# cbiffle/rtiow-rust

Measured on AMD Instinct MI355X. Metric: Msamples/s (pixels*spp/s), book-1 random-spheres 1200x800, higher is better.
Workload: dtype f32

## Files before the change

include/rtiow_gpu_debug.h:

```cpp
#ifndef RTIOW_GPU_DEBUG_H
#define RTIOW_GPU_DEBUG_H
#include "rtiow_gpu.h"
#ifdef __cplusplus
extern "C" {
#endif

int rtg_debug_box_plan(rtg_builder* b, const rtg_id* world, size_t n, const uint32_t* words, size_t n_records,
                       uint8_t* mask_out, size_t capacity);

#ifdef __cplusplus
}
#endif
#endif
```

rtiow-rust_amd/capi.py:

```python
import ctypes as C
import math
import os
import time

import numpy as np

from . import noise

c_f32p = C.POINTER(C.c_float)
c_u32p = C.POINTER(C.c_uint32)
c_u8p = C.POINTER(C.c_uint8)

INVALID_ID = 0xFFFFFFFF
FLAG_COUNTERS = 1
FLAG_TRACE_KERNEL = 2
FLAG_PARTIAL = 4
FLAG_RESUME = 8
FLAG_SUM_SQUARES = 16
FLAG_SAMPLE_COUNTS = 32
FLAG_RETIRE = 64
RETIRE_MAX_RADIUS = 8
FLAG_DENOISE = 128
DENOISE_MAX_RADIUS = 8
DENOISE_MAX_PATCH = 3
# ... 202 lines not shown
    if be.prefix != "rtg_":
        raise ValueError("%s: %s (prefix %s) does not implement RTG_FLAG_%s" % (_FLAG_OF[part][0], be.path, be.prefix, _FLAG_OF[part][1]))


class Frame:

    def __init__(self, nx, ny, squares=False, counts=False, retire=False, denoise=None, features=None):
        lay = self.layout = FrameLayout(nx, ny, squares, counts, retire, _given(denoise), _given(features))
        self.nx, self.ny, self.squares = nx, ny, lay.squares
        self.buf = np.zeros(lay.words, dtype=np.float32)

        def plane(at, *shape):
            return None if at is None else self.buf[at:at + math.prod(shape)].reshape(shape)

        def block(cls, at):
            return None if at is None else cls.from_buffer(self.buf, at * 4)
        self.planes = plane(0, *((2, ny, nx, 3) if lay.squares else (ny, nx, 3)))
        self.counts = None if lay.counts is None else plane(lay.counts, ny, nx).view(np.uint32)
        self.denoised, self.albedo, self.normal = (plane(at, ny, nx, 3) for at in (lay.denoised, lay.albedo, lay.normal))
        self.depth = plane(lay.depth, ny, nx)
        self.retire, self.denoise, self.features = block(Retire, lay.retire), block(Denoise, lay.denoise), block(Features, lay.features)
        if self.denoise is not None:
            self.set_in(make_denoise(denoise))
        if self.features is not None:
            self.set_in(make_features(features))

    def flags(self):
        return {"squares": self.squares, "counts": self.counts is not None, "retire": self.retire is not None,
                "denoise": self.denoise is not None, "features": self.features is not None}

    def set_in(self, block):
        C.memmove(C.addressof(getattr(self, type(block).__name__.lower())), C.addressof(block), block.OUT_OFFSET)

    def copy_in(self, out=None, counts=None, retire=None):
        if out is not None:
            self.planes[...] = out
        if counts is not None:
            self.counts[...] = counts
        if retire is not None:
            C.memmove(C.addressof(self.retire), C.addressof(retire), C.sizeof(Retire))

    def copy_back(self, out=None, counts=None, retire=None):
        if out is not None:
            out[...] = self.planes
        if counts is not None:
            counts[...] = self.counts
        if retire is not None:
            C.memmove(C.addressof(retire), C.addressof(self.retire), C.sizeof(Retire))


class CountsFrame(Frame):

    def __init__(self, nx, ny, squares=False, retire=False):
        if retire and not squares:
            raise ValueError("a retire frame has two float planes: squares=True")
        super().__init__(nx, ny, squares, True, retire)


class DenoiseFrame(Frame):

    def __init__(self, nx, ny, counts=False, retire=False, denoise=None):
        super().__init__(nx, ny, True, counts, retire, denoise if _given(denoise) else True)


class FeaturesFrame(Frame):

    def __init__(self, nx, ny, squares=False, counts=False, retire=False, denoise=None, features=None):
        super().__init__(nx, ny, squares, counts, retire, denoise, features if _given(features) else True)


def features_frame(nx, ny, squares=False, counts=False, retire=False, denoise=None, features=None):
    return FeaturesFrame(nx, ny, squares, counts, retire, denoise, features)


def denoise_frame(nx, ny, counts=False, retire=False, denoise=None):
    return DenoiseFrame(nx, ny, counts, retire, denoise)


def counts_frame(nx, ny, squares=False, retire=False):
    return CountsFrame(nx, ny, squares, retire)


def _counts_call(out, counts, nx, ny, squares, retire=None):
    counts = np.asarray(counts)
    if counts.shape != (ny, nx):
        raise ValueError("counts= must have shape (ny, nx) = %s" % ((ny, nx),))
    if (out.dtype == np.float32 and out.flags.c_contiguous and counts.dtype == np.uint32 and counts.flags.c_contiguous
            and out.ctypes.data + out.nbytes == counts.ctypes.data
            and (retire is None or C.addressof(retire) == out.ctypes.data + retire_block_offset(nx, ny))):
        return out, None
    f = CountsFrame(nx, ny, squares, retire is not None)
    f.copy_in(out, counts, retire)
    return f.planes, f


def _host_frame(out, nx, ny, squares, kw):
    shape = (2, ny, nx, 3) if squares else (ny, nx, 3)
    if out is None:
        if _resumes(kw):
            raise ValueError("resume=True needs out= (the running sum to continue)")
        return np.zeros(shape, dtype=np.float32)
    if squares and not (isinstance(out, np.ndarray) and out.shape == shape and out.dtype == np.float32 and out.flags.c_contiguous):
        raise ValueError("squares=True needs out= a C-contiguous float32 array of shape %s" % (shape,))
    return out


def _render(supported, call, nx, ny, ns, seed, stats, out, counters, counts, retire, denoise, features, kw, exact, forward=False):
    kw = dict(kw)
    squares = kw.pop("squares", None)
    has_rt, has_dn, has_ft = _given(retire), _given(denoise), _given(features)
    in_place = isinstance(out, Frame)
    f = None
    plain = forward and not (in_place or isinstance(counts, np.ndarray) or isinstance(retire, Retire)
                             or isinstance(denoise, (dict, Denoise)) or isinstance(features, (dict, Features)))
    if plain:
        flags, parts = {"squares": squares, "counts": counts, "retire": retire, "denoise": denoise, "features": features}, ()
    else:
        if has_dn and not squares and (exact or not in_place):
            raise ValueError("denoise= needs squares=True (the filter reads both planes)")
        blocks = [make(x) for x, make in ((denoise, make_denoise), (features, make_features)) if _given(x) and x is not True]
        if in_place:
            f, name = out, type(out).__name__
            if (f.nx, f.ny) != (nx, ny):
                raise ValueError("out= is a %s of another size" % name)
            if isinstance(counts, np.ndarray) or (exact and (counts is not None or retire is not None)):
                raise ValueError("out= a %s brings its own counts / retire views" % name)
            if has_ft and f.features is None:
                raise ValueError("features=: out= must be a FeaturesFrame or an array")
            if (has_dn and f.denoise is None) or (has_rt and f.retire is None):
                raise ValueError("out= a %s has no such block" % name)
            if ((squares is not None or exact) and bool(squares) != f.squares) or (
                    exact and (has_dn != (f.denoise is not None) or has_ft != (f.features is not None))):
                raise ValueError("out= a %s: squares= / denoise= / features= must say what the frame holds" % name)
            if isinstance(retire, Retire):
                blocks.append(retire)
            flags = f.flags()
        else:
            if has_rt and not (isinstance(retire, Retire) and isinstance(counts, np.ndarray) and squares):
                raise ValueError("retire= needs a Retire, squares=True and counts= a uint32 array (the call writes it)")
            if counts is not None and np.asarray(counts).shape != (ny, nx):
                raise ValueError("counts= must have shape (ny, nx) = %s" % ((ny, nx),))
            if out is None and _resumes(kw):
                raise ValueError("resume=True needs out= (the running sum to continue)")
            flags = {"squares": bool(squares), "counts": counts is not None, "retire": has_rt, "denoise": has_dn, "features": has_ft}
        parts = [part for part, on in flags.items() if on]
    for part in parts:
        supported(part)
    if in_place:
        for block in blocks:
            f.set_in(block)
        ret, buf = f, f.buf
    elif (has_dn or has_ft) and not plain:
        f = (FeaturesFrame(nx, ny, squares, counts is not None, has_rt, denoise if has_dn else None, features) if has_ft else
             DenoiseFrame(nx, ny, counts is not None, has_rt, denoise))
        f.copy_in(None if out is None else _host_frame(out, nx, ny, squares, kw), counts, retire if has_rt else None)
        ret, buf = f, f.buf
    else:
        ret = out = buf = _host_frame(out, nx, ny, squares, kw)
        if counts is not None and not plain:
            buf, f = _counts_call(out, counts, nx, ny, squares, retire if has_rt else None)
    p = make_params(nx, ny, ns, seed=seed, flags=FLAG_COUNTERS if stats and counters else 0, **flags, **kw)
    st = call(p, buf)
    if f is not None and not in_place:
        f.copy_back(out, counts if has_rt else None, retire if has_rt else None)
    return (ret, st.as_dict()) if stats else ret


def _adaptive_host(cast, nx, ny, ns, step, target_se, min_samples, budget_s, out, seed, stats, radius, denoise, features, kw):
    if features is not None:
        f = FeaturesFrame(nx, ny, True, True, False, denoise) if out is None else out
        what = "features=: out= must be a FeaturesFrame(nx, ny, squares=True, counts=True, denoise=...)"
    elif denoise is not None:
        f = DenoiseFrame(nx, ny, True) if out is None else out
        what = "denoise=: out= must be a DenoiseFrame(nx, ny, counts=True)"
    else:
        f = CountsFrame(nx, ny, True) if out is None else out
        what = "out= must be a CountsFrame(nx, ny, squares=True)"
    on = {"denoise": True if denoise is not None else None, "features": True if features is not None else None}
    if not isinstance(f, Frame) or (f.nx, f.ny) != (nx, ny) or f.flags() != {
            "squares": True, "counts": True, "retire": False, "denoise": denoise is not None, "features": features is not None}:
        raise ValueError(what)
    for block in (features, denoise):
        if block is not None:
            f.set_in(block)
    more = () if features is None else (f,)
    f.counts[...] = ns
    active = np.ones((ny, nx), dtype=bool)
    t0 = time.perf_counter()
    done = 0
    while done < ns:
        end = min(ns, done + step)
        _, st = cast(end, seed=seed, out=f, sample_begin=done, resume=True, partial=True, squares=True, stats=True, counters=False,
                     **on, **kw)
        if features is not None:
            f.features.compute = 0
        if stats is not None:
            stats.append(st)
        done = end
        held = np.minimum(f.counts, done).astype(np.uint32)
        se = noise.standard_error_counts(f.planes[0], f.planes[1], held)
        if radius:
            retire = noise.retire(active, done, se, min_samples, target_se, radius=radius, present=f.counts > 0)
        else:
            retire = noise.retire(active, done, se, min_samples, target_se)
        f.counts[retire] = done
        active &= ~retire
        pv = CountsFrame(nx, ny)
        pv.copy_in(f.planes[0], held)
        cast(done, seed=seed, out=pv, sample_begin=done, resume=True, **kw)
        if denoise is not None:
            yield (held, pv.planes, se, f.denoised.copy()) + more
        else:
            yield (held, pv.planes, se) + more
        if not active.any():
            return
        if budget_s is not None and time.perf_counter() - t0 >= budget_s:
            return


ERR_INVALID, ERR_EMPTY_BVH, ERR_NAN, ERR_RANGE, ERR_UNSUPPORTED, ERR_DEVICE = -1, -2, -3, -4, -5, -6


class RtError(RuntimeError):
    def __init__(self, code, msg):
        super().__init__("rt error %d: %s" % (code, msg))
        self.code = code


def _f3(v):
    return (C.c_float * 3)(float(v[0]), float(v[1]), float(v[2]))


ABI_SYMBOLS = [
    "version", "last_error", "device_count", "builder_create", "builder_destroy",
    "texture_constant", "texture_checker", "texture_perlin", "builder_set_perlin_tables",
    "material_lambertian", "material_metal", "material_dielectric", "material_diffuse_light",
    "material_isotropic", "object_sphere", "object_rect", "object_flip_normals", "object_translate",
    "object_scale", "object_rotate_y", "object_and", "object_rect_prism", "object_linear_move",
    "object_constant_medium", "object_bvh", "object_bvh_sah", "camera_look", "scene_create", "scene_destroy",
    "scene_set_option", "scene_info", "par_cast", "par_cast_device", "par_cast_multi", "multi_reset", "debug_hit_top", "debug_samples", "debug_math", "debug_flatten", "debug_flatten_pool2", "tonemap", "tonemap_device",
]


class Backend:

    def __init__(self, path, prefix):
        if not os.path.exists(path):
            raise FileNotFoundError(
                "%s not found -- build it first (python -c 'import __graft_entry__ as g; g.build()')" % path)
        self.path = path
        self.prefix = prefix
        self.lib = C.CDLL(path)
        f = self._fn
        f("last_error", C.c_char_p, [])
        f("version", C.c_char_p, [])
        f("builder_create", C.c_int, [C.POINTER(C.c_void_p)])
        f("builder_destroy", None, [C.c_void_p])
        f("texture_constant", C.c_uint32, [C.c_void_p, c_f32p])
        f("texture_checker", C.c_uint32, [C.c_void_p, C.c_uint32, C.c_uint32])
        f("texture_perlin", C.c_uint32, [C.c_void_p, C.c_float])
        f("builder_set_perlin_tables", C.c_int, [C.c_void_p, c_f32p, c_u8p, c_u8p, c_u8p])
        f("material_lambertian", C.c_uint32, [C.c_void_p, C.c_uint32])
        f("material_metal", C.c_uint32, [C.c_void_p, c_f32p, C.c_float])
        f("material_dielectric", C.c_uint32, [C.c_void_p, C.c_float])
        f("material_diffuse_light", C.c_uint32, [C.c_void_p, C.c_uint32, C.c_float])
        f("material_isotropic", C.c_uint32, [C.c_void_p, C.c_uint32])
        f("object_sphere", C.c_uint32, [C.c_void_p, C.c_float, C.c_uint32])
        f("object_rect", C.c_uint32, [C.c_void_p, C.c_int] + [C.c_float] * 5 + [C.c_uint32])
        f("object_flip_normals", C.c_uint32, [C.c_void_p, C.c_uint32])
        f("object_translate", C.c_uint32, [C.c_void_p, c_f32p, C.c_uint32])
        f("object_scale", C.c_uint32, [C.c_void_p, c_f32p, C.c_uint32])
        f("object_rotate_y", C.c_uint32, [C.c_void_p, C.c_float, C.c_uint32])
        f("object_and", C.c_uint32, [C.c_void_p, C.c_uint32, C.c_uint32])
        f("object_rect_prism", C.c_uint32, [C.c_void_p, c_f32p, c_f32p, C.c_uint32])
        f("object_linear_move", C.c_uint32, [C.c_void_p, C.c_uint32, c_f32p])
        f("object_constant_medium", C.c_uint32, [C.c_void_p, C.c_uint32, C.c_float, C.c_uint32])
        f("object_bvh", C.c_uint32, [C.c_void_p, c_u32p, C.c_size_t, C.c_float, C.c_float])
        f("object_bvh_sah", C.c_uint32, [C.c_void_p, c_u32p, C.c_size_t, C.c_float, C.c_float])
        f("camera_look", C.c_int, [c_f32p, c_f32p, c_f32p] + [C.c_float] * 6 + [C.POINTER(Camera)])
        f("scene_create", C.c_int, [C.c_void_p, c_u32p, C.c_size_t, C.c_int, C.POINTER(C.c_void_p)])
        f("scene_destroy", None, [C.c_void_p])
        self._declare_render()
        f("debug_hit_top", C.c_int, [C.c_void_p, C.c_size_t, c_f32p, C.c_uint64, C.c_float, c_f32p, c_u32p])
        f("debug_samples", C.c_int, [C.c_void_p, C.POINTER(Camera), C.POINTER(Params), C.c_size_t,
                                     c_u32p, c_u32p, c_u32p, c_f32p, c_u32p])
        f("debug_math", C.c_int, [C.c_int, C.c_int, C.c_size_t, c_f32p, c_f32p, c_f32p])
        f("tonemap", C.c_int, [C.c_int, C.c_size_t, c_f32p, c_u8p])

    def _declare_render(self):
        f = self._fn
        f("device_count", C.c_int, [C.POINTER(C.c_int)])
        f("scene_set_option", C.c_int, [C.c_void_p, C.c_char_p, C.c_int])
        f("scene_info", C.c_int, [C.c_void_p, c_u32p, c_u32p, c_u32p, C.POINTER(C.c_uint64), c_u32p])
        f("par_cast", C.c_int, [C.c_void_p, C.POINTER(Camera), C.POINTER(Params), c_f32p, C.POINTER(Stats)])
        f("par_cast_device", C.c_int, [C.c_void_p, C.POINTER(Camera), C.POINTER(Params), C.c_void_p,
                                       C.c_void_p, C.POINTER(Stats)])
        f("par_cast_multi", C.c_int, [C.POINTER(C.c_void_p), C.c_int, C.POINTER(Camera), C.POINTER(Params), c_f32p,
                                      C.POINTER(Stats)])
        f("multi_reset", C.c_int, [C.c_char_p, C.POINTER(C.c_uint64)])
        f("debug_flatten", C.c_int, [C.c_void_p, c_u32p, C.c_size_t, c_u32p, c_u32p, c_u32p, C.c_size_t])
        f("debug_flatten_pool2", C.c_int, [C.c_void_p, c_u32p, C.c_size_t, c_u32p, c_u32p, c_u32p, C.c_size_t])
        f("tonemap_device", C.c_int, [C.c_int, C.c_size_t, C.c_void_p, C.c_void_p, C.c_void_p])
        f("debug_box_plan", C.c_int, [C.c_void_p, c_u32p, C.c_size_t, c_u32p, C.c_size_t, c_u8p, C.c_size_t])

    def _fn(self, name, restype, argtypes):
        try:
            fn = getattr(self.lib, self.prefix + name)
        except AttributeError:
            def fn(*_a, _n=self.prefix + name):
                raise RtError(ERR_INVALID, "%s: symbol %s is not exported by this build" % (self.path, _n))
            setattr(self, "_" + name, fn)
            return fn
        fn.restype = restype
        fn.argtypes = argtypes
        setattr(self, "_" + name, fn)
        return fn

    def last_error(self):
        return (self._last_error() or b"").decode()

    def check(self, code):
        if code != 0:
            raise RtError(code, self.last_error())

    def check_id(self, i):
        if i == INVALID_ID:
            raise RtError(-1, self.last_error())
        return i

    def builder(self):
        return Builder(self)

    def device_count(self):
        n = C.c_int(0)
        self.check(self._device_count(C.byref(n)))
        return n.value

    def camera_look(self, look_from, look_at, up, fov, aspect, aperture, focus_dist, exposure=(0.0, 1.0)):
        cam = Camera()
        self.check(self._camera_look(_f3(look_from), _f3(look_at), _f3(up), fov, aspect, aperture,
                                     focus_dist, exposure[0], exposure[1], C.byref(cam)))
        return cam

    def par_cast_multi(self, scenes, camera, nx, ny, ns, seed=0xDEADBEEF, stats=False, out=None, counters=None, **kw):
        kw = dict(kw)
        counts, retire, denoise, features = (kw.pop(k, None) for k in ("counts", "retire", "denoise", "features"))
        return _render(lambda part: _supported(self, part), lambda p, buf: self._par_cast_multi_call(scenes, camera, p, buf),
                       nx, ny, ns, seed, stats, out, True if counters is None else counters, counts, retire, denoise, features, kw,
                       exact=False, forward=True)

    def _par_cast_multi_call(self, scenes, camera, p, buf):
        st = Stats.new()
        arr = (C.c_void_p * len(scenes))(*[s.h for s in scenes])
        self.check(self._par_cast_multi(arr, len(scenes), C.byref(camera), C.byref(p), buf.ctypes.data_as(c_f32p), C.byref(st)))
        return st

    def adaptive_multi(self, scenes, camera, nx, ny, ns, step, target_se, min_samples=16, budget_s=None, out=None, seed=0xDEADBEEF,
                       stats=None, radius=0, denoise=None, features=None, **kw):
        if step < 1:
            raise ValueError("step must be >= 1")
        if not 0 <= radius <= RETIRE_MAX_RADIUS:
            raise ValueError("radius must be in 0 .. %d" % RETIRE_MAX_RADIUS)
        _supported(self, "squares")
        _supported(self, "counts")
        features = make_features(features) if _given(features) else None
        denoise = make_denoise(denoise) if _given(denoise) else None
        yield from _adaptive_host(lambda n, **k: self.par_cast_multi(scenes, camera, nx, ny, n, **k), nx, ny, ns, step,
                                  target_se, min_samples, budget_s, out, seed, stats, radius, denoise, features, kw)

    def multi_reset(self, rccl_library=None):
        n = C.c_uint64(0)
        self.check(self._multi_reset(rccl_library.encode() if rccl_library else None, C.byref(n)))
        return n.value

    def tonemap(self, img, device=0):
        x = np.ascontiguousarray(img, dtype=np.float32)
        out = np.empty(x.shape, dtype=np.uint8)
        self.check(self._tonemap(device, x.size, x.ctypes.data_as(c_f32p), out.ctypes.data_as(c_u8p)))
        return out

    def debug_math(self, op, x, y=None, device=0):
        x = np.ascontiguousarray(x, dtype=np.float32)
        out = np.empty_like(x)
        yp = None
        if y is not None:
            y = np.ascontiguousarray(y, dtype=np.float32)
            yp = y.ctypes.data_as(c_f32p)
        self.check(self._debug_math(device, op, x.size, x.ctypes.data_as(c_f32p), yp,
                                    out.ctypes.data_as(c_f32p)))
        return out


class Builder:

    def __init__(self, backend):
        self.be = backend
        h = C.c_void_p()
        backend.check(backend._builder_create(C.byref(h)))
        self.h = h
        self._scenes = []

    def close(self):
        if self.h:
            self.be._builder_destroy(self.h)
            self.h = None

    def __del__(self):
        try:
            self.close()
        except Exception:
            pass

    def constant(self, color):
        return self.be.check_id(self.be._texture_constant(self.h, _f3(color)))

    def checker(self, t0, t1):
        return self.be.check_id(self.be._texture_checker(self.h, t0, t1))

    def perlin(self, scale):
        return self.be.check_id(self.be._texture_perlin(self.h, scale))

    def set_perlin_tables(self, vecs, perm_x, perm_y, perm_z):
        vecs = np.ascontiguousarray(vecs, dtype=np.float32).reshape(768)
        px, py, pz = (np.ascontiguousarray(a, dtype=np.uint8) for a in (perm_x, perm_y, perm_z))
        self.be.check(self.be._builder_set_perlin_tables(
            self.h, vecs.ctypes.data_as(c_f32p), px.ctypes.data_as(c_u8p), py.ctypes.data_as(c_u8p),
            pz.ctypes.data_as(c_u8p)))

    def lambertian(self, albedo):
        return self.be.check_id(self.be._material_lambertian(self.h, albedo))

    def metal(self, albedo, fuzz):
        return self.be.check_id(self.be._material_metal(self.h, _f3(albedo), fuzz))

    def dielectric(self, ref_idx):
        return self.be.check_id(self.be._material_dielectric(self.h, ref_idx))

    def diffuse_light(self, emission, brightness):
        return self.be.check_id(self.be._material_diffuse_light(self.h, emission, brightness))

    def isotropic(self, albedo):
        return self.be.check_id(self.be._material_isotropic(self.h, albedo))

    def sphere(self, radius, material):
        return self.be.check_id(self.be._object_sphere(self.h, radius, material))

    def rect(self, orthogonal_to, range0, range1, k, material):
        return self.be.check_id(self.be._object_rect(self.h, orthogonal_to, range0[0], range0[1],
                                                     range1[0], range1[1], k, material))

    def flip_normals(self, obj):
        return self.be.check_id(self.be._object_flip_normals(self.h, obj))

    def translate(self, offset, obj):
        return self.be.check_id(self.be._object_translate(self.h, _f3(offset), obj))

    def scale(self, factor, obj):
        return self.be.check_id(self.be._object_scale(self.h, _f3(factor), obj))

    def rotate_y(self, degrees, obj):
        return self.be.check_id(self.be._object_rotate_y(self.h, degrees, obj))

    def and_(self, a, b):
        return self.be.check_id(self.be._object_and(self.h, a, b))

    def rect_prism(self, p0, p1, material):
        return self.be.check_id(self.be._object_rect_prism(self.h, _f3(p0), _f3(p1), material))

    def linear_move(self, obj, motion):
        return self.be.check_id(self.be._object_linear_move(self.h, obj, _f3(motion)))

    def constant_medium(self, boundary, density, material):
        return self.be.check_id(self.be._object_constant_medium(self.h, boundary, density, material))

    def bvh(self, objs, exposure=(0.0, 1.0)):
        arr = (C.c_uint32 * max(1, len(objs)))(*objs)
        return self.be.check_id(self.be._object_bvh(self.h, arr, len(objs), exposure[0], exposure[1]))

    def flatten(self, world):
        arr = (C.c_uint32 * max(1, len(world)))(*world)
        n, feat = C.c_uint32(), C.c_uint32()
        self.be.check(self.be._debug_flatten(self.h, arr, len(world), C.byref(n), C.byref(feat), None, 0))
        words = np.zeros((n.value, 8), dtype=np.uint32)
        self.be.check(self.be._debug_flatten(self.h, arr, len(world), C.byref(n), C.byref(feat),
                                             words.ctypes.data_as(c_u32p), n.value))
        return words, feat.value

    def flatten_pool2(self, world):
        arr = (C.c_uint32 * max(1, len(world)))(*world)
        n = C.c_uint32()
        table = np.zeros(24, dtype=np.uint32)
        self.be.check(self.be._debug_flatten_pool2(self.h, arr, len(world), C.byref(n), table.ctypes.data_as(c_u32p), None, 0))
        words = np.zeros((n.value, 8), dtype=np.uint32)
        self.be.check(self.be._debug_flatten_pool2(self.h, arr, len(world), C.byref(n), table.ctypes.data_as(c_u32p),
                                                   words.ctypes.data_as(c_u32p), n.value))
        items = [tuple(int(v) for v in table[4 * k:4 * k + 4]) for k in range(int(table[20]))]
        return words, items, int(table[21]), int(table[22])

    def box_plan(self, world=None, words=None):
        if words is not None:
            words = np.ascontiguousarray(words, dtype=np.uint32)
            mask = np.zeros(len(words), dtype=np.uint8)
            n = self.be._debug_box_plan(None, None, 0, words.ctypes.data_as(c_u32p), len(words), mask.ctypes.data_as(c_u8p), len(mask))
        else:
            arr = (C.c_uint32 * max(1, len(world)))(*world)
            n = self.be._debug_box_plan(self.h, arr, len(world), None, 0, None, 0)
            if n < 0:
                self.be.check(n)
            mask = np.zeros(n, dtype=np.uint8)
            n = self.be._debug_box_plan(self.h, arr, len(world), None, 0, mask.ctypes.data_as(c_u8p), len(mask))
        if n < 0:
            self.be.check(n)
        return mask

    def bvh_sah(self, objs, exposure=(0.0, 1.0)):
        arr = (C.c_uint32 * max(1, len(objs)))(*objs)
        return self.be.check_id(self.be._object_bvh_sah(self.h, arr, len(objs), exposure[0], exposure[1]))

    def scene(self, world, device=0):
        arr = (C.c_uint32 * max(1, len(world)))(*world)
        h = C.c_void_p()
        self.be.check(self.be._scene_create(self.h, arr, len(world), device, C.byref(h)))
        sc = self.be.scene_class(self.be, h, self)
        sc.apply_env_options()
        return sc


class Scene:
    def __init__(self, backend, handle, builder):
        self.be = backend
        self.h = handle
        self._builder = builder

    def close(self):
        if self.h:
            self.be._scene_destroy(self.h)
            self.h = None

    def __del__(self):
        try:
            self.close()
        except Exception:
            pass

    ENV_OPTIONS = ("kernel", "chunks", "lpt", "lpt_phase1", "lpt_deep", "lpt_shift", "ray_lds", "sync", "block", "wg_per_cu", "window",
                   "box_leave", "refill_min", "gather_min", "run_ahead", "run_ahead_min", "sphere_min", "verbose", "bvh4", "box_chains", "box_prune", "force_rccl", "multi_gather", "multi_planes", "scratch_mb", "frames_in_flight", "small_frames", "drain_share", "hoist", "deep_sized", "mat_lds", "pool2", "p2_refill", "p2_box_leave", "p2_park", "p2_sphere", "p2_prism", "p2_list", "p2_push")

    def set_option(self, name, value):
        self.be.check(self.be._scene_set_option(self.h, name.encode(), int(value)))

    def apply_env_options(self):
        if not hasattr(self.be, "_scene_set_option"):
            return
        for name in self.ENV_OPTIONS:
            v = os.environ.get("RTG_" + name.upper())
            if v is not None:
                self.set_option(name, int(v))

    def info(self):
        a, b, c, d, e = C.c_uint32(), C.c_uint32(), C.c_uint32(), C.c_uint64(), C.c_uint32()
        self.be.check(self.be._scene_info(self.h, C.byref(a), C.byref(b), C.byref(c), C.byref(d), C.byref(e)))
        return {"instructions": a.value, "materials": b.value, "textures": c.value, "hbm_bytes": d.value, "box_followers": e.value}

    def _par_cast_args(self, args, threads):
        return args

    def par_cast(self, camera, nx, ny, ns, seed=0xDEADBEEF, stats=False, out=None, threads=0, counts=None, counters=None,
                 retire=None, denoise=None, features=None, **kw):
        def call(p, buf):
            st = Stats.new()
            self.be.check(self.be._par_cast(*self._par_cast_args(
                [self.h, C.byref(camera), C.byref(p), buf.ctypes.data_as(c_f32p), C.byref(st)], threads)))
            return st
        return _render(lambda part: _supported(self.be, part), call, nx, ny, ns, seed, stats, out,
                       stats if counters is None else counters, counts, retire, denoise, features, kw, exact=True)

    def par_cast_device(self, camera, params, d_out_ptr, stream=None, want_stats=False, sample_begin=None, partial=None,
                        resume=None, squares=None, counts=None, retire=None, denoise=None, features=None):
        over = {"squares": squares, "counts": counts, "retire": retire, "denoise": denoise, "features": features}
        bits = {"squares": FLAG_SUM_SQUARES, "counts": FLAG_SAMPLE_COUNTS, "retire": FLAG_RETIRE, "denoise": FLAG_DENOISE,
                "features": FLAG_FEATURES}
        has = {part: bool(params.flags & bits[part] if on is None else on if isinstance(on, (bool, int)) else True)
               for part, on in over.items()}
        for part in ("features", "denoise", "squares", "counts", "retire"):
            if has[part] if part == "squares" else _given(over[part]):
                _supported(self.be, part)
        lay = FrameLayout(params.nx, params.ny, **has)
        blocks = [(over[part], 4 * at, n) for part, at, n in (("retire", lay.retire, C.sizeof(Retire)),
                                                             ("denoise", lay.denoise, Denoise.OUT_OFFSET),
                                                             ("features", lay.features, Features.OUT_OFFSET))
                  if isinstance(over[part], C.Structure)]
        for block, at, n in blocks:
            self._block_copy(d_out_ptr, block, stream, True, at, n)
        if _given(counts) and counts is not True:
            self._upload_counts(lay, counts, d_out_ptr, stream)
        if sample_begin is not None or partial is not None or resume is not None or any(on is not None for on in over.values()):
            q = Params()
            C.pointer(q)[0] = params
            if sample_begin is not None:
                q.sample_begin = sample_begin
            for on, bit in [(partial, FLAG_PARTIAL), (resume, FLAG_RESUME)] + [(on if on is None else has[part], bits[part])
                                                                             for part, on in over.items()]:
                if on is not None:
                    q.flags = (q.flags | bit) if on else (q.flags & ~bit)
            params = q
        st = Stats.new()
        self.be.check(self.be._par_cast_device(self.h, C.byref(camera), C.byref(params), d_out_ptr, stream,
                                               C.byref(st) if want_stats else None))
        for block, at, _ in blocks:
            self._block_copy(d_out_ptr, block, stream, False, at, C.sizeof(block))
        return st.as_dict() if want_stats else None

    def _block_copy(self, d_out_ptr, block, stream, to_device, offset, nbytes):
        hip, hs = _hip_runtime(), _stream(stream)
        dev, host = C.c_void_p(_device_ptr(d_out_ptr) + offset), C.c_void_p(C.addressof(block))
        what = "hipMemcpyAsync(%s block)" % type(block).__name__.lower()
        _hip_ok(hip.hipMemcpyAsync(*((dev, host, nbytes, 1) if to_device else (host, dev, nbytes, 2)), hs), what)
        _hip_ok(hip.hipStreamSynchronize(hs), what)

    def _upload_counts(self, lay, counts, d_out_ptr, stream):
        hip, hs = _hip_runtime(), _stream(stream)
        dst = C.c_void_p(_device_ptr(d_out_ptr) + 4 * lay.counts)
        if hasattr(counts, "data_ptr") and getattr(counts, "is_cuda", False):
            if tuple(counts.shape) != (lay.ny, lay.nx) or counts.element_size() != 4 or not counts.is_contiguous():
                raise ValueError("counts= must be a contiguous 4-byte [ny, nx] tensor")
            _hip_ok(hip.hipMemcpyAsync(dst, C.c_void_p(counts.data_ptr()), 4 * lay.n, 3, hs), "hipMemcpyAsync(count plane)")
        else:
            host = np.ascontiguousarray(counts, dtype=np.uint32)
            if host.shape != (lay.ny, lay.nx):
                raise ValueError("counts= must have shape (ny, nx) = %s" % ((lay.ny, lay.nx),))
            _hip_ok(hip.hipMemcpyAsync(dst, C.c_void_p(host.ctypes.data), 4 * lay.n, 1, hs), "hipMemcpyAsync(count plane)")
            _hip_ok(hip.hipStreamSynchronize(hs), "hipMemcpyAsync(count plane)")

    def _loop_block(self, part, given, make):
        if not _given(given):
            return None
        _supported(self.be, part)
        return make(given)

    def adaptive(self, camera, nx, ny, ns, step, target_se, min_samples=16, budget_s=None, out=None, seed=0xDEADBEEF,
                 stats=None, radius=0, preview=None, stream=None, denoise=None, denoised=None, features=None, **kw):
        if step < 1:
            raise ValueError("step must be >= 1")
        _supported(self.be, "squares")
        _supported(self.be, "counts")
        if not 0 <= radius <= RETIRE_MAX_RADIUS:
            raise ValueError("radius must be in 0 .. %d" % RETIRE_MAX_RADIUS)
        features, denoise = self._loop_block("features", features, make_features), self._loop_block("denoise", denoise, make_denoise)
        if out is not None and not isinstance(out, Frame):
            _supported(self.be, "retire")
            if preview is None:
                raise ValueError("a device frame needs a device preview buffer (preview=)")
            if denoise is not None and denoised is None:
                raise ValueError("denoise= on a device frame needs a device buffer for the filtered frame (denoised=)")
            yield from self._adaptive_device(camera, nx, ny, ns, step, target_se, min_samples, budget_s, out, seed, stats,
                                             radius, preview, stream, kw, denoise, denoised, features)
            return
        yield from _adaptive_host(lambda n, **k: self.par_cast(camera, nx, ny, n, **k), nx, ny, ns, step, target_se,
                                  min_samples, budget_s, out, seed, stats, radius, denoise, features, kw)

    def _adaptive_device(self, camera, nx, ny, ns, step, target_se, min_samples, budget_s, out, seed, stats, radius, preview,
                         stream, kw, denoise=None, denoised=None, features=None):
        hip, hs, ok = _hip_runtime(), _stream(stream), _hip_ok
        d_out, d_pv = _device_ptr(out), _device_ptr(preview)
        lay = FrameLayout(nx, ny, True, True, True, denoise is not None, features is not None)
        plane, counts_at = lay.n, d_out + 4 * lay.counts
        ok(hip.hipMemsetD32Async(C.c_void_p(counts_at), ns - (1 << 32) if ns >= 1 << 31 else ns, plane, hs), "hipMemsetD32Async(counts)")
        block = Retire(target_se=float(target_se), min_samples=int(min_samples), radius=int(radius))
        self._block_copy(d_out, block, stream, True, 4 * lay.retire, C.sizeof(Retire))
        if denoise is not None:
            self._block_copy(d_out, denoise, stream, True, 4 * lay.denoise, Denoise.OUT_OFFSET)
        more = ()
        if features is not None:
            self._block_copy(d_out, features, stream, True, 4 * lay.features, Features.OUT_OFFSET)
            more = (4 * lay.features,)
        t0 = time.perf_counter()
        done = 0
        while done < ns:
            end = min(ns, done + step)
            st = self.par_cast_device(camera, make_params(nx, ny, end, seed=seed, sample_begin=done, resume=True, partial=True,
                                                          squares=True, counts=True, retire=True, denoise=denoise is not None,
                                                          features=features is not None, **kw), d_out, hs,
                                      want_stats=stats is not None)
            if features is not None and features.compute:
                features.compute = 0
                self._block_copy(d_out, features, stream, True, 4 * lay.features, Features.OUT_OFFSET)
            if denoise is not None:
                ok(hip.hipMemcpyAsync(C.c_void_p(_device_ptr(denoised)), C.c_void_p(d_out + 4 * lay.denoised), plane * 3 * 4, 3, hs),
                   "hipMemcpyAsync(denoised)")
            if stats is not None:
                stats.append(st)
            done = end
            ok(hip.hipMemcpyAsync(C.c_void_p(d_pv), C.c_void_p(d_out), plane * 3 * 4, 3, hs), "hipMemcpyAsync(preview)")
            ok(hip.hipMemcpyAsync(C.c_void_p(d_pv + plane * 3 * 4), C.c_void_p(counts_at), plane * 4, 3, hs), "hipMemcpyAsync(preview counts)")
            self.par_cast_device(camera, make_params(nx, ny, done, seed=seed, sample_begin=done, resume=True, counts=True, **kw),
                                 d_pv, hs)
            self._block_copy(d_out, block, stream, False, 4 * lay.retire, C.sizeof(Retire))
            info = block.as_dict()
            if denoise is not None:
                yield (done, preview, info, denoised) + more
            else:
                yield (done, preview, info) + more
            if info["active"] == 0:
                return
            if budget_s is not None and time.perf_counter() - t0 >= budget_s:
                return

    def progressive(self, camera, nx, ny, ns, step, seed=0xDEADBEEF, budget_s=None, out=None, preview=None, stream=None,
                    squares=False, target_rmse=None, denoise=None, denoised=None, features=None, **kw):
        if step < 1:
            raise ValueError("step must be >= 1")
        features = self._loop_block("features", features, make_features)
        squares = bool(squares) or target_rmse is not None or _given(denoise)
        if squares:
            _supported(self.be, "squares")
        denoise = self._loop_block("denoise", denoise, make_denoise)
        if out is not None and not isinstance(out, np.ndarray):
            if target_rmse is not None:
                raise ValueError("target_rmse needs host frames: there is no device-side error reduction")
            if preview is None:
                raise ValueError("a device running sum needs a device preview buffer (preview=)")
            if denoise is not None and denoised is None:
                raise ValueError("denoise= on a device frame needs a device buffer for the filtered frame (denoised=)")
            yield from self._progressive_device(camera, nx, ny, ns, step, seed, budget_s, out, preview, stream, squares, kw,
                                                denoise, denoised, features)
            return
        shape = (2, ny, nx, 3) if squares else (ny, nx, 3)
        acc = np.zeros(shape, dtype=np.float32) if out is None else out
        frame = None
        if features is not None:
            frame = FeaturesFrame(nx, ny, squares, denoise=denoise, features=features)
        elif denoise is not None:
            frame = DenoiseFrame(nx, ny, denoise=denoise)
        if frame is not None:
            frame.copy_in(acc)
        on = {"denoise": True if denoise is not None else None, "features": True if features is not None else None}
        more = () if features is None else (frame,)
        sums = acc[0] if squares else acc
        t0 = time.perf_counter()
        done = 0
        while done < ns:
            end = min(ns, done + step)
            self.par_cast(camera, nx, ny, end, seed=seed, out=acc if frame is None else frame, sample_begin=done, resume=True, partial=True,
                          squares=squares, **on, **kw)
            if frame is not None:
                frame.copy_back(acc)
            if features is not None:
                frame.features.compute = 0
            done = end
            pv = sums.copy()
            self.par_cast(camera, nx, ny, done, seed=seed, out=pv, sample_begin=done, resume=True, **kw)
            if squares:
                se = noise.standard_error(acc[0], acc[1], done)
                if denoise is not None:
                    yield (done, pv, se, frame.denoised.copy()) + more
                else:
                    yield (done, pv, se) + more
                if target_rmse is not None and float(np.sqrt(np.mean(se * se))) <= target_rmse:
                    return
            else:
                yield (done, pv) + more
            if budget_s is not None and time.perf_counter() - t0 >= budget_s:
                return

    def _progressive_device(self, camera, nx, ny, ns, step, seed, budget_s, acc, preview, stream, squares, kw, denoise=None,
                            denoised=None, features=None):
        hip, hs = _hip_runtime(), _stream(stream)
        d_acc, d_preview = C.c_void_p(_device_ptr(acc)), C.c_void_p(_device_ptr(preview))
        lay = FrameLayout(nx, ny, squares, False, False, denoise is not None, features is not None)
        if denoise is not None:
            self._block_copy(acc, denoise, stream, True, 4 * lay.denoise, Denoise.OUT_OFFSET)
        more = ()
        if features is not None:
            self._block_copy(acc, features, stream, True, 4 * lay.features, Features.OUT_OFFSET)
            more = (4 * lay.features,)
        t0 = time.perf_counter()
        done = 0
        while done < ns:
            end = min(ns, done + step)
            self.par_cast_device(camera, make_params(nx, ny, end, seed=seed, sample_begin=done, resume=True, partial=True,
                                                     squares=squares, denoise=denoise is not None, features=features is not None,
                                                     **kw), d_acc, hs)
            if features is not None and features.compute:
                features.compute = 0
                self._block_copy(acc, features, stream, True, 4 * lay.features, Features.OUT_OFFSET)
            done = end
            if denoise is not None:
                _hip_ok(hip.hipMemcpyAsync(C.c_void_p(_device_ptr(denoised)), C.c_void_p(d_acc.value + 4 * lay.denoised), lay.n * 3 * 4, 3, hs),
                        "hipMemcpyAsync(denoised)")
            _hip_ok(hip.hipMemcpyAsync(d_preview, d_acc, lay.n * 3 * 4, 3, hs), "hipMemcpyAsync(preview)")
            self.par_cast_device(camera, make_params(nx, ny, done, seed=seed, sample_begin=done, resume=True, **kw), d_preview, hs)
            if denoise is not None:
                yield (done, preview, acc, denoised) + more
            else:
                yield ((done, preview, acc) if squares else (done, preview)) + more
            if budget_s is not None:
                _hip_ok(hip.hipStreamSynchronize(hs), "hipStreamSynchronize")
                if time.perf_counter() - t0 >= budget_s:
                    return

    def debug_hit_top(self, rays, seed=1, t_near=0.001):
        rays = np.ascontiguousarray(rays, dtype=np.float32).reshape(-1, 7)
        n = rays.shape[0]
        out = np.zeros((n, 8), dtype=np.float32)
        mat = np.zeros(n, dtype=np.uint32)
        self.be.check(self.be._debug_hit_top(self.h, n, rays.ctypes.data_as(c_f32p), seed, t_near,
                                             out.ctypes.data_as(c_f32p), mat.ctypes.data_as(c_u32p)))
        return out, mat

    def debug_samples(self, camera, nx, ny, ns, xs, ys, samples, seed=0xDEADBEEF, trace_kernel=False, **kw):
        p = make_params(nx, ny, ns, seed=seed, flags=FLAG_TRACE_KERNEL if trace_kernel else 0, **kw)
        xs, ys, samples = (np.ascontiguousarray(a, dtype=np.uint32) for a in (xs, ys, samples))
        n = xs.size
        rgb = np.zeros((n, 3), dtype=np.float32)
        info = np.zeros((n, 4), dtype=np.uint32)
        self.be.check(self.be._debug_samples(self.h, C.byref(camera), C.byref(p), n,
                                             xs.ctypes.data_as(c_u32p), ys.ctypes.data_as(c_u32p),
                                             samples.ctypes.data_as(c_u32p), rgb.ctypes.data_as(c_f32p),
                                             info.ctypes.data_as(c_u32p)))
        return rgb, info


Backend.scene_class = Scene
```

rtiow-rust_amd/csrc/rt_box_plan.h:

```cpp
#pragma once
#include <cmath>
#include <cstddef>
#include <cstdint>
#include <cstring>
#include <vector>

#include "flat_scene.h"

namespace rtg {

constexpr uint8_t BOX_KEPT = 0, BOX_FOLLOWER = 1, BOX_PRUNED = 2;
#ifndef RT_BOX_PLAN_PROBES
#define RT_BOX_PLAN_PROBES 256
#endif
#ifndef RT_BOX_PLAN_FULL
#define RT_BOX_PLAN_FULL 0
#endif
constexpr uint32_t BOX_PLAN_PROBES = RT_BOX_PLAN_PROBES;
constexpr bool BOX_PLAN_FULL = RT_BOX_PLAN_FULL != 0;

struct BoxPlan {
  uint32_t n_pruned = 0;
  uint32_t n_sure = 0;
  uint32_t n_rays = 0;
};

namespace box_plan_detail {
inline float as_f(uint32_t u) {
  float f;
  std::memcpy(&f, &u, 4);
  return f;
}
inline bool aabb_hit(const uint32_t* lo, const uint32_t* hi, const float* o, const float* inv, float t_near, float best) {
  const float mn[3] = {as_f(lo[0]), as_f(lo[2]), as_f(hi[0])}, mx[3] = {as_f(lo[1]), as_f(lo[3]), as_f(hi[1])};
  float t0[3], t1[3];
  for (int a = 0; a < 3; a++) {
    const float u = (mn[a] - o[a]) * inv[a], v = (mx[a] - o[a]) * inv[a];
    t0[a] = inv[a] < 0.f ? v : u, t1[a] = inv[a] < 0.f ? u : v;
  }
  const float start = fmaxf(t_near, fmaxf(fmaxf(t0[0], t0[1]), t0[2]));
  const float end = fminf(best, fminf(fminf(t1[0], t1[1]), t1[2]));
  return end > start;
}
inline bool sphere_hit(const uint32_t* lo, uint32_t flags, const float* o, const float* d, float dd, float t_near, float best, float* t_out) {
  float p[3] = {o[0], o[1], o[2]};
  if (flags & F_TRANSLATE)
    for (int a = 0; a < 3; a++) p[a] = o[a] - as_f(lo[a]);
  const float r = as_f(lo[3]);
  const float b = p[0] * d[0] + p[1] * d[1] + p[2] * d[2];
  const float c = p[0] * p[0] + p[1] * p[1] + p[2] * p[2] - r * r;
  const float disc = b * b - dd * c;
  if (disc > 0.f) {
    const float sq = sqrtf(disc);
    float t = (-b - sq) / dd;
    if (t < best && t >= t_near) return *t_out = t, true;
    t = (-b + sq) / dd;
    if (t < best && t >= t_near) return *t_out = t, true;
  }
  return false;
}
struct Rng {
  uint64_t s;
  uint64_t next() {
    uint64_t z = (s += 0x9e3779b97f4a7c15ull);
    z = (z ^ (z >> 30)) * 0xbf58476d1ce4e5b9ull;
    z = (z ^ (z >> 27)) * 0x94d049bb133111ebull;
    return z ^ (z >> 31);
  }
  float unit() { return (float)(next() >> 40) * (1.f / 16777216.f); }
  void in_unit_sphere(float* v) {
    do {
      for (int a = 0; a < 3; a++) v[a] = 2.f * unit() - 1.f;
    } while (v[0] * v[0] + v[1] * v[1] + v[2] * v[2] >= 1.f);
  }
};
}

inline BoxPlan box_plan(const uint32_t (*lo)[4], const uint32_t (*hi)[4], size_t n, const uint8_t* follower, uint8_t* mask,
                        uint8_t* sure = nullptr, uint32_t n_probes = BOX_PLAN_PROBES) {
  using namespace box_plan_detail;
  BoxPlan out;
  for (size_t j = 0; j < n; j++) {
    mask[j] = follower && follower[j] ? BOX_FOLLOWER : BOX_KEPT;
    if (sure) sure[j] = 0;
  }
  auto op = [&](size_t j) { return hi[j][3] & 0xffu; };
  auto skip = [&](size_t j) { return (size_t)hi[j][2]; };
  if (n < 4 || n > 0x7fffffffu) return out;
  std::vector<int32_t> parent(n, -1);
  std::vector<uint32_t> depth(n, 0);
  {
    std::vector<uint32_t> open;
    for (size_t j = 0; j < n; j++) {
      while (!open.empty() && skip(open.back()) <= j) open.pop_back();
      if (!open.empty()) parent[j] = (int32_t)open.back(), depth[j] = (uint32_t)open.size();
      if (op(j) != OP_BOX) continue;
      if (skip(j) <= j || skip(j) >= n || (!open.empty() && skip(j) > skip(open.back()))) return out;
      open.push_back((uint32_t)j);
    }
  }
  auto leaf_box = [&](size_t j) { return op(j) == OP_BOX && j + 2 < n && op(j + 1) == OP_SPHERE && skip(j) == j + 2; };
  auto finite6 = [&](size_t j) {
    return std::isfinite(as_f(lo[j][0])) && std::isfinite(as_f(lo[j][1])) && std::isfinite(as_f(lo[j][2])) &&
           std::isfinite(as_f(lo[j][3])) && std::isfinite(as_f(hi[j][0])) && std::isfinite(as_f(hi[j][1]));
  };
  auto contains = [&](size_t j, size_t c) {
    return as_f(lo[j][0]) <= as_f(lo[c][0]) && as_f(lo[j][1]) >= as_f(lo[c][1]) && as_f(lo[j][2]) <= as_f(lo[c][2]) &&
           as_f(lo[j][3]) >= as_f(lo[c][3]) && as_f(hi[j][0]) <= as_f(hi[c][0]) && as_f(hi[j][1]) >= as_f(hi[c][1]);
  };
  std::vector<uint8_t> prunable(n, 0);
  uint32_t n_prunable = 0;
  for (size_t j = n; j-- > 0;) {
    if (op(j) != OP_BOX || j + 1 >= n || op(j + 1) != OP_BOX) continue;
    const size_t L = j + 1, R = skip(L);
    if (!(L < R && R < skip(j)) || op(R) != OP_BOX || skip(R) != skip(j)) continue;
    if (!finite6(j) || !finite6(L) || !finite6(R) || !contains(j, L) || !contains(j, R)) continue;
    if (!(leaf_box(L) || prunable[L]) || !(leaf_box(R) || prunable[R])) continue;
    prunable[j] = 1, n_prunable++;
  }
  if (!n_prunable) return out;
  std::vector<uint8_t> choosable(prunable);
  for (size_t j = 0; j + 1 < n; j++) {
    if (!prunable[j] || !follower) continue;
    size_t k = j + 1;
    while (k + 1 < n && follower[k] && !leaf_box(k)) k++;
    if (follower[k] && leaf_box(k)) choosable[j] = 0;
  }

  std::vector<uint64_t> n_pass(n, 0);
  std::vector<uint32_t> spheres, starts;
  for (size_t j = 0; j < n; j++)
    if (op(j) == OP_SPHERE) spheres.push_back((uint32_t)j);
  auto centre = [&](uint32_t j, float* c) {
    for (int a = 0; a < 3; a++) c[a] = (hi[j][3] & F_TRANSLATE) ? as_f(lo[j][a]) : 0.f;
  };
  float cmin[3] = {INFINITY, INFINITY, INFINITY}, cmax[3] = {-INFINITY, -INFINITY, -INFINITY};
  for (uint32_t j : spheres) {
    float c[3];
    centre(j, c);
    for (int a = 0; a < 3; a++) cmin[a] = fminf(cmin[a], c[a]), cmax[a] = fmaxf(cmax[a], c[a]);
  }
  std::vector<uint8_t> enclosing(n, 0);
  for (uint32_t j : spheres) {
    float cj[3];
    centre(j, cj);
    const float r = as_f(lo[j][3]);
    float far2 = 0.f;
    for (int a = 0; a < 3; a++) {
      const float d = fmaxf(cmax[a] - cj[a], cj[a] - cmin[a]);
      far2 += d * d;
    }
    const bool all = spheres.size() > 1 && far2 < r * r;
    enclosing[j] = all;
    if (!all && std::isfinite(r) && std::isfinite(cj[0]) && std::isfinite(cj[1]) && std::isfinite(cj[2])) starts.push_back(j);
  }
  uint64_t n_rays = 0;
  if (!starts.empty()) {
    Rng rng{0x626f78706c616e31ull ^ (uint64_t)n};
    const float t_near = 0.001f;
    while (n_rays < n_probes) {
      const uint32_t s0 = starts[rng.next() % starts.size()];
      float c[3], nrm[3], o[3], d[3], v[3];
      centre(s0, c);
      do rng.in_unit_sphere(nrm);
      while (nrm[0] * nrm[0] + nrm[1] * nrm[1] + nrm[2] * nrm[2] < 1e-4f);
      const float len = sqrtf(nrm[0] * nrm[0] + nrm[1] * nrm[1] + nrm[2] * nrm[2]), r0 = as_f(lo[s0][3]);
      for (int a = 0; a < 3; a++) nrm[a] /= len, o[a] = c[a] + r0 * nrm[a];
      const uint32_t bounces = 1u + (uint32_t)(rng.next() % 3u);
      for (uint32_t k = 0; k <= bounces && n_rays < n_probes; k++) {
        rng.in_unit_sphere(v);
        for (int a = 0; a < 3; a++) d[a] = nrm[a] + v[a];
        const float inv[3] = {1.f / d[0], 1.f / d[1], 1.f / d[2]};
        const float dd = d[0] * d[0] + d[1] * d[1] + d[2] * d[2];
        float best = 3.402823466e+38f;
        int64_t best_pc = -1;
        n_rays++;
        for (size_t pc = 0; pc < n;) {
          const uint32_t o_ = op(pc);
          if (o_ == OP_BOX) {
            if (aabb_hit(lo[pc], hi[pc], o, inv, t_near, best)) n_pass[pc]++, pc++;
            else pc = skip(pc);
          } else if (o_ == OP_SPHERE) {
            float t;
            if (sphere_hit(lo[pc], hi[pc][3], o, d, dd, t_near, best, &t)) best = t, best_pc = (int64_t)pc;
            pc++;
          } else break;
        }
        if (best_pc < 0 || enclosing[best_pc]) break;
        centre((uint32_t)best_pc, c);
        const float r = as_f(lo[best_pc][3]);
        for (int a = 0; a < 3; a++) o[a] = o[a] + best * d[a], nrm[a] = (o[a] - c[a]) / r;
        if (!(std::isfinite(nrm[0]) && std::isfinite(nrm[1]) && std::isfinite(nrm[2]))) break;
      }
    }
  }
  out.n_rays = (uint32_t)n_rays;

  uint64_t states = 0;
  for (size_t j = 0; BOX_PLAN_FULL && j < n; j++)
    if (op(j) == OP_BOX) states += depth[j] + 2u;
  const bool dp = BOX_PLAN_FULL && states <= (1ull << 26);
  std::vector<uint32_t> kidx(n, 0);
  std::vector<uint8_t> pruned(n, 0);
  if (dp) {
    std::vector<std::vector<uint64_t>> acc(n);
    std::vector<std::vector<uint8_t>> choice(n);
    std::vector<uint64_t> path_pass;
    for (size_t j = n; j-- > 0;) {
      if (op(j) != OP_BOX) continue;
      const uint32_t dj = depth[j];
      if (acc[j].empty()) acc[j].assign(dj + 2u, 0);
      path_pass.assign(dj + 1u, n_rays);
      for (int32_t a = parent[j], k = (int32_t)dj; a >= 0; a = parent[a], k--) path_pass[k] = n_pass[a];
      std::vector<uint64_t> f(dj + 1u);
      choice[j].assign(dj + 1u, 0);
      for (uint32_t k = 0; k <= dj; k++) {
        const uint64_t own = follower && follower[j] ? 0u : path_pass[k];
        const uint64_t keep = own + acc[j][dj + 1u], leave = acc[j][k];
        if (choosable[j] && leave <= keep) f[k] = leave, choice[j][k] = 1;
        else f[k] = keep;
      }
      std::vector<uint64_t>().swap(acc[j]);
      if (parent[j] >= 0) {
        std::vector<uint64_t>& up = acc[parent[j]];
        if (up.empty()) up.assign(dj + 1u, 0);
        for (uint32_t k = 0; k <= dj; k++) up[k] += f[k];
      }
    }
    for (size_t j = 0; j < n; j++) {
      if (op(j) != OP_BOX) continue;
      const int32_t p = parent[j];
      kidx[j] = p < 0 ? 0u : (pruned[p] ? kidx[p] : depth[j]);
      pruned[j] = choice[j][kidx[j]];
    }
  } else {
    for (size_t j = 0; j < n; j++) pruned[j] = choosable[j] && n_rays && n_pass[j] == n_rays;
  }
  for (size_t j = 0; j < n; j++) {
    if (!pruned[j] || mask[j] == BOX_FOLLOWER) continue;
    mask[j] = BOX_PRUNED, out.n_pruned++;
    if (n_pass[j] == n_rays) {
      out.n_sure++;
      if (sure) sure[j] = 1;
    }
  }
  return out;
}

}
```

rtiow-rust_amd/csrc/rtg_api.hip:

```cpp
#include <hip/hip_runtime.h>

#include <dlfcn.h>
#include <rccl/rccl.h>

#include <chrono>
#include <cmath>
#include <cstdio>
#include <cstdlib>
#include <cstring>
#include <map>
#include <mutex>
#include <functional>
#include <string>
#include <tuple>
#include <vector>

#include "../../include/rtiow_gpu.h"
#include "../../include/rtiow_gpu_debug.h"
#include "rt_pool.h"
#include "rt_box_plan.h"
#include "rt_retire.h"
#include "rt_denoise.h"
#include "rt_features.h"
#include "rt_multi_planes.h"
#include "rt_pool_full.h"
#include "rt_sync_full.h"
#include "rt_pool2.h"
#include "rt_trace.h"
#include "scene_builder.h"

using namespace rtg;

#include "rtg_kernels.inc"

namespace {
thread_local std::string g_err;

int fail(int code, const std::string& msg) {
  g_err = msg;
  return code;
}
int hip_fail(hipError_t e, const char* what) {
  return fail(RTG_ERR_DEVICE, std::string(what) + ": " + hipGetErrorString(e));
}
#define HIP_TRY(expr)                                   \
  do {                                                  \
    hipError_t e_ = (expr);                             \
    if (e_ != hipSuccess) return hip_fail(e_, #expr);   \
  } while (0)
}

struct rtg_builder {
  SceneBuilder sb;
};

constexpr int RTG_MAX_FRAMES = 4;
enum class KernelKind { baseline, lean_pool, full_pool, lock_step, pool2 };
struct LaunchCtx {
  unsigned long long* d_counters = nullptr;
  hipEvent_t ev0 = nullptr, ev1 = nullptr, done = nullptr;
  bool busy = false;
  float* d_stack = nullptr;
  size_t stack_bytes = 0;
  uint32_t* d_slots = nullptr;
  size_t slots_bytes = 0;
  float* d_scratch = nullptr;
  size_t scratch_bytes = 0;
  LaunchConsts* d_consts = nullptr;
  uint32_t* d_lpt = nullptr;
  size_t lpt_bytes = 0;
  LptQueue lpt_desc{};
  KernelKind last_kernel = KernelKind::baseline;
  uint32_t last_pix_work = 0;
  uint32_t* d_list = nullptr;
  size_t list_bytes = 0;
  uint32_t* d_compact = nullptr;
  size_t compact_bytes = 0;
  unsigned long long counts_samples = 0;
  void* d_retire = nullptr;
  size_t retire_bytes = 0;
  const char* refusal = nullptr;
  void* d_denoise = nullptr;
  size_t denoise_bytes = 0;
  rtg_denoise denoise_in{};
  uint32_t* d_features = nullptr;
  size_t features_bytes = 0;
  rtg_features features_in{};
};

struct rtg_scene {
  int device = 0;
  DevScene dev{};
  uint32_t features = 0;
  uint32_t n_prog = 0, n_mat = 0, n_tex = 0;
  uint64_t bytes = 0;
  void* buffers[15] = {};
  const uint32_t* d_parent = nullptr;
  hipStream_t own_stream = nullptr;
  int num_cus = 0;
  float* d_frame = nullptr;
  size_t frame_bytes = 0;
  int force_chunks = 0;
  uint64_t scratch_limit = 0;
  bool whole_scratch = false;
  int verbose = 0;
  int window = -1;
  int ray_lds = 1;
  int force_rccl = 0;
  int multi_gather = 0;
  float* d_pack = nullptr;
  size_t pack_bytes = 0;
  float* d_recv = nullptr;
  size_t recv_bytes = 0;
  int multi_planes = 0;
  hipEvent_t post0 = nullptr, post1 = nullptr;
  hipEvent_t pack0 = nullptr, pack1 = nullptr, unpack0 = nullptr;
  int bvh4 = 0;
  uint32_t wide_bytes = 0;
  int box_chains = 1;
  uint32_t n_followers = 0;
  const uint32_t* d_chain_off = nullptr;
  uint32_t chain_bytes = 0;
  int box_prune = 1;
  uint32_t n_pruned = 0;
  float plan_ms = 0.f;
  const uint32_t* d_prune_off[2] = {nullptr, nullptr};
  uint32_t prune_bytes[2] = {0, 0};
  std::vector<uint32_t> plan_ops;
  std::vector<uint8_t> plan_mask;
  int sync_full = -1;
  uint32_t n_box = 0;
  int lpt = 2;
  int lpt_deep = 4;
  int lpt_shift = 0;
  int lpt_phase1 = 0;
  int kernel_version = 3;
  PoolTuning pool_tune{40, 16, 24, 16, 16, 40};
  PoolTuning full_tune{20, 24, 32, 16, 24, 40};
  PoolTuning sync_tune{20, 16, 32, 16, 16, 40};
  int wg_per_cu = 0;
  int full_threads = 0;
  int pool_threads = 0;
  int mat_lds = 1;
  int deep_sized = 1;
  int hoist = 1;
  uint32_t seg_first = 0, seg_end = 0;
  int drain_share = 1;
  int pool2 = 1;
  uint32_t n_prog2 = 0, n_box2 = 0;
  DevScene dev2{};
  const P2Table* d_p2 = nullptr;
  Pool2Tuning pool2_tune{24, 48, 40, 4, 8, 24, 2};
  int guide_lds = 0;
  int small_frames = 1;
  LaunchCtx ctx[RTG_MAX_FRAMES];
  int n_ctx = 1, next_ctx = 0;
  LaunchCtx* cx = &ctx[0];
};

static void ctx_free_buffers(LaunchCtx* c) {
  if (c->busy) (void)hipEventSynchronize(c->done);
  c->busy = false;
  if (c->d_scratch) (void)hipFree(c->d_scratch);
  if (c->d_slots) (void)hipFree(c->d_slots);
  if (c->d_stack) (void)hipFree(c->d_stack);
  if (c->d_lpt) (void)hipFree(c->d_lpt);
  if (c->d_list) (void)hipFree(c->d_list);
  if (c->d_compact) (void)hipFree(c->d_compact);
  if (c->d_retire) (void)hipFree(c->d_retire);
  if (c->d_denoise) (void)hipFree(c->d_denoise);
  if (c->d_features) (void)hipFree(c->d_features);
  c->d_scratch = nullptr, c->scratch_bytes = 0, c->d_slots = nullptr, c->slots_bytes = 0;
  c->d_stack = nullptr, c->stack_bytes = 0, c->d_lpt = nullptr, c->lpt_bytes = 0;
  c->d_list = nullptr, c->list_bytes = 0, c->d_compact = nullptr, c->compact_bytes = 0;
  c->d_retire = nullptr, c->retire_bytes = 0;
  c->d_denoise = nullptr, c->denoise_bytes = 0;
  c->d_features = nullptr, c->features_bytes = 0;
}

static int ctx_acquire(rtg_scene* s) {
  LaunchCtx* c = &s->ctx[s->next_ctx];
  s->next_ctx = (s->next_ctx + 1) % s->n_ctx;
  if (!c->d_counters) {
    if (hipMalloc((void**)&c->d_counters, 64 * sizeof(unsigned long long)) != hipSuccess || hipMemset(c->d_counters, 0, 64 * sizeof(unsigned long long)) != hipSuccess ||
        hipMalloc((void**)&c->d_consts, sizeof(LaunchConsts) + sizeof(ListConsts)) != hipSuccess || hipEventCreate(&c->ev0) != hipSuccess ||
        hipEventCreate(&c->ev1) != hipSuccess || hipEventCreateWithFlags(&c->done, hipEventDisableTiming) != hipSuccess)
      return fail(RTG_ERR_DEVICE, "scene: launch-context allocation failed");
  }
  if (c->busy) {
    hipError_t e = hipEventSynchronize(c->done);
    c->busy = false;
    if (e != hipSuccess) return hip_fail(e, "hipEventSynchronize(previous frame of this launch context)");
  }
  s->cx = c;
  return RTG_OK;
}
static int ctx_release(rtg_scene* s, hipStream_t stream) {
  hipError_t e = hipEventRecord(s->cx->done, stream);
  if (e != hipSuccess) return hip_fail(e, "hipEventRecord(done)");
  s->cx->busy = true;
  return RTG_OK;
}

struct SampleSlice {
  uint32_t begin = 0;
  bool divide = true;
  bool squares = false;
  bool counts = false;
  uint32_t list_work = 0;
  ListConsts list{};
  bool retire = false;
  bool denoise = false;
  bool features = false;
  bool features_done = false;
  bool sliced() const { return begin != 0u || !divide; }
};
static SampleSlice slice_of(const rtg_params* p) {
  SampleSlice sl;
  if (p->flags & RTG_FLAG_RESUME) sl.begin = p->sample_begin;
  if (p->flags & RTG_FLAG_PARTIAL) sl.divide = false;
  if (p->flags & RTG_FLAG_SUM_SQUARES) sl.squares = true;
  if (p->flags & RTG_FLAG_SAMPLE_COUNTS) sl.counts = true;
  if (p->flags & RTG_FLAG_RETIRE) sl.retire = true;
  if (p->flags & RTG_FLAG_DENOISE) sl.denoise = true;
  if (p->flags & RTG_FLAG_FEATURES) sl.features = true;
  return sl;
}

static const char* retire_refusal(const rtg_retire& r, uint32_t nranks) {
  if (r.radius > RTG_RETIRE_MAX_RADIUS) return "RTG_FLAG_RETIRE: radius > RTG_RETIRE_MAX_RADIUS";
  if (!(r.target_se >= 0.0)) return "RTG_FLAG_RETIRE: target_se is NaN or negative";
  if (r.radius > 0u && nranks > 1u) return "RTG_FLAG_RETIRE: radius > 0 needs nranks = 1 (the neighbours live on other ranks)";
  return nullptr;
}

static const char* denoise_refusal(const rtg_denoise& r, uint32_t nranks) {
  if (r.radius > RTG_DENOISE_MAX_RADIUS) return "RTG_FLAG_DENOISE: radius > RTG_DENOISE_MAX_RADIUS";
  if (r.patch > RTG_DENOISE_MAX_PATCH) return "RTG_FLAG_DENOISE: patch > RTG_DENOISE_MAX_PATCH";
  if (!(r.k > 0.f) || !std::isfinite(r.k)) return "RTG_FLAG_DENOISE: k is NaN, infinite or <= 0";
  if (r.reserved_in != 0u) return "RTG_FLAG_DENOISE: reserved_in != 0";
  if (nranks > 1u) return "RTG_FLAG_DENOISE needs nranks = 1 (the neighbours live on other ranks)";
  return nullptr;
}

static const char* features_refusal(const rtg_features& r, bool denoise) {
  if (r.grid == 0u || r.grid > RTG_FEATURES_MAX_GRID) return "RTG_FLAG_FEATURES: grid is 0 or > RTG_FEATURES_MAX_GRID";
  if (r.compute > 1u) return "RTG_FLAG_FEATURES: compute > 1";
  if (r.reserved_in != 0u) return "RTG_FLAG_FEATURES: reserved_in != 0";
  for (float sg : {r.sigma_normal, r.sigma_albedo, r.sigma_depth})
    if (denoise && (!(sg > 0.f) || !std::isfinite(sg))) return "RTG_FLAG_FEATURES with RTG_FLAG_DENOISE: a sigma is NaN, infinite or <= 0";
  return nullptr;
}

#include "rtg_launch.inc"

template <typename T>
struct DevBuf {
  T* p = nullptr;
  ~DevBuf() {
    if (p) (void)hipFree(p);
  }
  hipError_t alloc(size_t n) { return hipMalloc((void**)&p, (n ? n : 1) * sizeof(T)); }
};

extern "C" {

const char* rtg_version(void) { return "rtiow-rust_amd 0.2 (gfx950 HIP; flat-program ray-pool kernels; flat-program encoding 3: OP_SEG = 9, OP_SAVE / OP_MERGE / OP_EXT = 10 / 11 / 12, OP_LIST = 13, MEDIUM lo.y = 1 / density)"; }
const char* rtg_last_error(void) { return g_err.c_str(); }

int rtg_device_count(int* n) {
  if (!n) return fail(RTG_ERR_INVALID, "null argument");
  int c = 0;
  hipError_t e = hipGetDeviceCount(&c);
  if (e != hipSuccess) {
    *n = 0;
    return hip_fail(e, "hipGetDeviceCount");
  }
  *n = c;
  return RTG_OK;
}

int rtg_builder_create(rtg_builder** out) {
  if (!out) return fail(RTG_ERR_INVALID, "null argument");
  *out = new rtg_builder();
  return RTG_OK;
}
void rtg_builder_destroy(rtg_builder* b) { delete b; }

static rtg_id bad(const char* msg) {
  fail(RTG_ERR_INVALID, msg);
  return RTG_INVALID_ID;
}

rtg_id rtg_texture_constant(rtg_builder* b, const float rgb[3]) {
  if (!b || !rgb) return bad("null argument");
  HostTexture t;
  t.kind = TEX_CONSTANT;
  t.rgb[0] = rgb[0], t.rgb[1] = rgb[1], t.rgb[2] = rgb[2];
  b->sb.textures.push_back(t);
  return (rtg_id)b->sb.textures.size() - 1;
}
rtg_id rtg_texture_checker(rtg_builder* b, rtg_id t0, rtg_id t1) {
  if (!b) return bad("null argument");
  if (t0 >= b->sb.textures.size() || t1 >= b->sb.textures.size()) return bad("checker: bad texture handle");
  HostTexture t;
  t.kind = TEX_CHECKER;
  t.t0 = t0, t.t1 = t1;
  b->sb.textures.push_back(t);
  return (rtg_id)b->sb.textures.size() - 1;
}
rtg_id rtg_texture_perlin(rtg_builder* b, float scale) {
  if (!b) return bad("null argument");
  if (!b->sb.has_perlin) return bad("perlin: call rtg_builder_set_perlin_tables first");
  HostTexture t;
  t.kind = TEX_PERLIN;
  t.scale = scale;
  b->sb.textures.push_back(t);
  return (rtg_id)b->sb.textures.size() - 1;
}
int rtg_builder_set_perlin_tables(rtg_builder* b, const float vecs[768], const uint8_t px[256],
                                  const uint8_t py[256], const uint8_t pz[256]) {
  if (!b || !vecs || !px || !py || !pz) return fail(RTG_ERR_INVALID, "null argument");
  for (int i = 0; i < 256; i++) {
    b->sb.perlin_vecs[4 * i] = vecs[3 * i], b->sb.perlin_vecs[4 * i + 1] = vecs[3 * i + 1];
    b->sb.perlin_vecs[4 * i + 2] = vecs[3 * i + 2], b->sb.perlin_vecs[4 * i + 3] = 0.f;
    b->sb.perlin_perm[i] = px[i], b->sb.perlin_perm[256 + i] = py[i], b->sb.perlin_perm[512 + i] = pz[i];
  }
  b->sb.has_perlin = true;
  return RTG_OK;
}

static rtg_id push_material(rtg_builder* b, uint32_t kind, rtg_id tex, const float* albedo, float param) {
  if (!b) return bad("null argument");
  HostMaterial m;
  m.kind = kind;
  if (tex != RTG_INVALID_ID) {
    if (tex >= b->sb.textures.size()) return bad("material: bad texture handle");
    m.tex = tex;
  }
  if (albedo) m.albedo[0] = albedo[0], m.albedo[1] = albedo[1], m.albedo[2] = albedo[2];
  m.param = param;
  b->sb.materials.push_back(m);
  return (rtg_id)b->sb.materials.size() - 1;
}
rtg_id rtg_material_lambertian(rtg_builder* b, rtg_id albedo) {
  if (albedo == RTG_INVALID_ID) return bad("material: bad texture handle");
  return push_material(b, MAT_LAMBERTIAN, albedo, nullptr, 0.f);
}
rtg_id rtg_material_metal(rtg_builder* b, const float albedo[3], float fuzz) {
  if (!albedo) return bad("null argument");
  return push_material(b, MAT_METAL, RTG_INVALID_ID, albedo, fuzz);
}
rtg_id rtg_material_dielectric(rtg_builder* b, float ref_idx) {
  return push_material(b, MAT_DIELECTRIC, RTG_INVALID_ID, nullptr, ref_idx);
}
rtg_id rtg_material_diffuse_light(rtg_builder* b, rtg_id emission, float brightness) {
  if (emission == RTG_INVALID_ID) return bad("material: bad texture handle");
  return push_material(b, MAT_DIFFUSE_LIGHT, emission, nullptr, brightness);
}
rtg_id rtg_material_isotropic(rtg_builder* b, rtg_id albedo) {
  if (albedo == RTG_INVALID_ID) return bad("material: bad texture handle");
  return push_material(b, MAT_ISOTROPIC, albedo, nullptr, 0.f);
}

static rtg_id push_object(rtg_builder* b, const HostObject& o) {
  if (!b) return bad("null argument");
  try {
    return b->sb.add_object(o);
  } catch (const BuildError& e) {
    fail(e.code, e.msg);
    return RTG_INVALID_ID;
  }
}
rtg_id rtg_object_sphere(rtg_builder* b, float radius, rtg_id material) {
  HostObject o;
  o.kind = HostObject::SPHERE;
  o.f[0] = radius;
  o.mat = material;
  return push_object(b, o);
}
rtg_id rtg_object_rect(rtg_builder* b, int axis, float r0s, float r0e, float r1s, float r1e, float k, rtg_id material) {
  HostObject o;
  o.kind = HostObject::RECT;
  o.axis = axis;
  o.f[0] = k, o.f[1] = r0s, o.f[2] = r0e, o.f[3] = r1s, o.f[4] = r1e;
  o.mat = material;
  return push_object(b, o);
}
static rtg_id wrapper(rtg_builder* b, HostObject::Kind kind, const float* v, rtg_id child) {
  HostObject o;
  o.kind = kind;
  if (v) o.f[0] = v[0], o.f[1] = v[1], o.f[2] = v[2];
  o.a = child;
  return push_object(b, o);
}
rtg_id rtg_object_flip_normals(rtg_builder* b, rtg_id object) { return wrapper(b, HostObject::FLIP, nullptr, object); }
rtg_id rtg_object_translate(rtg_builder* b, const float offset[3], rtg_id object) {
  if (!offset) return bad("null argument");
  return wrapper(b, HostObject::TRANSLATE, offset, object);
}
rtg_id rtg_object_scale(rtg_builder* b, const float factor[3], rtg_id object) {
  if (!factor) return bad("null argument");
  return wrapper(b, HostObject::SCALE, factor, object);
}
rtg_id rtg_object_rotate_y(rtg_builder* b, float degrees, rtg_id object) {
  float radians = degrees * 3.14159265358979323846f / 180.f;
  float sc[3] = {sinf(radians), cosf(radians), 0.f};
  return wrapper(b, HostObject::ROTATE_Y, sc, object);
}
rtg_id rtg_object_and(rtg_builder* b, rtg_id o0, rtg_id o1) {
  HostObject o;
  o.kind = HostObject::AND;
  o.a = o0, o.b = o1;
  return push_object(b, o);
}
rtg_id rtg_object_rect_prism(rtg_builder* b, const float p0[3], const float p1[3], rtg_id m) {
  if (!b || !p0 || !p1) return bad("null argument");
  rtg_id zp = rtg_object_rect(b, 2, p0[0], p1[0], p0[1], p1[1], p1[2], m);
  rtg_id yp = rtg_object_rect(b, 1, p0[0], p1[0], p0[2], p1[2], p1[1], m);
  rtg_id xp = rtg_object_rect(b, 0, p0[1], p1[1], p0[2], p1[2], p1[0], m);
  if (zp == RTG_INVALID_ID || yp == RTG_INVALID_ID || xp == RTG_INVALID_ID) return RTG_INVALID_ID;
  rtg_id zn = rtg_object_flip_normals(b, rtg_object_rect(b, 2, p0[0], p1[0], p0[1], p1[1], p0[2], m));
  rtg_id yn = rtg_object_flip_normals(b, rtg_object_rect(b, 1, p0[0], p1[0], p0[2], p1[2], p0[1], m));
  rtg_id xn = rtg_object_flip_normals(b, rtg_object_rect(b, 0, p0[1], p1[1], p0[2], p1[2], p0[0], m));
  return rtg_object_and(b, rtg_object_and(b, zp, rtg_object_and(b, yp, xp)),
                        rtg_object_and(b, zn, rtg_object_and(b, yn, xn)));
}
rtg_id rtg_object_linear_move(rtg_builder* b, rtg_id object, const float motion[3]) {
  if (!motion) return bad("null argument");
  return wrapper(b, HostObject::MOVE, motion, object);
}
rtg_id rtg_object_constant_medium(rtg_builder* b, rtg_id boundary, float density, rtg_id material) {
  HostObject o;
  o.kind = HostObject::MEDIUM;
  o.f[0] = density;
  o.a = boundary;
  o.mat = material;
  return push_object(b, o);
}
rtg_id rtg_object_bvh(rtg_builder* b, const rtg_id* objects, size_t n, float e0, float e1) {
  if (!b || (!objects && n)) return bad("null argument");
  try {
    return b->sb.add_bvh(objects, n, e0, e1);
  } catch (const BuildError& e) {
    fail(e.code, e.msg);
    return RTG_INVALID_ID;
  }
}

rtg_id rtg_object_bvh_sah(rtg_builder* b, const rtg_id* objects, size_t n, float e0, float e1) {
  if (!b || (!objects && n)) return bad("null argument");
  try {
    return b->sb.add_bvh(objects, n, e0, e1, true);
  } catch (const BuildError& e) {
    fail(e.code, e.msg);
    return RTG_INVALID_ID;
  }
}

int rtg_camera_look(const float from[3], const float at[3], const float up[3], float fov, float aspect,
                    float aperture, float focus_dist, float e0, float e1, rtg_camera* out) {
  if (!from || !at || !up || !out) return fail(RTG_ERR_INVALID, "null argument");
  auto dot3 = [](const float* a, const float* b) { return (a[0] * b[0] + a[1] * b[1]) + a[2] * b[2]; };
  auto unit = [&](float* v) {
    float len = sqrtf(dot3(v, v));
    v[0] = v[0] / len, v[1] = v[1] / len, v[2] = v[2] / len;
  };
  auto cross3 = [](const float* a, const float* b, float* r) {
    r[0] = a[1] * b[2] - a[2] * b[1];
    r[1] = -(a[0] * b[2] - a[2] * b[0]);
    r[2] = a[0] * b[1] - a[1] * b[0];
  };
  float lens_radius = aperture / 2.f;
  float theta = fov * 3.14159265358979323846f / 180.f;
  float half_height = tanf(theta / 2.f);
  float half_width = aspect * half_height;
  float w[3] = {from[0] - at[0], from[1] - at[1], from[2] - at[2]};
  unit(w);
  float u[3], v[3];
  cross3(up, w, u);
  unit(u);
  cross3(w, u, v);
  float hw_fd = half_width * focus_dist, hh_fd = half_height * focus_dist;
  float h2 = (2.f * half_width) * focus_dist, v2 = (2.f * half_height) * focus_dist;
  for (int i = 0; i < 3; i++) {
    out->origin[i] = from[i];
    out->lower_left_corner[i] = ((from[i] - hw_fd * u[i]) - hh_fd * v[i]) - focus_dist * w[i];
    out->horizontal[i] = h2 * u[i];
    out->vertical[i] = v2 * v[i];
    out->u[i] = u[i];
    out->v[i] = v[i];
  }
  out->lens_radius = lens_radius;
  out->exposure_start = e0;
  out->exposure_end = e1;
  return RTG_OK;
}

static int upload(void** dst, const void* src, size_t bytes, uint64_t* total) {
  size_t alloc = bytes ? bytes : 16;
  HIP_TRY(hipMalloc(dst, alloc));
  if (bytes) HIP_TRY(hipMemcpy(*dst, src, bytes, hipMemcpyHostToDevice));
  *total += alloc;
  return RTG_OK;
}

static int prune_table(rtg_scene* s, int chains) {
  if (s->d_prune_off[chains] || !s->n_pruned) return RTG_OK;
  const size_t n = s->plan_mask.size();
  std::vector<uint8_t> drop(n);
  std::vector<uint32_t> off(n);
  for (size_t i = 0; i < n; i++) drop[i] = s->plan_mask[i] == BOX_PRUNED || (chains && s->plan_mask[i] == BOX_FOLLOWER);
  s->prune_bytes[chains] = lds_image_offsets(s->plan_ops.data(), n, off.data(), drop.data());
  int rc = upload(&s->buffers[13 + chains], off.data(), n * sizeof(uint32_t), &s->bytes);
  if (rc) return rc;
  s->d_prune_off[chains] = (const uint32_t*)s->buffers[13 + chains];
  return RTG_OK;
}

void rtg_scene_destroy(rtg_scene* s) {
  if (!s) return;
  (void)hipSetDevice(s->device);
  for (void* p : s->buffers)
    if (p) (void)hipFree(p);
  for (LaunchCtx& c : s->ctx) {
    ctx_free_buffers(&c);
    if (c.d_counters) (void)hipFree(c.d_counters);
    if (c.d_consts) (void)hipFree(c.d_consts);
    if (c.ev0) (void)hipEventDestroy(c.ev0);
    if (c.ev1) (void)hipEventDestroy(c.ev1);
    if (c.done) (void)hipEventDestroy(c.done);
  }
  if (s->d_frame) (void)hipFree(s->d_frame);
  if (s->d_pack) (void)hipFree(s->d_pack);
  if (s->d_recv) (void)hipFree(s->d_recv);
  if (s->post0) (void)hipEventDestroy(s->post0);
  if (s->post1) (void)hipEventDestroy(s->post1);
  for (hipEvent_t ev : {s->pack0, s->pack1, s->unpack0})
    if (ev) (void)hipEventDestroy(ev);
  if (s->own_stream) (void)hipStreamDestroy(s->own_stream);
  delete s;
}

int rtg_scene_create(rtg_builder* b, const rtg_id* world, size_t n, int device, rtg_scene** out) {
  if (!b || !out || (!world && n)) return fail(RTG_ERR_INVALID, "null argument");
  FlatScene fs;
  try {
    b->sb.flatten(world, n, &fs);
  } catch (const BuildError& e) {
    return fail(e.code, e.msg);
  }
  int ndev = 0;
  if (hipGetDeviceCount(&ndev) != hipSuccess || ndev == 0)
    return fail(RTG_ERR_DEVICE, "no HIP device: the rtiow hot path has no CPU fallback");
  if (device < 0 || device >= ndev) return fail(RTG_ERR_INVALID, "bad device index");
  HIP_TRY(hipSetDevice(device));
  rtg_scene* s = new rtg_scene();
  s->device = device;
  s->features = fs.features;
  s->n_prog = (uint32_t)fs.lo.size();
  s->n_mat = (uint32_t)fs.mat.size() / 2;
  s->n_tex = (uint32_t)fs.tex.size() / 2;
  int rc;
  if ((rc = upload(&s->buffers[0], fs.lo.data(), fs.lo.size() * 16, &s->bytes)) ||
      (rc = upload(&s->buffers[1], fs.hi.data(), fs.hi.size() * 16, &s->bytes)) ||
      (rc = upload(&s->buffers[2], fs.mat.data(), fs.mat.size() * 16, &s->bytes)) ||
      (rc = upload(&s->buffers[3], fs.tex.data(), fs.tex.size() * 16, &s->bytes)) ||
      (rc = upload(&s->buffers[4], fs.perlin_vecs.data(), sizeof(float) * 1024, &s->bytes)) ||
      (rc = upload(&s->buffers[5], fs.perlin_perm.data(), 768, &s->bytes))) {
    rtg_scene_destroy(s);
    return rc;
  }
  s->dev.lo = (const uint4*)s->buffers[0];
  s->dev.hi = (const uint4*)s->buffers[1];
  s->dev.mat = (const uint4*)s->buffers[2];
  s->dev.tex = (const uint4*)s->buffers[3];
  s->dev.perlin_vecs = (const float4*)s->buffers[4];
  s->dev.perlin_perm = (const uint8_t*)s->buffers[5];
  s->dev.n_prog = s->n_prog;
  s->dev.n_mat = s->n_mat;
  for (const Packet& h : fs.hi) s->n_box += (h.w[3] & 0xffu) == OP_BOX ? 1u : 0u;
  {
    std::vector<uint32_t> parent(fs.hi.size(), 0xffffffffu), open;
    for (size_t i = 0; i < fs.hi.size(); i++) {
      const uint32_t op = fs.hi[i].w[3] & 0xffu;
      if (op == OP_POP && !open.empty()) open.pop_back();
      parent[i] = open.empty() ? 0xffffffffu : open.back();
      if (op == OP_PUSH) open.push_back((uint32_t)i);
    }
    if ((rc = upload(&s->buffers[8], parent.data(), parent.size() * sizeof(uint32_t), &s->bytes))) {
      rtg_scene_destroy(s);
      return rc;
    }
    s->d_parent = (const uint32_t*)s->buffers[8];
  }
  for (size_t i = 0; i < fs.hi.size(); i++)
    if ((fs.hi[i].w[3] & 0xffu) == OP_SEG) s->seg_first = (uint32_t)i + 1u, s->seg_end = fs.hi[i].w[2];
  if (!fs.hi2.empty()) {
    if ((rc = upload(&s->buffers[9], fs.lo2.data(), fs.lo2.size() * 16, &s->bytes)) ||
        (rc = upload(&s->buffers[10], fs.hi2.data(), fs.hi2.size() * 16, &s->bytes)) ||
        (rc = upload(&s->buffers[11], &fs.p2, sizeof(P2Table), &s->bytes))) {
      rtg_scene_destroy(s);
      return rc;
    }
    s->dev2 = s->dev;
    s->dev2.lo = (const uint4*)s->buffers[9], s->dev2.hi = (const uint4*)s->buffers[10];
    s->dev2.n_prog = s->n_prog2 = (uint32_t)fs.hi2.size();
    s->dev2.lds_off = nullptr, s->dev2.lds_image_bytes = 0;
    s->d_p2 = (const P2Table*)s->buffers[11];
    for (const Packet& h : fs.hi2) s->n_box2 += (h.w[3] & 0xffu) == OP_BOX ? 1u : 0u;
  }
  if ((fs.features & (FEAT_ALL | FEAT_BOUNDARY)) == 0) {
    std::vector<uint32_t> ops(fs.hi.size()), off(fs.hi.size());
    for (size_t i = 0; i < fs.hi.size(); i++) ops[i] = fs.hi[i].w[3];
    s->dev.lds_image_bytes = lds_image_offsets(ops.data(), ops.size(), off.data());
    if ((rc = upload(&s->buffers[6], off.data(), off.size() * sizeof(uint32_t), &s->bytes))) {
      rtg_scene_destroy(s);
      return rc;
    }
    s->dev.lds_off = (const uint32_t*)s->buffers[6];
    std::vector<uint8_t> follower(fs.hi.size());
    s->n_followers = box_chain_followers(reinterpret_cast<const uint32_t (*)[4]>(fs.lo.data()), reinterpret_cast<const uint32_t (*)[4]>(fs.hi.data()), fs.hi.size(), follower.data());
    if (s->n_followers) {
      s->chain_bytes = lds_image_offsets(ops.data(), ops.size(), off.data(), follower.data());
      if ((rc = upload(&s->buffers[12], off.data(), off.size() * sizeof(uint32_t), &s->bytes))) {
        rtg_scene_destroy(s);
        return rc;
      }
      s->d_chain_off = (const uint32_t*)s->buffers[12];
    }
    if (s->dev.lds_image_bytes - LDS_BOX_BYTES * (s->n_box / 2u) <= 160u * 1024u) {
      s->plan_mask.resize(fs.hi.size());
      const auto t0 = std::chrono::steady_clock::now();
      s->n_pruned = box_plan(reinterpret_cast<const uint32_t (*)[4]>(fs.lo.data()), reinterpret_cast<const uint32_t (*)[4]>(fs.hi.data()), fs.hi.size(), follower.data(), s->plan_mask.data()).n_pruned;
      s->plan_ms = std::chrono::duration<float, std::milli>(std::chrono::steady_clock::now() - t0).count();
      if (s->n_pruned) {
        s->plan_ops = ops;
        if ((rc = prune_table(s, 1))) {
          rtg_scene_destroy(s);
          return rc;
        }
      }
    }
    std::vector<uint32_t> wide;
    if (build_wide_image(fs.lo.data(), fs.hi.data(), fs.hi.size(), wide)) {
      if ((rc = upload(&s->buffers[7], wide.data(), wide.size() * sizeof(uint32_t), &s->bytes))) {
        rtg_scene_destroy(s);
        return rc;
      }
      s->wide_bytes = (uint32_t)(wide.size() * sizeof(uint32_t));
    }
  }
  hipDeviceProp_t prop;
  if (hipGetDeviceProperties(&prop, device) == hipSuccess) s->num_cus = prop.multiProcessorCount;
  if (s->num_cus <= 0) s->num_cus = 256;
  if ((rc = ctx_acquire(s))) {
    rtg_scene_destroy(s);
    return rc;
  }
  s->next_ctx = 0;
  *out = s;
  return RTG_OK;
}


int rtg_scene_set_option(rtg_scene* s, const char* name, int value) {
  if (!s || !name) return fail(RTG_ERR_INVALID, "null argument");
  const std::string k(name);
  const uint32_t u = (uint32_t)value;
  if (k == "kernel") s->kernel_version = value;
  else if (k == "chunks") s->force_chunks = value;
  else if (k == "scratch_mb") s->scratch_limit = value > 0 ? (uint64_t)value << 20 : 0;
  else if (k == "lpt") s->lpt = value;
  else if (k == "lpt_phase1") s->lpt_phase1 = value;
  else if (k == "lpt_deep") s->lpt_deep = value;
  else if (k == "lpt_shift") s->lpt_shift = std::min(6, std::max(0, value));
  else if (k == "ray_lds") s->ray_lds = value;
  else if (k == "box_chains") {
    if (!value) {
      HIP_TRY(hipSetDevice(s->device));
      int rc = prune_table(s, 0);
      if (rc) return rc;
    }
    s->box_chains = value;
  }
  else if (k == "box_prune") {
    if (value < 0 || value > 2) return fail(RTG_ERR_INVALID, "box_prune: 0 .. 2");
    s->box_prune = value;
  }
  else if (k == "bvh4") {
    if (value && !s->wide_bytes) return fail(RTG_ERR_INVALID, "bvh4: the scene is not one Bvh of spheres (no 4-wide image)");
    if (value && pool_lds_bytes(s->wide_bytes, s->n_mat, (uint32_t)(s->pool_threads > 0 ? s->pool_threads : RT_POOL_MAX_THREADS) / 64u, true, false) > 160 * 1024)
      return fail(RTG_ERR_INVALID, "bvh4: the 4-wide image does not fit a CU's 160 KB of LDS (the 4-wide walk only exists LDS-staged)");
    s->bvh4 = value;
  }
  else if (k == "frames_in_flight") {
    if (value < 1 || value > RTG_MAX_FRAMES) return fail(RTG_ERR_INVALID, "frames_in_flight: 1 .. 4");
    HIP_TRY(hipSetDevice(s->device));
    for (int i = value; i < RTG_MAX_FRAMES; i++) ctx_free_buffers(&s->ctx[i]);
    s->n_ctx = value, s->next_ctx = 0;
  }
  else if (k == "force_rccl") s->force_rccl = value;
  else if (k == "multi_gather") s->multi_gather = value;
  else if (k == "multi_planes") s->multi_planes = value;
  else if (k == "sync") s->sync_full = value;
  else if (k == "block") {
    if (value < 64 || value > 1024 || value % 64) return fail(RTG_ERR_INVALID, "block: a multiple of 64 in [64, 1024]");
    s->pool_threads = s->full_threads = value;
  }
  else if (k == "wg_per_cu") s->wg_per_cu = value;
  else if (k == "drain_share") s->drain_share = value;
  else if (k == "hoist") s->hoist = value;
  else if (k == "pool2") s->pool2 = value;
  else if (k == "deep_sized") s->deep_sized = value;
  else if (k == "mat_lds") s->mat_lds = value;
  else if (k == "guide_lds") s->guide_lds = value;
  else if (k == "small_frames") s->small_frames = value;
  else if (k == "verbose") s->verbose = value;
  else if (k == "window") s->window = value;
  else if (k == "box_leave") s->pool_tune.box_leave = s->full_tune.box_leave = s->sync_tune.box_leave = u;
  else if (k == "refill_min") s->pool_tune.refill_min = s->full_tune.refill_min = s->sync_tune.refill_min = u;
  else if (k == "gather_min") s->pool_tune.gather_min = s->full_tune.gather_min = s->sync_tune.gather_min = u;
  else if (k == "run_ahead") s->pool_tune.run_ahead = s->full_tune.run_ahead = s->sync_tune.run_ahead = u;
  else if (k == "run_ahead_min") s->pool_tune.run_ahead_min = s->full_tune.run_ahead_min = s->sync_tune.run_ahead_min = u;
  else if (k == "sphere_min") s->pool_tune.sphere_min = s->full_tune.sphere_min = s->sync_tune.sphere_min = std::max(1u, u);
  else if (k == "p2_refill") s->pool2_tune.refill_min = u;
  else if (k == "p2_box_leave") s->pool2_tune.box_leave = u;
  else if (k == "p2_park") s->pool2_tune.park_max = u;
  else if (k == "p2_sphere") s->pool2_tune.t_sphere = std::max(1u, u);
  else if (k == "p2_prism") s->pool2_tune.t_prism = std::max(1u, u);
  else if (k == "p2_list") s->pool2_tune.t_list = std::max(1u, u);
  else if (k == "p2_push") s->pool2_tune.t_push = std::max(1u, u);
  else return fail(RTG_ERR_INVALID, "rtg_scene_set_option: unknown option '" + k + "'");
  return RTG_OK;
}

int rtg_scene_info(const rtg_scene* s, uint32_t* n_instructions, uint32_t* n_materials, uint32_t* n_textures,
                   uint64_t* hbm_bytes, uint32_t* n_box_followers) {
  if (!s) return fail(RTG_ERR_INVALID, "null argument");
  if (n_instructions) *n_instructions = s->n_prog;
  if (n_materials) *n_materials = s->n_mat;
  if (n_textures) *n_textures = s->n_tex;
  if (hbm_bytes) *hbm_bytes = s->bytes;
  if (n_box_followers) *n_box_followers = s->n_followers;
  return RTG_OK;
}

static DevCamera to_dev(const rtg_camera* c) {
  DevCamera d;
  auto v = [](const float* p) { return V3{p[0], p[1], p[2]}; };
  d.origin = v(c->origin), d.llc = v(c->lower_left_corner), d.horizontal = v(c->horizontal);
  d.vertical = v(c->vertical), d.u = v(c->u), d.v = v(c->v);
  d.lens_radius = c->lens_radius, d.e0 = c->exposure_start, d.e1 = c->exposure_end;
  return d;
}

static int check_params(const rtg_scene* s, const rtg_camera* camera, const rtg_params* p, DevParams* out) {
  if (!s || !camera || !p) return fail(RTG_ERR_INVALID, "null argument");
  if (p->struct_size != sizeof(rtg_params)) return fail(RTG_ERR_INVALID, "rtg_params.struct_size mismatch");
  if (p->nx == 0 || p->ny == 0 || p->ns == 0) return fail(RTG_ERR_INVALID, "nx, ny, ns must be > 0");
  if ((uint64_t)p->nx * p->ny > 0xffffffffull) return fail(RTG_ERR_INVALID, "image too large for 32-bit pixel index");
  if (!(camera->exposure_start < camera->exposure_end))
    return fail(RTG_ERR_RANGE, "Uniform::sample_single called with low >= high");
  if (!std::isfinite(camera->exposure_start) || !std::isfinite(camera->exposure_end))
    return fail(RTG_ERR_RANGE, "Uniform::sample_single called with non-finite boundaries");
  if (!std::isfinite(camera->exposure_end - camera->exposure_start))
    return fail(RTG_ERR_RANGE, "exposure range wider than f32::MAX is not supported");
  DevParams d;
  d.nx = p->nx, d.ny = p->ny, d.ns = p->ns, d.max_bounces = p->max_bounces;
  d.t_near = p->t_near;
  d.seed_lo = (uint32_t)p->seed, d.seed_hi = (uint32_t)(p->seed >> 32);
  d.tile_w = p->tile_w ? p->tile_w : 16u;
  d.tile_h = p->tile_h ? p->tile_h : 16u;
  if (d.tile_w % 8u || d.tile_h % 8u) return fail(RTG_ERR_INVALID, "tile_w / tile_h must be multiples of 8");
  d.nranks = p->nranks ? p->nranks : 1u;
  d.rank = p->rank;
  if (d.rank >= d.nranks) return fail(RTG_ERR_INVALID, "rank >= nranks");
  if ((p->flags & RTG_FLAG_RESUME) && p->sample_begin > p->ns) return fail(RTG_ERR_INVALID, "RTG_FLAG_RESUME: sample_begin > ns");
  if ((p->flags & RTG_FLAG_RETIRE) && (~p->flags & (RTG_FLAG_SAMPLE_COUNTS | RTG_FLAG_SUM_SQUARES)))
    return fail(RTG_ERR_INVALID, "RTG_FLAG_RETIRE needs RTG_FLAG_SAMPLE_COUNTS | RTG_FLAG_SUM_SQUARES");
  if ((p->flags & RTG_FLAG_DENOISE) && !(p->flags & RTG_FLAG_SUM_SQUARES)) return fail(RTG_ERR_INVALID, "RTG_FLAG_DENOISE needs RTG_FLAG_SUM_SQUARES");
  if ((p->flags & RTG_FLAG_DENOISE) && d.nranks > 1u) return fail(RTG_ERR_INVALID, "RTG_FLAG_DENOISE needs nranks = 1 (the neighbours live on other ranks)");
  *out = d;
  return RTG_OK;
}

static int print_schedule_stats(rtg_scene* s, float ms) {
  if (s->cx->lpt_desc.n_blocks && s->cx->d_lpt) {
    std::vector<uint32_t> ctl(LPT_CTL);
    HIP_TRY(hipMemcpy(ctl.data(), s->cx->lpt_desc.ctl, LPT_CTL * sizeof(uint32_t), hipMemcpyDeviceToHost));
    std::string line;
    for (uint32_t c = 0; c < LPT_CLASSES; c++)
      if (ctl[c]) line += " " + std::to_string(c) + ":" + std::to_string(ctl[c]);
    fprintf(stderr, "[rtg] cost-ordered queue: %u of %u blocks filed, class:blocks%s\n", ctl[LPT_CLASSES], s->cx->lpt_desc.n_blocks, line.c_str());
  }
  unsigned long long q[24];
  HIP_TRY(hipMemcpy(q, s->cx->d_counters + 8, sizeof(q), hipMemcpyDeviceToHost));
  if (q[18]) {
    const double us = (double)ms * 1000. / (double)q[16], n = (double)q[18];
    fprintf(stderr, "[rtg] wave timeline (us from its start): sees the work queue empty at min %.0f / mean %.0f / max %.0f; done at mean %.0f / max %.0f\n",
            (double)((1ull << 62) - q[19]) * us, (double)q[20] / n * us, (double)q[21] * us, (double)q[17] / n * us, (double)q[16] * us);
  }
  double tt = (double)(q[8] + q[9] + q[10] + q[11]);
  fprintf(stderr, "[rtg] wave-time shares (s_memtime, instrumented variant): shade %.1f%% gen+pull|service %.1f%% box %.1f%% sphere %.1f%%; "
          "per pass: shade %.0f, gen|service %.0f, box %.0f, sphere %.0f ticks\n", 100 * q[8] / tt, 100 * q[9] / tt, 100 * q[10] / tt,
          100 * q[11] / tt, q[4] ? (double)q[8] / q[4] : 0., q[4] ? (double)q[9] / q[4] : 0., q[0] ? (double)q[10] / q[0] : 0.,
          q[2] ? (double)q[11] / q[2] : 0.);
  if (q[15]) {
    unsigned long long f[2];
    HIP_TRY(hipMemcpy(f, s->cx->d_counters + 5, sizeof(f), hipMemcpyDeviceToHost));
    fprintf(stderr, "[rtg] services %llu: finish step %.1f%% of wave time (%.0f ticks each), refill step %.1f%% (%.0f ticks per refill)\n", f[0],
            100 * f[1] / tt, f[0] ? (double)f[1] / f[0] : 0., 100 * q[15] / tt, q[6] ? (double)q[15] / q[6] : 0.);
  }
#ifdef RT_CENSUS
  {
    unsigned long long c[32];
    HIP_TRY(hipMemcpy(c, s->cx->d_counters + 32, sizeof(c), hipMemcpyDeviceToHost));
    static const char* nm[13] = {"BOX", "END", "no-ray", "held", "?", "?", "SPHERE", "RECT", "PUSH", "POP", "MEDIUM", "PRISM", "BEND"};
    for (int k = 0; k < 2; k++) {
      std::string line;
      char buf[64];
      for (int j = 0; j < 13; j++)
        if (c[16 * k + j]) snprintf(buf, sizeof buf, " %s %.1f", nm[j], (double)c[16 * k + j] / (double)c[16 * k + 15]), line += buf;
      fprintf(stderr, "[rtg] lane census at %s (%llu):%s\n", k ? "slow-pass iterations" : "box steps", c[16 * k + 15], line.c_str());
    }
  }
#endif
  fprintf(stderr, "[rtg] pool schedule: box steps %llu (avg %.1f lanes), sphere passes %llu (avg %.1f lanes), shade passes %llu "
            "(avg %.1f lanes), end / camera-ray passes %llu (avg %.1f lanes), refills %llu (avg %.1f lanes)\n", q[0], q[0] ? (double)q[1] / q[0] : 0.0, q[2],
            q[2] ? (double)q[3] / q[2] : 0.0, q[4], q[4] ? (double)q[5] / q[4] : 0.0, q[12], q[12] ? (double)q[13] / q[12] : 0.0, q[6],
            q[6] && q[7] ? (double)q[7] / q[6] : 0.0);
  return RTG_OK;
}

int rtg_par_cast_device(rtg_scene* s, const rtg_camera* camera, const rtg_params* params, float* d_out,
                        void* hip_stream, rtg_stats* stats) {
  DevParams d;
  int rc = check_params(s, camera, params, &d);
  if (rc) return rc;
  if (!d_out) return fail(RTG_ERR_INVALID, "null output");
  if (stats && stats->struct_size != sizeof(rtg_stats)) return fail(RTG_ERR_INVALID, "rtg_stats.struct_size mismatch");
  HIP_TRY(hipSetDevice(s->device));
  hipStream_t stream = (hipStream_t)hip_stream;
  if ((rc = ctx_acquire(s))) return rc;
  DevCamera cam = to_dev(camera);
  bool count = stats && (params->flags & RTG_FLAG_COUNTERS);
  const SampleSlice sl = slice_of(params);
#define HIP_TRY_CTX(expr)                               \
  do {                                                  \
    hipError_t e_ = (expr);                             \
    if (e_ != hipSuccess) {                             \
      (void)hipStreamSynchronize(stream);               \
      return hip_fail(e_, #expr);                       \
    }                                                   \
  } while (0)
  if ((sl.denoise || sl.features) && !sl.counts) {
    if (sl.denoise) {
      const void* d_block = reinterpret_cast<const uint32_t*>(d_out) + denoise_block_word(d.nx, d.ny, false, false);
      HIP_TRY(hipMemcpyAsync(&s->cx->denoise_in, d_block, offsetof(rtg_denoise, filtered), hipMemcpyDeviceToHost, stream));
    }
    if (sl.features) HIP_TRY(read_features_block(d, d_out, stream, sl, &s->cx->features_in));
    HIP_TRY(hipStreamSynchronize(stream));
    if (sl.denoise)
      if (const char* why = denoise_refusal(s->cx->denoise_in, d.nranks)) return fail(RTG_ERR_INVALID, why);
    if (sl.features)
      if (const char* why = features_refusal(s->cx->features_in, sl.denoise)) return fail(RTG_ERR_INVALID, why);
  }
  if (count) {
    HIP_TRY_CTX(hipMemsetAsync(s->cx->d_counters, 0, 7 * sizeof(unsigned long long), stream));
    HIP_TRY_CTX(hipMemsetAsync(s->cx->d_counters + 8, 0, 24 * sizeof(unsigned long long), stream));
    HIP_TRY_CTX(hipMemsetAsync(s->cx->d_counters + 32, 0, 32 * sizeof(unsigned long long), stream));
  }
#ifdef RT_TIMELINE
  static uint32_t* d_tl = nullptr;
  const size_t tl_bytes = (size_t)1024 * 16 * 16 * sizeof(uint32_t);
  if (!count) {
    if (!d_tl) HIP_TRY_CTX(hipMalloc((void**)&d_tl, tl_bytes));
    HIP_TRY_CTX(hipMemsetAsync(d_tl, 0, tl_bytes, stream));
    static unsigned long long tl_ptr;
    tl_ptr = (unsigned long long)(uintptr_t)d_tl;
    HIP_TRY_CTX(hipMemcpyAsync(s->cx->d_counters + 31, &tl_ptr, sizeof(tl_ptr), hipMemcpyHostToDevice, stream));
  }
#endif
  if (stats) HIP_TRY_CTX(hipEventRecord(s->cx->ev0, stream));
  s->cx->refusal = nullptr;
  HIP_TRY_CTX(count ? launch_render<true>(s, cam, d, d_out, stream, sl) : launch_render<false>(s, cam, d, d_out, stream, sl));
  if ((rc = ctx_release(s, stream))) {
    (void)hipStreamSynchronize(stream);
    return rc;
  }
#undef HIP_TRY_CTX
  if (s->cx->refusal) return fail(RTG_ERR_INVALID, s->cx->refusal);
  if (stats) {
    HIP_TRY(hipEventRecord(s->cx->ev1, stream));
    HIP_TRY(hipEventSynchronize(s->cx->ev1));
    float ms = 0.f;
    HIP_TRY(hipEventElapsedTime(&ms, s->cx->ev0, s->cx->ev1));
#ifdef RT_TIMELINE
    if (!count && getenv("RTG_TIMELINE_OUT")) {
      std::vector<uint32_t> h_tl(tl_bytes / sizeof(uint32_t));
      HIP_TRY(hipMemcpy(h_tl.data(), d_tl, tl_bytes, hipMemcpyDeviceToHost));
      if (FILE* f = fopen(getenv("RTG_TIMELINE_OUT"), "wb")) {
        fwrite(&ms, sizeof(ms), 1, f);
        fwrite(h_tl.data(), 1, tl_bytes, f);
        fclose(f);
      }
    }
#endif
    stats->kernel_ms = ms;
    stats->samples = sl.counts ? s->cx->counts_samples : owned_pixels(d) * (d.ns - sl.begin);
    unsigned long long h[8] = {0, 0, 0, 0, 0, 0, 0, 0};
    if (count) HIP_TRY(hipMemcpy(h, s->cx->d_counters, sizeof(h), hipMemcpyDeviceToHost));
    stats->aabb_tests = h[0], stats->prim_tests = h[1], stats->shaded_hits = h[2], stats->rays = h[3], stats->draws = h[4];
    if (count && s->verbose && (rc = print_schedule_stats(s, ms))) return rc;
  }
  return RTG_OK;
}

struct FrameBlocks {
  rtg_retire retire{};
  rtg_denoise denoise{};
  rtg_features features{};
};
struct FrameLayout {
  size_t bytes = 0;
  size_t count_bytes = 0;
  size_t block_bytes = 0, dblock_bytes = 0, fblock_bytes = 0;
  size_t plane_bytes = 0, fplanes_bytes = 0;
  size_t in_bytes = 0;
  size_t frame_bytes = 0;
};
static FrameLayout frame_layout(uint32_t nx, uint32_t ny, const SampleSlice& sl) {
  FrameLayout L;
  const size_t n = (size_t)nx * ny;
  L.bytes = n * 3 * sizeof(float) * (sl.squares ? 2 : 1);
  L.count_bytes = sl.counts ? n * sizeof(uint32_t) : 0;
  L.block_bytes = sl.retire ? retire_block_word(nx, ny) * sizeof(float) : 0;
  L.dblock_bytes = sl.denoise ? denoise_block_word(nx, ny, sl.counts, sl.retire) * sizeof(float) : 0;
  L.fblock_bytes = sl.features ? features_block_word(nx, ny, sl) * sizeof(float) : 0;
  L.plane_bytes = n * 3 * sizeof(float), L.fplanes_bytes = n * 7 * sizeof(float);
  L.in_bytes = sl.denoise ? L.dblock_bytes + sizeof(rtg_denoise) + L.plane_bytes : sl.retire ? L.block_bytes + sizeof(rtg_retire) : L.bytes + L.count_bytes;
  L.frame_bytes = sl.features ? L.fblock_bytes + sizeof(rtg_features) + L.fplanes_bytes : L.in_bytes;
  return L;
}
static int check_blocks(const FrameLayout& L, const SampleSlice& sl, const float* out_rgb, uint32_t nranks, FrameBlocks* fb) {
  const char* base = reinterpret_cast<const char*>(out_rgb);
  if (sl.retire) {
    memcpy(&fb->retire, base + L.block_bytes, sizeof(rtg_retire));
    if (const char* why = retire_refusal(fb->retire, nranks)) return fail(RTG_ERR_INVALID, why);
  }
  if (sl.denoise) {
    memcpy(&fb->denoise, base + L.dblock_bytes, sizeof(rtg_denoise));
    if (const char* why = denoise_refusal(fb->denoise, nranks)) return fail(RTG_ERR_INVALID, why);
  }
  if (sl.features) {
    memcpy(&fb->features, base + L.fblock_bytes, sizeof(rtg_features));
    if (const char* why = features_refusal(fb->features, sl.denoise)) return fail(RTG_ERR_INVALID, why);
  }
  return RTG_OK;
}
struct Extents {
  struct { size_t lo, hi; } e[4];
  int n = 0;
  void add(size_t lo, size_t hi) {
    if (hi > lo) e[n].lo = lo, e[n].hi = hi, n++;
  }
};
static Extents upload_extents(const FrameLayout& L, const SampleSlice& sl, bool other_ranks, uint32_t features_compute) {
  Extents x;
  if (other_ranks || sl.begin != 0u || sl.counts) x.add(0, L.in_bytes);
  else if (sl.denoise) x.add(L.dblock_bytes, L.dblock_bytes + sizeof(rtg_denoise));
  if (sl.features) x.add(L.fblock_bytes, L.fblock_bytes + sizeof(rtg_features) + (other_ranks || (features_compute == 0u && sl.denoise) ? L.fplanes_bytes : 0));
  return x;
}
static Extents copy_back_extents(const FrameLayout& L, const SampleSlice& sl, uint32_t features_compute) {
  Extents x;
  x.add(0, sl.retire ? L.bytes + L.count_bytes : L.bytes);
  if (sl.retire) x.add(L.block_bytes + offsetof(rtg_retire, active), L.block_bytes + offsetof(rtg_retire, reserved2));
  if (sl.denoise) x.add(L.dblock_bytes + offsetof(rtg_denoise, filtered), L.in_bytes);
  if (sl.features) x.add(L.fblock_bytes + offsetof(rtg_features, traced), L.fblock_bytes + sizeof(rtg_features) + (features_compute ? L.fplanes_bytes : 0));
  return x;
}

int rtg_par_cast(rtg_scene* s, const rtg_camera* camera, const rtg_params* params, float* out_rgb, rtg_stats* stats) {
  if (!s || !params || !out_rgb) return fail(RTG_ERR_INVALID, "null argument");
  {
    DevParams d;
    const int rc0 = check_params(s, camera, params, &d);
    if (rc0) return rc0;
  }
  const SampleSlice sl = slice_of(params);
  const FrameLayout L = frame_layout(params->nx, params->ny, sl);
  FrameBlocks fb;
  if (int rc0 = check_blocks(L, sl, out_rgb, params->nranks ? params->nranks : 1u, &fb)) return rc0;
  HIP_TRY(hipSetDevice(s->device));
  hipError_t e = grow((void**)&s->d_frame, &s->frame_bytes, L.frame_bytes ? L.frame_bytes : 16);
  if (e != hipSuccess) return hip_fail(e, "hipMalloc(framebuffer)");
  float* d_out = s->d_frame;
  char* dev = reinterpret_cast<char*>(d_out);
  char* host = reinterpret_cast<char*>(out_rgb);
  const Extents up = upload_extents(L, sl, params->nranks > 1, fb.features.compute);
  for (int i = 0; i < up.n && e == hipSuccess; i++) e = hipMemcpy(dev + up.e[i].lo, host + up.e[i].lo, up.e[i].hi - up.e[i].lo, hipMemcpyHostToDevice);
  int rc = (e == hipSuccess) ? rtg_par_cast_device(s, camera, params, d_out, nullptr, stats) : hip_fail(e, "hipMemcpy");
  if (rc == RTG_OK) {
    e = hipDeviceSynchronize();
    const Extents back = copy_back_extents(L, sl, fb.features.compute);
    for (int i = 0; i < back.n && e == hipSuccess; i++) e = hipMemcpy(host + back.e[i].lo, dev + back.e[i].lo, back.e[i].hi - back.e[i].lo, hipMemcpyDeviceToHost);
    if (e != hipSuccess) rc = hip_fail(e, "render / copy back");
  }
  return rc;
}

#include "rtg_multi.inc"

#include "rtg_probes.inc"

}
```

rtiow-rust_amd/csrc/rtg_launch.inc:

```
static uint64_t scratch_cap(int n_ctx) {
  size_t free_b = 0, total_b = 0;
  if (hipMemGetInfo(&free_b, &total_b) != hipSuccess) return (16ull << 30) / (uint64_t)std::max(1, n_ctx);
  return (uint64_t)free_b / 2 / (uint64_t)std::max(1, n_ctx);
}

static uint32_t samples_per_pass(const rtg_scene* s, uint64_t pix_work, uint32_t ns) {
  const uint64_t per_sample = pix_work * 3 * sizeof(float);
  uint64_t budget = s->scratch_limit ? s->scratch_limit : std::max<uint64_t>(scratch_cap(s->n_ctx), s->cx->scratch_bytes);
  if (s->whole_scratch) budget = ~0ull;
  uint64_t k = std::max<uint64_t>(1, budget / std::max<uint64_t>(per_sample, 1));
  k = std::min<uint64_t>(k, 0xfffffffeull / std::max<uint64_t>(pix_work, 1));
  k = std::max<uint64_t>(1, std::min<uint64_t>(k, ns));
  const uint64_t n_pass = (ns + k - 1) / k;
  return (uint32_t)((ns + n_pass - 1) / n_pass);
}

static uint64_t rank_pix_work(const DevParams& d) {
  const uint32_t tiles_x = (d.nx + d.tile_w - 1) / d.tile_w, tiles_y = (d.ny + d.tile_h - 1) / d.tile_h, tiles = tiles_x * tiles_y;
  const uint32_t owned = tiles > d.rank ? (tiles - d.rank + d.nranks - 1) / d.nranks : 0;
  return ((uint64_t)owned * d.tile_w * d.tile_h + 255u) & ~255ull;
}
static uint64_t owned_pixels(const DevParams& d) {
  uint64_t px = 0;
  uint32_t tiles_x = (d.nx + d.tile_w - 1) / d.tile_w, tiles_y = (d.ny + d.tile_h - 1) / d.tile_h;
  for (uint32_t ty = 0; ty < tiles_y; ty++)
    for (uint32_t tx = 0; tx < tiles_x; tx++) {
      if ((ty * tiles_x + tx) % d.nranks != d.rank) continue;
      uint32_t w = std::min(d.tile_w, d.nx - tx * d.tile_w), h = std::min(d.tile_h, d.ny - ty * d.tile_h);
      px += (uint64_t)w * h;
    }
  return px;
}

static hipError_t grow(void** buf, size_t* have, size_t need) {
  if (need <= *have) return hipSuccess;
  if (*buf) (void)hipFree(*buf);
  *buf = nullptr, *have = 0;
  hipError_t e = hipMalloc(buf, need);
  if (e == hipSuccess) *have = need;
  return e;
}

static hipError_t setup_lpt(rtg_scene* s, ChunkMode& cm, uint64_t capacity);
static void launch_pass_setup(rtg_scene* s, const LaunchConsts& c, uint32_t* queue, hipStream_t stream);

static hipError_t kernel_setup(rtg_scene* s, const void* kernel, int bt, size_t lds, int* per_cu) {
  static std::mutex mu;
  static std::map<std::pair<int, const void*>, size_t> raised;
  static std::map<std::tuple<int, const void*, int, size_t>, int> occupancy;
  std::lock_guard<std::mutex> lock(mu);
  size_t& have = raised[std::make_pair(s->device, kernel)];
  if (have < lds) {
    static std::map<int, int> device_cap;
    int& cap = device_cap[s->device];
    if (cap == 0 && (hipDeviceGetAttribute(&cap, hipDeviceAttributeMaxSharedMemoryPerBlock, s->device) != hipSuccess || cap <= 0)) cap = 64 * 1024;
    const int want = std::min(160 * 1024, std::max(cap, (int)std::min<size_t>(lds, 160 * 1024)));
    hipError_t e = hipFuncSetAttribute(kernel, hipFuncAttributeMaxDynamicSharedMemorySize, want);
    if (e == hipSuccess) {
      have = (size_t)want;
    } else {
      (void)hipGetLastError();
      e = hipFuncSetAttribute(kernel, hipFuncAttributeMaxDynamicSharedMemorySize, (int)lds);
      if (e != hipSuccess) return e;
      have = lds;
    }
  }
  const auto key = std::make_tuple(s->device, kernel, bt, lds);
  auto it = occupancy.find(key);
  if (it == occupancy.end()) {
    int n = 0;
    hipError_t e = hipOccupancyMaxActiveBlocksPerMultiprocessor(&n, kernel, bt, lds);
    if (e != hipSuccess) return e;
    it = occupancy.emplace(key, n).first;
  }
  *per_cu = s->wg_per_cu > 0 ? s->wg_per_cu : std::max(1, it->second);
  return hipSuccess;
}

struct PoolGeometry { int bt; uint32_t grid, work_block; };
static PoolGeometry pool_geometry(const rtg_scene* s, uint64_t total_work, int bt_max, int forced_bt, uint32_t pool, bool shrink_mid) {
  PoolGeometry g;
  g.bt = forced_bt > 0 && forced_bt <= bt_max ? forced_bt : bt_max;
  g.work_block = WORK_BLOCK;
  const uint64_t lanes_worth = (total_work + 63) / 64;
  const uint64_t cus = (uint64_t)std::max(1, s->num_cus);
  if (s->small_frames && lanes_worth < cus * (uint64_t)(bt_max / 64)) {
    if (forced_bt <= 0) g.bt = 64 * (int)std::min<uint64_t>((uint64_t)(bt_max / 64), (lanes_worth + cus - 1) / cus);
    g.work_block = 64;
    g.grid = (uint32_t)std::max<uint64_t>(1, (lanes_worth + (uint64_t)(g.bt / 64) - 1) / (uint64_t)(g.bt / 64));
    return g;
  }
  const uint64_t waves = (uint64_t)(g.bt / 64);
  uint64_t want = (total_work + waves * pool - 1) / (waves * pool);
  g.grid = (uint32_t)std::min<uint64_t>(want ? want : 1, 0xffffffffull);
  if (s->small_frames && shrink_mid && total_work < std::min<uint64_t>(g.grid, cus) * waves * WORK_BLOCK * 4) g.work_block = 64;
  return g;
}

struct PoolLaunch {
  KernelKind kind;
  int bt, per_cu;
  size_t lds;
  PoolGeometry geo;
  uint32_t pool;
};

template <typename Chunks, typename Issue>
static hipError_t sample_passes(rtg_scene* s, const DevParams& d, float* d_out, hipStream_t stream, const SampleSlice& sl,
                                const PoolLaunch& L, uint32_t per_pass, Chunks chunks, Issue issue) {
  for (uint32_t s0 = sl.begin; s0 < d.ns; s0 += per_pass) {
    DevParams dp = d;
    dp.ns = std::min(d.ns, s0 + per_pass);
    ChunkMode cm = chunks(s0, dp.ns);
    cm.work_block = L.geo.work_block;
    const uint64_t total_work = (uint64_t)cm.pix_work * cm.n_chunks;
    if (total_work > 0xfffffffeull) return hipErrorInvalidValue;
    const uint32_t grid = (uint32_t)std::min<uint64_t>(L.geo.grid, (uint64_t)s->num_cus * L.per_cu);
    hipError_t e = setup_lpt(s, cm, (uint64_t)grid * (uint32_t)(L.bt / 64) * L.pool);
    if (e != hipSuccess) return e;
    if (cm.lpt) cm.work_block = WORK_BLOCK;
    e = issue(s0, dp, cm, grid, (uint32_t)total_work);
    if (e == hipSuccess) e = hipGetLastError();
    if (e != hipSuccess) return e;
    if (cm.scratch && sl.counts) {
      void (*fold)(DevParams, ChunkMode, PixMap, float*, ListConsts) = sl.squares ? fold_samples_list_kernel<true> : fold_samples_list_kernel<false>;
      hipLaunchKernelGGL(fold, dim3((uint32_t)(((uint64_t)cm.pix_work + 255) / 256)), dim3(256), 0, stream, dp, cm, make_pixmap(dp), d_out, sl.list);
      e = hipGetLastError();
      if (e != hipSuccess) return e;
    } else if (cm.scratch) {
      void (*fold)(DevParams, ChunkMode, PixMap, float*, uint32_t) = sl.squares ? fold_samples_sq_kernel : fold_samples_kernel;
      hipLaunchKernelGGL(fold, dim3((uint32_t)(((uint64_t)cm.pix_work + 255) / 256)), dim3(256), 0, stream, dp, cm, make_pixmap(dp), d_out,
                         sl.divide ? d.ns : 0u);
      e = hipGetLastError();
      if (e != hipSuccess) return e;
    }
  }
  return hipSuccess;
}

template <bool COUNT>
static hipError_t launch_pool(rtg_scene* s, const DevCamera& cam, const DevParams& d, float* d_out,
                              hipStream_t stream, const SampleSlice& sl) {
  const uint64_t pix_work = sl.counts ? sl.list_work : rank_pix_work(d);
  if (pix_work == 0) return hipSuccess;
  if (pix_work > 0xfffffffeull) return hipErrorInvalidValue;
  const uint32_t ns_call = d.ns - sl.begin;
  uint64_t n_chunks = ns_call;
  if (s->force_chunks > 0) n_chunks = (uint64_t)s->force_chunks;
  if (n_chunks > ns_call) n_chunks = ns_call;
  const bool use_scratch = n_chunks > 1 || sl.sliced() || sl.squares || sl.counts;
  uint32_t per_pass = d.ns, chunk = d.ns;
  if (use_scratch) {
    per_pass = samples_per_pass(s, pix_work, ns_call);
    chunk = (uint32_t)((ns_call + n_chunks - 1) / n_chunks);
    if (per_pass < ns_call || sl.begin % chunk != 0u || sl.squares || sl.counts) chunk = 1u;
    hipError_t ea = grow((void**)&s->cx->d_scratch, &s->cx->scratch_bytes, pix_work * per_pass * 3 * sizeof(float));
    if (ea != hipSuccess) return ea;
  }
  s->cx->last_pix_work = use_scratch && per_pass == d.ns ? (uint32_t)pix_work : 0u;
  uint32_t* queue = (uint32_t*)(s->cx->d_counters + 7);
  const uint64_t work0 = pix_work * (use_scratch ? (std::min(ns_call, per_pass) + chunk - 1) / chunk : 1u);
  const PoolGeometry geo = pool_geometry(s, work0, RT_POOL_MAX_THREADS, s->pool_threads, POOL, true);
  const int bt = geo.bt;
  const uint32_t waves = (uint32_t)bt / 64;
  const size_t lds_limit = 160 * 1024;
  const bool wide = s->bvh4 && s->wide_bytes != 0 && !sl.counts;
  const bool chains = !COUNT && !wide && s->box_chains && s->d_chain_off != nullptr;
  const bool prune = !wide && s->box_prune && (!COUNT || s->box_prune == 2) && s->d_prune_off[s->box_chains ? 1 : 0] != nullptr;
  DevScene dev = s->dev;
  if (wide) dev.lds_off = (const uint32_t*)s->buffers[7], dev.lds_image_bytes = s->wide_bytes;
  if (chains) dev.lds_off = s->d_chain_off, dev.lds_image_bytes = s->chain_bytes;
  if (prune) dev.lds_off = s->d_prune_off[s->box_chains ? 1 : 0], dev.lds_image_bytes = s->prune_bytes[s->box_chains ? 1 : 0];
  const uint32_t image = dev.lds_image_bytes;
  bool use_lds = image != 0 && pool_lds_bytes(image, s->n_mat, waves, true, false) <= lds_limit;
  if (wide && !use_lds) return hipErrorNotSupported;
  bool ray_lds = s->ray_lds && pool_lds_bytes(image, s->n_mat, waves, use_lds, true) <= lds_limit && (!use_lds || image < (1u << 17));
  size_t lds = pool_lds_bytes(image, s->n_mat, waves, use_lds, ray_lds);
  if (s->verbose && s->ray_lds && !ray_lds && use_lds && image >= (1u << 17) && pool_lds_bytes(image, s->n_mat, waves, use_lds, true) <= lds_limit)
    fprintf(stderr, "[rtg] pool: the LDS image is %u B (>= 128 KB): the slots' hot fields stay in global memory although they would fit LDS (their 16-bit best_pc holds image offsets / 8 < 2^14)\n", image);
  void (*kernel)(DevScene, const LaunchConsts*, float*, uint32_t, uint32_t*, unsigned long long*, PoolTuning, uint32_t*);
  if (sl.counts) {
    if (ray_lds) kernel = use_lds ? render_lean_pool<true, COUNT, true, false, true> : render_lean_pool<false, COUNT, true, false, true>;
    else kernel = use_lds ? render_lean_pool<true, COUNT, false, false, true> : render_lean_pool<false, COUNT, false, false, true>;
  } else if (wide) kernel = ray_lds ? render_lean_pool<true, COUNT, true, true> : render_lean_pool<true, COUNT, false, true>;
  else if (ray_lds) kernel = use_lds ? render_lean_pool<true, COUNT, true> : render_lean_pool<false, COUNT, true>;
  else kernel = use_lds ? render_lean_pool<true, COUNT, false> : render_lean_pool<false, COUNT, false>;
  if (s->verbose && (chains || prune) && use_lds)
    fprintf(stderr, "[rtg] pool: box chains: %u follower record(s)%s, box pruning: %u interior record(s)%s (plan %.2f ms): LDS image %u B, %u records of %u; without followers %u B, full image %u B\n",
            s->n_followers, s->box_chains ? " dropped" : " kept", s->n_pruned, prune ? " dropped" : " kept", s->plan_ms, image,
            s->n_prog - (s->box_chains ? s->n_followers : 0u) - (prune ? s->n_pruned : 0u), s->n_prog, s->chain_bytes ? s->chain_bytes : s->dev.lds_image_bytes, s->dev.lds_image_bytes);
  PoolLaunch L{KernelKind::lean_pool, bt, 0, lds, geo, POOL};
  hipError_t e = kernel_setup(s, (const void*)kernel, bt, lds, &L.per_cu);
  if (e != hipSuccess) return e;
  auto chunks = [&](uint32_t s0, uint32_t end) {
    ChunkMode cm{};
    cm.scratch = nullptr, cm.chunk = d.ns, cm.n_chunks = 1, cm.pix_work = (uint32_t)pix_work, cm.s_begin = s0;
    if (use_scratch) {
      cm.chunk = chunk;
      cm.n_chunks = (end - s0 + chunk - 1) / chunk;
      cm.scratch = s->cx->d_scratch - 3ull * s0 * pix_work;
    }
    return cm;
  };
  auto issue = [&](uint32_t s0, const DevParams& dp, const ChunkMode& cm, uint32_t grid, uint32_t total_work) {
    if (s->verbose)
      fprintf(stderr, "[rtg] pool: samples [%u, %u) of %u: grid %u x %d threads, %d WG/CU, lds %zu B (program staged: %d, hot slot fields in LDS: %d), %u chunk(s) of %u samples, cost-ordered queue after %u chunk(s)\n",
              s0, dp.ns, d.ns, grid, bt, L.per_cu, lds, (int)use_lds, (int)ray_lds, cm.n_chunks, cm.chunk, (cm.lpt_samples - (cm.lpt_samples ? s0 : 0u)) / (cm.chunk ? cm.chunk : 1u));
    hipError_t eg = grow((void**)&s->cx->d_slots, &s->cx->slots_bytes, (size_t)grid * waves * POOL * POOL_FIELDS * sizeof(uint32_t));
    if (eg != hipSuccess) return eg;
    launch_pass_setup(s, LaunchConsts{cam, dp, cm, make_pixmap(dp)}, queue, stream);
    hipLaunchKernelGGL(kernel, dim3(grid), dim3(bt), lds, stream, dev, (const LaunchConsts*)s->cx->d_consts, d_out, total_work, queue,
                       s->cx->d_counters, s->pool_tune, s->cx->d_slots);
    return hipSuccess;
  };
  return sample_passes(s, d, d_out, stream, sl, L, per_pass, chunks, issue);
}

static bool build_wide_image(const Packet* lo, const Packet* hi, size_t n, std::vector<uint32_t>& out) {
  struct T { uint32_t box; int left, right; uint32_t sphere; };
  std::vector<T> nodes;
  auto op_of = [&](size_t i) { return hi[i].w[3] & 0xffu; };
  if (n < 4 || op_of(n - 1) != OP_END || op_of(0) != OP_BOX || hi[0].w[2] != n - 1) return false;
  bool ok = true;
  std::function<int(size_t, size_t&)> parse = [&](size_t i, size_t& end) -> int {
    if (i >= n || op_of(i) != OP_BOX) { ok = false; end = i + 1; return -1; }
    end = hi[i].w[2];
    const int id = (int)nodes.size();
    nodes.push_back(T{(uint32_t)i, -1, -1, 0});
    if (op_of(i + 1) == OP_SPHERE) {
      if (end != i + 2) ok = false;
      nodes[id].sphere = (uint32_t)(i + 1);
      return id;
    }
    size_t e1 = 0, e2 = 0;
    const int l = parse(i + 1, e1);
    if (!ok || e1 >= end) { ok = false; return id; }
    const int r = parse(e1, e2);
    if (e2 != end) ok = false;
    nodes[id].left = l, nodes[id].right = r;
    return id;
  };
  size_t end0 = 0;
  const int root = parse(0, end0);
  if (!ok || root < 0 || nodes[root].left < 0) return false;
  out.clear();
  auto alloc = [&](uint32_t bytes) { const uint32_t at = (uint32_t)out.size() * 4u; out.resize(out.size() + bytes / 4u, 0u); return at; };
  std::function<uint32_t(int, uint32_t, uint32_t)> emit = [&](int t, uint32_t parent, uint32_t level) -> uint32_t {
    if (level > 7u) { ok = false; return 0; }
    const uint32_t at = alloc(WIDE_NODE_BYTES);
    int entry[4];
    uint32_t n_ch = 0;
    for (int x : {nodes[t].left, nodes[t].right}) {
      if (nodes[x].left < 0) entry[n_ch++] = x;
      else entry[n_ch++] = nodes[x].left, entry[n_ch++] = nodes[x].right;
    }
    uint32_t child[4] = {0, 0, 0, 0}, leafmask = 0;
    for (uint32_t k = 0; k < n_ch; k++) {
      const T e = nodes[entry[k]];
      const Packet bl = lo[e.box], bh = hi[e.box];
      uint32_t* b = out.data() + at / 4u + 4u + 12u * k;
      b[0] = bl.w[0], b[1] = bl.w[1], b[2] = bl.w[2], b[3] = bl.w[3], b[4] = bh.w[0], b[5] = bh.w[1];
      b[6] = bl.w[1], b[7] = bl.w[0], b[8] = bl.w[3], b[9] = bl.w[2], b[10] = bh.w[1], b[11] = bh.w[0];
      if (e.left < 0) {
        const uint32_t sp = alloc(WIDE_SPHERE_BYTES);
        uint32_t* r = out.data() + sp / 4u;
        r[0] = hi[e.sphere].w[2], r[1] = hi[e.sphere].w[3];
        r[2] = lo[e.sphere].w[0], r[3] = lo[e.sphere].w[1], r[4] = lo[e.sphere].w[2], r[5] = lo[e.sphere].w[3];
        r[6] = at, r[7] = 0u;
        child[k] = sp, leafmask |= 1u << k;
      } else {
        child[k] = emit(entry[k], at, level + 1u);
      }
    }
    uint32_t* h = out.data() + at / 4u;
    h[0] = parent, h[1] = LDS_BOX_BIT | OP_BOX | (level << 8) | (n_ch << 12) | (leafmask << 16);
    h[2] = (child[0] >> 3) | ((child[1] >> 3) << 16), h[3] = (child[2] >> 3) | ((child[3] >> 3) << 16);
    return at;
  };
  emit(root, WIDE_NO_PARENT, 0u);
  return ok && out.size() * 4u < 512u * 1024u;
}

static hipError_t setup_lpt(rtg_scene* s, ChunkMode& cm, uint64_t capacity) {
  cm.lpt = nullptr, cm.lpt_samples = 0, cm.lpt_deep = 0;
  const uint32_t n_blocks = cm.pix_work / LPT_BLOCK;
  if (!s->lpt || !cm.scratch || cm.n_chunks < 6 || n_blocks < 64 || n_blocks > 65536 || cm.pix_work % LPT_BLOCK) return hipSuccess;
  uint32_t phase1 = std::max<uint32_t>(std::min(8u, std::max(2u, cm.n_chunks / 8u)), (uint32_t)((2 * capacity + cm.pix_work - 1) / cm.pix_work));
  if (s->lpt_phase1 > 0) phase1 = (uint32_t)s->lpt_phase1;
  if (phase1 < 1 || phase1 > cm.n_chunks / 3) return hipSuccess;
  const size_t words = 16 + (size_t)n_blocks * (1 + LPT_CLASSES) + LPT_CTL;
  hipError_t e = grow((void**)&s->cx->d_lpt, &s->cx->lpt_bytes, words * sizeof(uint32_t));
  if (e != hipSuccess) return e;
  LptQueue q;
  memset(&q, 0, sizeof(q));
  static_assert(sizeof(LptQueue) <= 64, "descriptor slot");
  q.cost = s->cx->d_lpt + 16, q.ctl = q.cost + n_blocks, q.list = q.ctl + LPT_CTL;
  q.n_blocks = n_blocks, q.phase1 = phase1;
  q.phase2_base = phase1 * cm.pix_work;
  q.span = LPT_BLOCK * (cm.n_chunks - phase1);
  q.mode = (uint32_t)s->lpt, q.shift = (uint32_t)s->lpt_shift;
  s->cx->lpt_desc = q;
  cm.lpt = reinterpret_cast<const LptQueue*>(s->cx->d_lpt);
  cm.lpt_samples = cm.s_begin + phase1 * cm.chunk;
  cm.lpt_deep = (uint32_t)s->lpt_deep;
  return hipSuccess;
}

static void launch_pass_setup(rtg_scene* s, const LaunchConsts& c, uint32_t* queue, hipStream_t stream) {
  const bool lpt = c.cm.lpt != nullptr;
  const LptQueue q = lpt ? s->cx->lpt_desc : LptQueue{};
  hipLaunchKernelGGL(write_pass_setup, dim3(1), dim3(256), 0, stream, s->cx->d_consts, c, (unsigned long long*)queue,
                     lpt ? reinterpret_cast<LptQueue*>(s->cx->d_lpt) : (LptQueue*)nullptr, q, lpt ? q.n_blocks + LPT_CTL : 0u);
}

template <bool COUNT>
static hipError_t launch_full_pool(rtg_scene* s, const DevCamera& cam, const DevParams& d, float* d_out,
                                   hipStream_t stream, const SampleSlice& sl) {
  const uint64_t pix_work = sl.counts ? sl.list_work : rank_pix_work(d);
  if (pix_work == 0) return hipSuccess;
  if (pix_work > 0xfffffffeull) return hipErrorInvalidValue;
  const uint32_t ns_call = d.ns - sl.begin;
  const uint32_t per_pass = samples_per_pass(s, pix_work, ns_call);
  const bool tex = (s->features & FEAT_TEXTURE) != 0;
  const int bt_max = tex ? RT_FULL_TEX_THREADS : 1024;
  const PoolGeometry geo = pool_geometry(s, pix_work * std::min(ns_call, per_pass), bt_max, s->full_threads, FPOOL, false);
  const int bt = geo.bt;
  const uint32_t waves = (uint32_t)bt / 64;
  hipError_t e = grow((void**)&s->cx->d_scratch, &s->cx->scratch_bytes, pix_work * per_pass * 3 * sizeof(float));
  if (e != hipSuccess) return e;
  s->cx->last_pix_work = per_pass == d.ns ? (uint32_t)pix_work : 0u;
  uint32_t* queue = (uint32_t*)(s->cx->d_counters + 7);
  const size_t list_bytes = full_pool_lds_bytes(0, waves);
  const size_t budget = 160 * 1024;
  uint32_t window = s->n_prog;
  int prog = 1;
  if ((size_t)window * 32 + list_bytes > budget) window = (uint32_t)((budget - list_bytes) / 32), prog = 2;
  if (s->window >= 0) {
    window = std::min<uint32_t>(s->n_prog, (uint32_t)s->window);
    prog = window == 0 ? 0 : (window == s->n_prog ? 1 : 2);
  }
  const size_t mat_bytes = (size_t)s->n_mat * 32;
  const bool mats_in_lds = s->mat_lds > 0 && prog == 1 && full_pool_lds_bytes(window, waves) + mat_bytes <= budget;
  const size_t lds = full_pool_lds_bytes(window, waves) + (mats_in_lds ? mat_bytes : 0);
  void (*kernel)(DevScene, const LaunchConsts*, float*, uint32_t, uint32_t*, unsigned long long*, PoolTuning, uint32_t*, float*,
                 uint32_t);
  const bool genb = (s->features & FEAT_BOUNDARY) != 0;
  if (sl.counts && genb) {
    if (prog == 0) kernel = tex ? render_full_pool<0, true, COUNT, true, true> : render_full_pool<0, false, COUNT, true, true>;
    else if (prog == 1) kernel = tex ? render_full_pool<1, true, COUNT, true, true> : render_full_pool<1, false, COUNT, true, true>;
    else kernel = tex ? render_full_pool<2, true, COUNT, true, true> : render_full_pool<2, false, COUNT, true, true>;
  } else if (sl.counts) {
    if (prog == 0) kernel = tex ? render_full_pool<0, true, COUNT, false, true> : render_full_pool<0, false, COUNT, false, true>;
    else if (prog == 1) kernel = tex ? render_full_pool<1, true, COUNT, false, true> : render_full_pool<1, false, COUNT, false, true>;
    else kernel = tex ? render_full_pool<2, true, COUNT, false, true> : render_full_pool<2, false, COUNT, false, true>;
  } else if (genb) {
    if (prog == 0) kernel = tex ? render_full_pool<0, true, COUNT, true> : render_full_pool<0, false, COUNT, true>;
    else if (prog == 1) kernel = tex ? render_full_pool<1, true, COUNT, true> : render_full_pool<1, false, COUNT, true>;
    else kernel = tex ? render_full_pool<2, true, COUNT, true> : render_full_pool<2, false, COUNT, true>;
  } else if (prog == 0) kernel = tex ? render_full_pool<0, true, COUNT> : render_full_pool<0, false, COUNT>;
  else if (prog == 1) kernel = tex ? render_full_pool<1, true, COUNT> : render_full_pool<1, false, COUNT>;
  else kernel = tex ? render_full_pool<2, true, COUNT> : render_full_pool<2, false, COUNT>;
  const bool tiny_bvh = s->n_box <= 32u;
  const bool tiny_frame = pix_work * std::min(ns_call, per_pass) <= (uint64_t)std::max(1, s->num_cus) * 64u;
  const bool lock_step = (s->sync_full > 0 || (s->sync_full < 0 && (s->n_box == 0 || tiny_bvh || tiny_frame))) && prog == 1;
  const bool p2_size_ok = s->pool2 > 1 || pix_work * (uint64_t)ns_call >= (32ull << 20);
  const bool mats3 = s->mat_lds > 0 && pool2_lds_bytes(s->n_prog2, s->n_mat, waves) <= budget;
  const size_t lds3 = pool2_lds_bytes(s->n_prog2, mats3 ? s->n_mat : 0u, waves);
  const bool pool2 = s->pool2 > 0 && p2_size_ok && s->n_prog2 != 0 && !lock_step && !genb && lds3 <= budget;
  PoolLaunch L{KernelKind::full_pool, bt, 0, lds, geo, FPOOL};
  LaunchConsts consts{};
  consts.parent = s->d_parent;
  e = kernel_setup(s, (const void*)kernel, bt, lds, &L.per_cu);
  if (e != hipSuccess) return e;
  void (*sync_kernel)(DevScene, const LaunchConsts*, float*, uint32_t, uint32_t*, unsigned long long*, PoolTuning, float*, uint32_t) = nullptr;
  void (*pool2_kernel)(DevScene, const LaunchConsts*, float*, uint32_t, uint32_t*, unsigned long long*, Pool2Tuning, uint32_t*, const P2Table*) = nullptr;
  if (lock_step) {
    L.kind = KernelKind::lock_step;
    if (sl.counts && genb) sync_kernel = tex ? render_full_sync<1, true, COUNT, true, true> : render_full_sync<1, false, COUNT, true, true>;
    else if (sl.counts) sync_kernel = tex ? render_full_sync<1, true, COUNT, false, true> : render_full_sync<1, false, COUNT, false, true>;
    else if (genb) sync_kernel = tex ? render_full_sync<1, true, COUNT, true> : render_full_sync<1, false, COUNT, true>;
    else sync_kernel = tex ? render_full_sync<1, true, COUNT, false> : render_full_sync<1, false, COUNT, false>;
    L.lds = (size_t)window * 32;
    L.geo = pool_geometry(s, pix_work * std::min(ns_call, per_pass), bt_max, s->full_threads, 64u, false);
    if (L.geo.bt != bt) L.geo = geo;
    e = kernel_setup(s, (const void*)sync_kernel, bt, L.lds, &L.per_cu);
  } else if (pool2) {
    L.kind = KernelKind::pool2;
    if (sl.counts) pool2_kernel = tex ? render_full_pool2<true, COUNT, true> : render_full_pool2<false, COUNT, true>;
    else pool2_kernel = tex ? render_full_pool2<true, COUNT> : render_full_pool2<false, COUNT>;
    L.lds = lds3;
    const uint32_t tab = s->n_prog2 * 32u + DC_WORDS * 4u;
    consts.mat_lds = mats3 ? tab + P2_TABLE_BYTES : 0u;
    consts.p2_lists = tab + P2_TABLE_BYTES + (mats3 ? s->n_mat * 32u : 0u);
    e = kernel_setup(s, (const void*)pool2_kernel, bt, L.lds, &L.per_cu);
  } else {
    if (mats_in_lds) consts.mat_lds = (uint32_t)full_pool_lds_bytes(window, waves);
    if (s->hoist > 0 && s->seg_end > s->seg_first) consts.seg_first = s->seg_first * RSZ, consts.seg_end = s->seg_end * RSZ;
  }
  if (e != hipSuccess) return e;
  s->cx->last_kernel = L.kind;
  auto chunks = [&](uint32_t s0, uint32_t end) {
    ChunkMode cm{};
    cm.scratch = s->cx->d_scratch - 3ull * s0 * pix_work, cm.chunk = 1u, cm.n_chunks = end - s0, cm.pix_work = (uint32_t)pix_work, cm.s_begin = s0;
    cm.drain_share = (uint32_t)std::max(0, s->drain_share);
    return cm;
  };
  auto issue = [&](uint32_t s0, const DevParams& dp, const ChunkMode& cm, uint32_t grid, uint32_t total_work) {
    hipError_t eg = grow((void**)&s->cx->d_slots, &s->cx->slots_bytes, (size_t)grid * std::max(full_pool_wg_words(waves), pool2_slot_words(waves)) * sizeof(uint32_t));
    if (eg != hipSuccess) return eg;
    eg = grow((void**)&s->cx->d_stack, &s->cx->stack_bytes, (size_t)grid * waves * (genb ? 2 : 1) * MAX_XFORM_DEPTH * 6 * 64 * sizeof(float));
    if (eg != hipSuccess) return eg;
    const bool p2 = L.kind == KernelKind::pool2;
    if (s->verbose)
      fprintf(stderr, "[rtg] full pool%s: samples [%u, %u) of %u: grid %u x %d threads, %d WG/CU, lds %zu B (program window: %u of %u records), cost-ordered queue after %u chunk(s)\n",
              p2 ? " 2 (second program)" : "", s0, dp.ns, d.ns, grid, bt, L.per_cu, p2 ? lds3 : lds, p2 ? s->n_prog2 : window, p2 ? s->n_prog2 : s->n_prog,
              cm.lpt_samples - (cm.lpt_samples ? s0 : 0u));
    LaunchConsts c = consts;
    c.cam = cam, c.P = dp, c.cm = cm, c.pm = make_pixmap(dp);
    launch_pass_setup(s, c, queue, stream);
    if (L.kind == KernelKind::lock_step)
      hipLaunchKernelGGL(sync_kernel, dim3(grid), dim3(bt), L.lds, stream, s->dev, (const LaunchConsts*)s->cx->d_consts, d_out, total_work, queue,
                         s->cx->d_counters, s->sync_tune, s->cx->d_stack, window);
    else if (p2)
      hipLaunchKernelGGL(pool2_kernel, dim3(grid), dim3(bt), L.lds, stream, s->dev2, (const LaunchConsts*)s->cx->d_consts, d_out, total_work, queue,
                         s->cx->d_counters, s->pool2_tune, s->cx->d_slots, s->d_p2);
    else
      hipLaunchKernelGGL(kernel, dim3(grid), dim3(bt), L.lds, stream, s->dev, (const LaunchConsts*)s->cx->d_consts, d_out, total_work, queue,
                         s->cx->d_counters, s->full_tune, s->cx->d_slots, s->cx->d_stack, window);
    return hipSuccess;
  };
  return sample_passes(s, d, d_out, stream, sl, L, per_pass, chunks, issue);
}

static hipError_t launch_resolve(const DevParams& d, float* d_out, hipStream_t stream) {
  const uint64_t pix_work = rank_pix_work(d);
  if (pix_work == 0) return hipSuccess;
  if (pix_work > 0xfffffffeull) return hipErrorInvalidValue;
  hipLaunchKernelGGL(resolve_sum_kernel, dim3((uint32_t)((pix_work + 255) / 256)), dim3(256), 0, stream, d, make_pixmap(d), (uint32_t)pix_work, d_out);
  return hipGetLastError();
}

static hipError_t launch_resolve_counts(const DevParams& d, float* d_out, hipStream_t stream, const uint32_t* counts) {
  const uint64_t pix_work = rank_pix_work(d);
  if (pix_work == 0) return hipSuccess;
  if (pix_work > 0xfffffffeull) return hipErrorInvalidValue;
  hipLaunchKernelGGL(resolve_counts_kernel, dim3((uint32_t)(pix_work / 256u)), dim3(256), 0, stream, d, make_pixmap(d), (uint32_t)pix_work, d_out, counts);
  return hipGetLastError();
}

static hipError_t launch_retire(rtg_scene* s, const DevParams& d, float* d_out, hipStream_t stream, uint64_t pix_work, const rtg_retire& r) {
  const uint32_t n_blk = (uint32_t)(pix_work / 256u);
  const uint64_t plane = (uint64_t)d.nx * d.ny;
  RetireBufs b;
  b.pitch = (d.nx + 31u) / 32u + 1u;
  hipError_t e = grow(&s->cx->d_retire, &s->cx->retire_bytes, (size_t)n_blk * 28u + (size_t)d.ny * b.pitch * 4u);
  if (e != hipSuccess) return e;
  b.blk_se2 = reinterpret_cast<double*>(s->cx->d_retire);
  b.blk_held = reinterpret_cast<unsigned long long*>(b.blk_se2 + n_blk);
  b.blk_u32 = reinterpret_cast<uint32_t*>(b.blk_held + n_blk);
  b.okbits = b.blk_u32 + 3ull * n_blk;
  b.planes = d_out;
  b.counts = reinterpret_cast<uint32_t*>(d_out + 6ull * plane);
  b.block = reinterpret_cast<uint32_t*>(d_out) + retire_block_word(d.nx, d.ny);
  const RetireArgs a{r.target_se, d.ns, r.min_samples, r.radius};
  if (n_blk != 0u) {
    const PixMap pm = make_pixmap(d);
    hipLaunchKernelGGL(retire_mark_kernel, dim3(n_blk), dim3(256), 0, stream, d, pm, a, b);
    hipLaunchKernelGGL(retire_apply_kernel, dim3(n_blk), dim3(256), 0, stream, d, pm, a, b);
  }
  hipLaunchKernelGGL(retire_finish_kernel, dim3(1), dim3(256), 0, stream, n_blk, b);
  return hipGetLastError();
}

static hipError_t launch_denoise(rtg_scene* s, const DevParams& d, float* d_out, hipStream_t stream, const SampleSlice& sl, const rtg_denoise& in,
                                 const rtg_features* guide = nullptr) {
  const uint64_t n_pix = (uint64_t)d.nx * d.ny;
  const uint32_t n_blk = (uint32_t)((n_pix + 255u) / 256u);
  const size_t frec_at = (size_t)n_pix * 32u + (((size_t)n_blk * 8u + 15u) & ~(size_t)15u);
  hipError_t e = grow(&s->cx->d_denoise, &s->cx->denoise_bytes, frec_at + (guide ? (size_t)n_pix * 32u : 0u));
  if (e != hipSuccess) return e;
  uint32_t* words = reinterpret_cast<uint32_t*>(d_out);
  DenoiseBufs b;
  b.planes = d_out;
  b.counts = sl.counts ? words + 6ull * n_pix : nullptr;
  b.rec = reinterpret_cast<float4*>(s->cx->d_denoise);
  b.blk_u32 = reinterpret_cast<uint32_t*>(b.rec + 2ull * n_pix);
  b.block = words + denoise_block_word(d.nx, d.ny, sl.counts, sl.retire);
  b.outp = reinterpret_cast<float*>(b.block + 16);
  const DenoiseArgs a{in.k, in.radius, in.patch, d.ns};
  const int guided = !guide ? 0 : (s->guide_lds > 0 ? 2 : 1);
  void (*filter)(uint32_t, uint32_t, DenoiseArgs, DenoiseBufs, DenoiseGuide) =
      guided == 0 ? denoise_filter_kernel<0> : (guided == 1 ? denoise_filter_kernel<1> : denoise_filter_kernel<2>);
  const size_t lds = denoise_lds_bytes(in.radius, in.patch, guided == 2);
// ... 220 lines not shown
```

rtiow-rust_amd/csrc/rtg_probes.inc:

```
int rtg_debug_hit_top(rtg_scene* s, size_t n, const float* rays, uint64_t seed, float t_near, float* out,
                      uint32_t* out_material) {
  if (!s || !rays || !out || !out_material) return fail(RTG_ERR_INVALID, "null argument");
  HIP_TRY(hipSetDevice(s->device));
  DevBuf<float> d_rays, d_out;
  DevBuf<uint32_t> d_mat;
  HIP_TRY(d_rays.alloc(7 * n));
  HIP_TRY(d_out.alloc(8 * n));
  HIP_TRY(d_mat.alloc(n));
  HIP_TRY(hipMemcpy(d_rays.p, rays, 7 * n * sizeof(float), hipMemcpyHostToDevice));
  dim3 grid((uint32_t)((n + 63) / 64)), block(64);
  if (n) {
    if (s->features & FEAT_DEEP)
      hipLaunchKernelGGL((debug_hit_top_kernel<FEAT_ALL | FEAT_DEEP>), grid, block, 0, 0, s->dev, (uint32_t)n, d_rays.p, (uint32_t)seed,
                         (uint32_t)(seed >> 32), t_near, d_out.p, d_mat.p);
    else if (s->features == 0)
      hipLaunchKernelGGL((debug_hit_top_kernel<0u>), grid, block, 0, 0, s->dev, (uint32_t)n, d_rays.p, (uint32_t)seed,
                         (uint32_t)(seed >> 32), t_near, d_out.p, d_mat.p);
    else
      hipLaunchKernelGGL((debug_hit_top_kernel<FEAT_ALL>), grid, block, 0, 0, s->dev, (uint32_t)n, d_rays.p,
                         (uint32_t)seed, (uint32_t)(seed >> 32), t_near, d_out.p, d_mat.p);
  }
  HIP_TRY(hipGetLastError());
  HIP_TRY(hipDeviceSynchronize());
  HIP_TRY(hipMemcpy(out, d_out.p, 8 * n * sizeof(float), hipMemcpyDeviceToHost));
  HIP_TRY(hipMemcpy(out_material, d_mat.p, n * sizeof(uint32_t), hipMemcpyDeviceToHost));
  return RTG_OK;
}

int rtg_debug_samples(rtg_scene* s, const rtg_camera* camera, const rtg_params* params, size_t n, const uint32_t* xs,
                      const uint32_t* ys, const uint32_t* samples, float* out_rgb, uint32_t* out_info) {
  DevParams d;
  int rc = check_params(s, camera, params, &d);
  if (rc) return rc;
  if (!xs || !ys || !samples || !out_rgb || !out_info) return fail(RTG_ERR_INVALID, "null argument");
  if (params->flags & (RTG_FLAG_PARTIAL | RTG_FLAG_RESUME)) return fail(RTG_ERR_INVALID, "rtg_debug_samples renders whole frames: RTG_FLAG_PARTIAL / RTG_FLAG_RESUME are not accepted");
  if (params->flags & RTG_FLAG_SUM_SQUARES) return fail(RTG_ERR_INVALID, "rtg_debug_samples: RTG_FLAG_SUM_SQUARES is not accepted");
  if (params->flags & RTG_FLAG_SAMPLE_COUNTS) return fail(RTG_ERR_INVALID, "rtg_debug_samples: RTG_FLAG_SAMPLE_COUNTS is not accepted");
  if (params->flags & RTG_FLAG_RETIRE) return fail(RTG_ERR_INVALID, "rtg_debug_samples: RTG_FLAG_RETIRE is not accepted");
  if (params->flags & RTG_FLAG_DENOISE) return fail(RTG_ERR_INVALID, "rtg_debug_samples: RTG_FLAG_DENOISE is not accepted");
  if (params->flags & RTG_FLAG_FEATURES) return fail(RTG_ERR_INVALID, "rtg_debug_samples: RTG_FLAG_FEATURES is not accepted");
  HIP_TRY(hipSetDevice(s->device));
  if (params->flags & RTG_FLAG_TRACE_KERNEL) {
    const uint32_t tiles_x = (d.nx + d.tile_w - 1) / d.tile_w;
    const uint64_t pix_work = rank_pix_work(d);
    const size_t trace_waves = (size_t)s->num_cus * std::max(32, s->wg_per_cu > 0 ? s->wg_per_cu * 16 : 0);
    const size_t table = (size_t)4 * d.ns * pix_work, slots = trace_waves * std::max(std::max(FPOOL, POOL), P2POOL) * 3;
    DevBuf<uint32_t> d_trace;
    HIP_TRY(d_trace.alloc(table + slots));
    HIP_TRY(hipMemset(d_trace.p, 0, (table + slots) * sizeof(uint32_t)));
    if ((rc = ctx_acquire(s))) return rc;
    HIP_TRY(grow((void**)&s->d_frame, &s->frame_bytes, (size_t)d.nx * d.ny * 3 * sizeof(float)));
    HIP_TRY(hipMemset(s->cx->d_counters, 0, 32 * sizeof(unsigned long long)));
    const unsigned long long ptrs[2] = {(unsigned long long)(uintptr_t)d_trace.p, (unsigned long long)(uintptr_t)(d_trace.p + table)};
    HIP_TRY(hipMemcpy(s->cx->d_counters + 30, ptrs, sizeof(ptrs), hipMemcpyHostToDevice));
    const DevCamera cam = to_dev(camera);
    s->whole_scratch = true;
    hipError_t e = launch_render<true>(s, cam, d, s->d_frame, nullptr);
    s->whole_scratch = false;
    if (e == hipSuccess) e = hipDeviceSynchronize();
    (void)hipMemset(s->cx->d_counters + 30, 0, 2 * sizeof(unsigned long long));
    if (e != hipSuccess) return hip_fail(e, "trace launch");
    if (s->cx->last_kernel == KernelKind::baseline || s->cx->last_pix_work == 0)
      return fail(RTG_ERR_UNSUPPORTED, "this scene / frame runs on the baseline kernel (or without the per-sample scratch): nothing to trace");
    std::vector<uint32_t> h_trace(table);
    std::vector<float> h_col((size_t)3 * d.ns * pix_work);
    HIP_TRY(hipMemcpy(h_trace.data(), d_trace.p, table * sizeof(uint32_t), hipMemcpyDeviceToHost));
    HIP_TRY(hipMemcpy(h_col.data(), s->cx->d_scratch, h_col.size() * sizeof(float), hipMemcpyDeviceToHost));
    for (size_t i = 0; i < n; i++) {
      const uint32_t x = xs[i], row = d.ny - 1u - ys[i], sm = samples[i];
      const uint32_t tx = x / d.tile_w, ty = row / d.tile_h, tile = ty * tiles_x + tx;
      if (x >= d.nx || ys[i] >= d.ny || sm >= d.ns || tile % d.nranks != d.rank) return fail(RTG_ERR_INVALID, "trace key outside this rank's frame");
      const uint32_t k = tile / d.nranks, lx = x - tx * d.tile_w, ly = row - ty * d.tile_h;
      const uint32_t b = (ly >> 3) * (d.tile_w >> 3) + (lx >> 3);
      const size_t w = (size_t)k * d.tile_w * d.tile_h + b * 64u + (ly & 7u) * 8u + (lx & 7u);
      const size_t at = (size_t)sm * pix_work + w;
      for (int c = 0; c < 3; c++) out_rgb[3 * i + c] = h_col[3 * at + c];
      for (int c = 0; c < 4; c++) out_info[4 * i + c] = h_trace[4 * at + c];
    }
    return RTG_OK;
  }
  DevBuf<uint32_t> dx, dy, ds, dinfo;
  DevBuf<float> drgb;
  HIP_TRY(dx.alloc(n));
  HIP_TRY(dy.alloc(n));
  HIP_TRY(ds.alloc(n));
  HIP_TRY(dinfo.alloc(4 * n));
  HIP_TRY(drgb.alloc(3 * n));
  HIP_TRY(hipMemcpy(dx.p, xs, n * 4, hipMemcpyHostToDevice));
  HIP_TRY(hipMemcpy(dy.p, ys, n * 4, hipMemcpyHostToDevice));
  HIP_TRY(hipMemcpy(ds.p, samples, n * 4, hipMemcpyHostToDevice));
  DevCamera cam = to_dev(camera);
  dim3 grid((uint32_t)((n + 63) / 64)), block(64);
  if (n) {
    if (s->features & FEAT_DEEP)
      hipLaunchKernelGGL((debug_samples_kernel<FEAT_ALL | FEAT_DEEP>), grid, block, 0, 0, s->dev, cam, d, (uint32_t)n, dx.p, dy.p, ds.p,
                         drgb.p, dinfo.p);
    else if (s->features == 0)
      hipLaunchKernelGGL((debug_samples_kernel<0u>), grid, block, 0, 0, s->dev, cam, d, (uint32_t)n, dx.p, dy.p, ds.p,
                         drgb.p, dinfo.p);
    else
      hipLaunchKernelGGL((debug_samples_kernel<FEAT_ALL>), grid, block, 0, 0, s->dev, cam, d, (uint32_t)n, dx.p, dy.p,
                         ds.p, drgb.p, dinfo.p);
  }
  HIP_TRY(hipGetLastError());
  HIP_TRY(hipDeviceSynchronize());
  HIP_TRY(hipMemcpy(out_rgb, drgb.p, 3 * n * sizeof(float), hipMemcpyDeviceToHost));
  HIP_TRY(hipMemcpy(out_info, dinfo.p, 4 * n * sizeof(uint32_t), hipMemcpyDeviceToHost));
  return RTG_OK;
}

int rtg_tonemap_device(int device, size_t n, const float* d_rgb, uint8_t* d_out, void* hip_stream) {
  if (!d_rgb || !d_out) return fail(RTG_ERR_INVALID, "null argument");
  HIP_TRY(hipSetDevice(device));
  if (n) hipLaunchKernelGGL(tonemap_kernel, dim3((uint32_t)((n + 255) / 256)), dim3(256), 0, (hipStream_t)hip_stream, n, d_rgb, d_out);
  HIP_TRY(hipGetLastError());
  return RTG_OK;
}

int rtg_tonemap(int device, size_t n, const float* rgb, uint8_t* out) {
  if (!rgb || !out) return fail(RTG_ERR_INVALID, "null argument");
  int ndev = 0;
  if (hipGetDeviceCount(&ndev) != hipSuccess || device < 0 || device >= ndev) return fail(RTG_ERR_DEVICE, "no HIP device");
  HIP_TRY(hipSetDevice(device));
  DevBuf<float> di;
  DevBuf<uint8_t> dout;
  HIP_TRY(di.alloc(n));
  HIP_TRY(dout.alloc(n));
  HIP_TRY(hipMemcpy(di.p, rgb, n * sizeof(float), hipMemcpyHostToDevice));
  int rc = rtg_tonemap_device(device, n, di.p, dout.p, nullptr);
  if (rc) return rc;
  HIP_TRY(hipDeviceSynchronize());
  HIP_TRY(hipMemcpy(out, dout.p, n, hipMemcpyDeviceToHost));
  return RTG_OK;
}

int rtg_debug_flatten(rtg_builder* b, const rtg_id* world, size_t n, uint32_t* n_instructions, uint32_t* features,
                      uint32_t* words_out, size_t capacity) {
  if (!b || (!world && n)) return fail(RTG_ERR_INVALID, "null argument");
  FlatScene fs;
  try {
    b->sb.flatten(world, n, &fs);
  } catch (const BuildError& e) {
    return fail(e.code, e.msg);
  }
  if (n_instructions) *n_instructions = (uint32_t)fs.lo.size();
  if (features) *features = fs.features;
  if (words_out) {
    size_t m = fs.lo.size() < capacity ? fs.lo.size() : capacity;
    for (size_t i = 0; i < m; i++) {
      std::memcpy(words_out + 8 * i, fs.lo[i].w, 16);
      std::memcpy(words_out + 8 * i + 4, fs.hi[i].w, 16);
    }
  }
  return RTG_OK;
}

int rtg_debug_flatten_pool2(rtg_builder* b, const rtg_id* world, size_t n, uint32_t* n_instructions, uint32_t* table_out,
                            uint32_t* words_out, size_t capacity) {
  if (!b || (!world && n)) return fail(RTG_ERR_INVALID, "null argument");
  FlatScene fs;
  try {
    b->sb.flatten(world, n, &fs);
  } catch (const BuildError& e) {
    return fail(e.code, e.msg);
  }
  if (n_instructions) *n_instructions = (uint32_t)fs.lo2.size();
  static_assert(sizeof(P2Table) == 24 * sizeof(uint32_t), "rtg_debug_flatten_pool2: table_out holds 24 words");
  if (table_out) std::memcpy(table_out, &fs.p2, sizeof(P2Table));
  if (words_out) {
    size_t m = fs.lo2.size() < capacity ? fs.lo2.size() : capacity;
    for (size_t i = 0; i < m; i++) {
      std::memcpy(words_out + 8 * i, fs.lo2[i].w, 16);
      std::memcpy(words_out + 8 * i + 4, fs.hi2[i].w, 16);
    }
  }
  return RTG_OK;
}

int rtg_debug_box_plan(rtg_builder* b, const rtg_id* world, size_t n, const uint32_t* words, size_t n_records, uint8_t* mask_out,
                       size_t capacity) {
  std::vector<Packet> lo, hi;
  bool lean = true;
  if (words) {
    lo.resize(n_records), hi.resize(n_records);
    for (size_t i = 0; i < n_records; i++) {
      std::memcpy(lo[i].w, words + 8 * i, 16), std::memcpy(hi[i].w, words + 8 * i + 4, 16);
      const uint32_t op = hi[i].w[3] & 0xffu;
      lean = lean && (op == OP_BOX || op == OP_SPHERE || op == OP_END) && !(hi[i].w[3] & F_MOVE);
      if (op == OP_BOX && hi[i].w[2] >= n_records) return fail(RTG_ERR_INVALID, "rtg_debug_box_plan: a skip pointer leaves the program");
    }
  } else {
    if (!b || (!world && n)) return fail(RTG_ERR_INVALID, "null argument");
    FlatScene fs;
    try {
      b->sb.flatten(world, n, &fs);
    } catch (const BuildError& e) {
      return fail(e.code, e.msg);
    }
    lean = (fs.features & (FEAT_ALL | FEAT_BOUNDARY)) == 0;
    lo.swap(fs.lo), hi.swap(fs.hi);
  }
  if (hi.size() > 0x7fffffffu) return fail(RTG_ERR_INVALID, "rtg_debug_box_plan: program too large");
  std::vector<uint8_t> follower(hi.size(), 0), mask(hi.size(), 0);
  if (lean && !hi.empty()) {
    box_chain_followers(reinterpret_cast<const uint32_t (*)[4]>(lo.data()), reinterpret_cast<const uint32_t (*)[4]>(hi.data()), hi.size(), follower.data());
    box_plan(reinterpret_cast<const uint32_t (*)[4]>(lo.data()), reinterpret_cast<const uint32_t (*)[4]>(hi.data()), hi.size(), follower.data(), mask.data());
  }
  if (mask_out) std::memcpy(mask_out, mask.data(), std::min(mask.size(), capacity));
  return (int)hi.size();
}

int rtg_debug_math(int device, int op, size_t n, const float* in, const float* in2, float* out) {
  if (!in || !out || op < 0 || op > 5 || (op == 5 && !in2)) return fail(RTG_ERR_INVALID, "bad argument");
  int ndev = 0;
  if (hipGetDeviceCount(&ndev) != hipSuccess || device < 0 || device >= ndev) return fail(RTG_ERR_DEVICE, "no HIP device");
  HIP_TRY(hipSetDevice(device));
  DevBuf<float> di, di2, dout;
  HIP_TRY(di.alloc(n));
  HIP_TRY(di2.alloc(n));
  HIP_TRY(dout.alloc(n));
  HIP_TRY(hipMemcpy(di.p, in, n * sizeof(float), hipMemcpyHostToDevice));
  if (in2) HIP_TRY(hipMemcpy(di2.p, in2, n * sizeof(float), hipMemcpyHostToDevice));
  if (n) hipLaunchKernelGGL(debug_math_kernel, dim3((uint32_t)((n + 255) / 256)), dim3(256), 0, 0, op, n, di.p, di2.p, dout.p);
  HIP_TRY(hipGetLastError());
  HIP_TRY(hipDeviceSynchronize());
  HIP_TRY(hipMemcpy(out, dout.p, n * sizeof(float), hipMemcpyDeviceToHost));
  return RTG_OK;
}
```

Before: 7293.

## Rebuild prunable BVH regions with SAH splits and area-based box pruning plan

Adds a host-side rebuild of prunable BVH subtrees: it recomputes leaf-box regions with a sweep SAH split and writes a new program image. It also adds an area-weighted planning mode for the box-pruning DP, which replaces random probe rays and now uses flat arrays. The launcher picks the rebuilt image when the box_tree option is set and the LDS image fits, and otherwise falls back to the reference image. The aim is to cut box tests per ray, at the cost of extra build time and a second set of device images.

Result: faster. 7768 (median of 6 runs) (+6.5%).

```diff
diff --git a/include/rtiow_gpu_debug.h b/include/rtiow_gpu_debug.h
--- a/include/rtiow_gpu_debug.h
+++ b/include/rtiow_gpu_debug.h
@@ -8,6 +8,9 @@
 int rtg_debug_box_plan(rtg_builder* b, const rtg_id* world, size_t n, const uint32_t* words, size_t n_records,
                        uint8_t* mask_out, size_t capacity);
 
+int rtg_debug_production_program(rtg_builder* b, const rtg_id* world, size_t n, const uint32_t* words, size_t n_records,
+                                 uint32_t* words_out, uint32_t* origin_out, uint8_t* mask_out, size_t capacity);
+
 #ifdef __cplusplus
 }
 #endif
diff --git a/rtiow-rust_amd/capi.py b/rtiow-rust_amd/capi.py
--- a/rtiow-rust_amd/capi.py
+++ b/rtiow-rust_amd/capi.py
@@ -528,6 +528,7 @@
         f("debug_flatten_pool2", C.c_int, [C.c_void_p, c_u32p, C.c_size_t, c_u32p, c_u32p, c_u32p, C.c_size_t])
         f("tonemap_device", C.c_int, [C.c_int, C.c_size_t, C.c_void_p, C.c_void_p, C.c_void_p])
         f("debug_box_plan", C.c_int, [C.c_void_p, c_u32p, C.c_size_t, c_u32p, C.c_size_t, c_u8p, C.c_size_t])
+        f("debug_production_program", C.c_int, [C.c_void_p, c_u32p, C.c_size_t, c_u32p, C.c_size_t, c_u32p, c_u32p, c_u8p, C.c_size_t])
 
     def _fn(self, name, restype, argtypes):
         try:
@@ -739,6 +740,25 @@
             self.be.check(n)
         return mask
 
+    def production_program(self, world=None, words=None):
+        if words is not None:
+            words = np.ascontiguousarray(words, dtype=np.uint32)
+            head = (None, None, 0, words.ctypes.data_as(c_u32p), len(words))
+            n = len(words)
+        else:
+            arr = (C.c_uint32 * max(1, len(world)))(*world)
+            head = (self.h, arr, len(world), None, 0)
+            n = self.be._debug_production_program(*head, None, None, None, 0)
+            if n < 0:
+                self.be.check(n)
+        out = np.zeros((n, 8), dtype=np.uint32)
+        origin = np.zeros(n, dtype=np.uint32)
+        mask = np.zeros(n, dtype=np.uint8)
+        n = self.be._debug_production_program(*head, out.ctypes.data_as(c_u32p), origin.ctypes.data_as(c_u32p), mask.ctypes.data_as(c_u8p), n)
+        if n < 0:
+            self.be.check(n)
+        return out, origin, mask
+
     def bvh_sah(self, objs, exposure=(0.0, 1.0)):
         arr = (C.c_uint32 * max(1, len(objs)))(*objs)
         return self.be.check_id(self.be._object_bvh_sah(self.h, arr, len(objs), exposure[0], exposure[1]))
@@ -770,7 +790,7 @@
             pass
 
     ENV_OPTIONS = ("kernel", "chunks", "lpt", "lpt_phase1", "lpt_deep", "lpt_shift", "ray_lds", "sync", "block", "wg_per_cu", "window",
-                   "box_leave", "refill_min", "gather_min", "run_ahead", "run_ahead_min", "sphere_min", "verbose", "bvh4", "box_chains", "box_prune", "force_rccl", "multi_gather", "multi_planes", "scratch_mb", "frames_in_flight", "small_frames", "drain_share", "hoist", "deep_sized", "mat_lds", "pool2", "p2_refill", "p2_box_leave", "p2_park", "p2_sphere", "p2_prism", "p2_list", "p2_push")
+                   "box_leave", "refill_min", "gather_min", "run_ahead", "run_ahead_min", "sphere_min", "verbose", "bvh4", "box_chains", "box_prune", "box_tree", "force_rccl", "multi_gather", "multi_planes", "scratch_mb", "frames_in_flight", "small_frames", "drain_share", "hoist", "deep_sized", "mat_lds", "pool2", "p2_refill", "p2_box_leave", "p2_park", "p2_sphere", "p2_prism", "p2_list", "p2_push")
 
     def set_option(self, name, value):
         self.be.check(self.be._scene_set_option(self.h, name.encode(), int(value)))
diff --git a/rtiow-rust_amd/csrc/rt_box_plan.h b/rtiow-rust_amd/csrc/rt_box_plan.h
--- a/rtiow-rust_amd/csrc/rt_box_plan.h
+++ b/rtiow-rust_amd/csrc/rt_box_plan.h
@@ -18,6 +18,12 @@
 #endif
 constexpr uint32_t BOX_PLAN_PROBES = RT_BOX_PLAN_PROBES;
 constexpr bool BOX_PLAN_FULL = RT_BOX_PLAN_FULL != 0;
+enum BoxPlanKind : int { BOX_PLAN_SURE = 0, BOX_PLAN_PROBE_DP = 1, BOX_PLAN_AREA = 2 };
+constexpr BoxPlanKind BOX_PLAN_DEFAULT = BOX_PLAN_FULL ? BOX_PLAN_PROBE_DP : BOX_PLAN_SURE;
+#ifndef RT_BOX_TREE_PLAN
+#define RT_BOX_TREE_PLAN 2
+#endif
+constexpr BoxPlanKind BOX_TREE_PLAN = (BoxPlanKind)(RT_BOX_TREE_PLAN);
 
 struct BoxPlan {
   uint32_t n_pruned = 0;
@@ -74,51 +80,69 @@
     } while (v[0] * v[0] + v[1] * v[1] + v[2] * v[2] >= 1.f);
   }
 };
-}
-
-inline BoxPlan box_plan(const uint32_t (*lo)[4], const uint32_t (*hi)[4], size_t n, const uint8_t* follower, uint8_t* mask,
-                        uint8_t* sure = nullptr, uint32_t n_probes = BOX_PLAN_PROBES) {
-  using namespace box_plan_detail;
-  BoxPlan out;
-  for (size_t j = 0; j < n; j++) {
-    mask[j] = follower && follower[j] ? BOX_FOLLOWER : BOX_KEPT;
-    if (sure) sure[j] = 0;
-  }
+inline bool finite6(const uint32_t* lo, const uint32_t* hi) {
+  return std::isfinite(as_f(lo[0])) && std::isfinite(as_f(lo[1])) && std::isfinite(as_f(lo[2])) && std::isfinite(as_f(lo[3])) &&
+         std::isfinite(as_f(hi[0])) && std::isfinite(as_f(hi[1]));
+}
+inline double box_area(const uint32_t* lo, const uint32_t* hi) {
+  const double dx = (double)as_f(lo[1]) - (double)as_f(lo[0]), dy = (double)as_f(lo[3]) - (double)as_f(lo[2]),
+               dz = (double)as_f(hi[1]) - (double)as_f(hi[0]);
+  return 2.0 * (dx * dy + dy * dz + dz * dx);
+}
+struct Shape {
+  std::vector<int32_t> parent;
+  std::vector<uint32_t> depth;
+  std::vector<uint8_t> prunable;
+  uint32_t n_prunable = 0;
+};
+inline bool leaf_box_at(const uint32_t (*hi)[4], size_t n, size_t j) {
+  return (hi[j][3] & 0xffu) == OP_BOX && j + 2 < n && (hi[j + 1][3] & 0xffu) == OP_SPHERE && hi[j][2] == j + 2;
+}
+inline bool program_shape(const uint32_t (*lo)[4], const uint32_t (*hi)[4], size_t n, Shape* sh) {
   auto op = [&](size_t j) { return hi[j][3] & 0xffu; };
   auto skip = [&](size_t j) { return (size_t)hi[j][2]; };
-  if (n < 4 || n > 0x7fffffffu) return out;
-  std::vector<int32_t> parent(n, -1);
-  std::vector<uint32_t> depth(n, 0);
-  {
-    std::vector<uint32_t> open;
-    for (size_t j = 0; j < n; j++) {
-      while (!open.empty() && skip(open.back()) <= j) open.pop_back();
-      if (!open.empty()) parent[j] = (int32_t)open.back(), depth[j] = (uint32_t)open.size();
-      if (op(j) != OP_BOX) continue;
-      if (skip(j) <= j || skip(j) >= n || (!open.empty() && skip(j) > skip(open.back()))) return out;
-      open.push_back((uint32_t)j);
-    }
-  }
-  auto leaf_box = [&](size_t j) { return op(j) == OP_BOX && j + 2 < n && op(j + 1) == OP_SPHERE && skip(j) == j + 2; };
-  auto finite6 = [&](size_t j) {
-    return std::isfinite(as_f(lo[j][0])) && std::isfinite(as_f(lo[j][1])) && std::isfinite(as_f(lo[j][2])) &&
-           std::isfinite(as_f(lo[j][3])) && std::isfinite(as_f(hi[j][0])) && std::isfinite(as_f(hi[j][1]));
-  };
+  sh->parent.assign(n, -1), sh->depth.assign(n, 0), sh->prunable.assign(n, 0), sh->n_prunable = 0;
+  if (n < 4 || n > 0x7fffffffu) return false;
+  std::vector<uint32_t> open;
+  for (size_t j = 0; j < n; j++) {
+    while (!open.empty() && skip(open.back()) <= j) open.pop_back();
+    if (!open.empty()) sh->parent[j] = (int32_t)open.back(), sh->depth[j] = (uint32_t)open.size();
+    if (op(j) != OP_BOX) continue;
+    if (skip(j) <= j || skip(j) >= n || (!open.empty() && skip(j) > skip(open.back()))) return false;
+    open.push_back((uint32_t)j);
+  }
   auto contains = [&](size_t j, size_t c) {
     return as_f(lo[j][0]) <= as_f(lo[c][0]) && as_f(lo[j][1]) >= as_f(lo[c][1]) && as_f(lo[j][2]) <= as_f(lo[c][2]) &&
            as_f(lo[j][3]) >= as_f(lo[c][3]) && as_f(hi[j][0]) <= as_f(hi[c][0]) && as_f(hi[j][1]) >= as_f(hi[c][1]);
   };
-  std::vector<uint8_t> prunable(n, 0);
-  uint32_t n_prunable = 0;
   for (size_t j = n; j-- > 0;) {
     if (op(j) != OP_BOX || j + 1 >= n || op(j + 1) != OP_BOX) continue;
     const size_t L = j + 1, R = skip(L);
     if (!(L < R && R < skip(j)) || op(R) != OP_BOX || skip(R) != skip(j)) continue;
-    if (!finite6(j) || !finite6(L) || !finite6(R) || !contains(j, L) || !contains(j, R)) continue;
-    if (!(leaf_box(L) || prunable[L]) || !(leaf_box(R) || prunable[R])) continue;
-    prunable[j] = 1, n_prunable++;
-  }
-  if (!n_prunable) return out;
+    if (!finite6(lo[j], hi[j]) || !finite6(lo[L], hi[L]) || !finite6(lo[R], hi[R]) || !contains(j, L) || !contains(j, R)) continue;
+    if (!(leaf_box_at(hi, n, L) || sh->prunable[L]) || !(leaf_box_at(hi, n, R) || sh->prunable[R])) continue;
+    sh->prunable[j] = 1, sh->n_prunable++;
+  }
+  return true;
+}
+}
+
+inline BoxPlan box_plan(const uint32_t (*lo)[4], const uint32_t (*hi)[4], size_t n, const uint8_t* follower, uint8_t* mask,
+                        uint8_t* sure = nullptr, uint32_t n_probes = BOX_PLAN_PROBES, BoxPlanKind kind = BOX_PLAN_DEFAULT) {
+  using namespace box_plan_detail;
+  BoxPlan out;
+  for (size_t j = 0; j < n; j++) {
+    mask[j] = follower && follower[j] ? BOX_FOLLOWER : BOX_KEPT;
+    if (sure) sure[j] = 0;
+  }
+  auto op = [&](size_t j) { return hi[j][3] & 0xffu; };
+  auto skip = [&](size_t j) { return (size_t)hi[j][2]; };
+  Shape shape;
+  if (!program_shape(lo, hi, n, &shape) || !shape.n_prunable) return out;
+  const std::vector<int32_t>& parent = shape.parent;
+  const std::vector<uint32_t>& depth = shape.depth;
+  const std::vector<uint8_t>& prunable = shape.prunable;
+  auto leaf_box = [&](size_t j) { return leaf_box_at(hi, n, j); };
   std::vector<uint8_t> choosable(prunable);
   for (size_t j = 0; j + 1 < n; j++) {
     if (!prunable[j] || !follower) continue;
@@ -155,7 +179,7 @@
     if (!all && std::isfinite(r) && std::isfinite(cj[0]) && std::isfinite(cj[1]) && std::isfinite(cj[2])) starts.push_back(j);
   }
   uint64_t n_rays = 0;
-  if (!starts.empty()) {
+  if (!starts.empty() && kind != BOX_PLAN_AREA) {
     Rng rng{0x626f78706c616e31ull ^ (uint64_t)n};
     const float t_near = 0.001f;
     while (n_rays < n_probes) {
@@ -195,35 +219,53 @@
     }
   }
   out.n_rays = (uint32_t)n_rays;
+  if (kind == BOX_PLAN_AREA) {
+    constexpr uint64_t ONE = 1ull << 30;
+    float rmin[3] = {INFINITY, INFINITY, INFINITY}, rmax[3] = {-INFINITY, -INFINITY, -INFINITY};
+    for (size_t j = 0; j + 1 < n; j++) {
+      if (!leaf_box(j) || enclosing[j + 1] || !finite6(lo[j], hi[j])) continue;
+      const float mn[3] = {as_f(lo[j][0]), as_f(lo[j][2]), as_f(hi[j][0])}, mx[3] = {as_f(lo[j][1]), as_f(lo[j][3]), as_f(hi[j][1])};
+      for (int a = 0; a < 3; a++) rmin[a] = fminf(rmin[a], mn[a]), rmax[a] = fmaxf(rmax[a], mx[a]);
+    }
+    const double dx = (double)rmax[0] - rmin[0], dy = (double)rmax[1] - rmin[1], dz = (double)rmax[2] - rmin[2];
+    const double sa_ref = 2.0 * (dx * dy + dy * dz + dz * dx);
+    if (!(sa_ref > 0.0) || !std::isfinite(sa_ref)) return out;
+    for (size_t j = 0; j < n; j++) {
+      if (op(j) != OP_BOX) continue;
+      const double r = finite6(lo[j], hi[j]) ? box_area(lo[j], hi[j]) / sa_ref : 1.0;
+      n_pass[j] = r >= 1.0 ? ONE : (r > 0.0 ? (uint64_t)(r * (double)ONE) : 0u);
+    }
+    n_rays = ONE;
+  }
 
   uint64_t states = 0;
-  for (size_t j = 0; BOX_PLAN_FULL && j < n; j++)
+  for (size_t j = 0; kind != BOX_PLAN_SURE && j < n; j++)
     if (op(j) == OP_BOX) states += depth[j] + 2u;
-  const bool dp = BOX_PLAN_FULL && states <= (1ull << 26);
+  const bool dp = kind != BOX_PLAN_SURE && states <= (1ull << 26);
   std::vector<uint32_t> kidx(n, 0);
   std::vector<uint8_t> pruned(n, 0);
   if (dp) {
-    std::vector<std::vector<uint64_t>> acc(n);
-    std::vector<std::vector<uint8_t>> choice(n);
-    std::vector<uint64_t> path_pass;
+    std::vector<uint64_t> at(n + 1, 0);
+    for (size_t j = 0; j < n; j++) at[j + 1] = at[j] + (op(j) == OP_BOX ? depth[j] + 2u : 0u);
+    std::vector<uint64_t> acc(at[n], 0);
+    std::vector<uint8_t> choice(at[n], 0);
+    std::vector<uint64_t> path_pass, f;
     for (size_t j = n; j-- > 0;) {
       if (op(j) != OP_BOX) continue;
       const uint32_t dj = depth[j];
-      if (acc[j].empty()) acc[j].assign(dj + 2u, 0);
+      uint64_t* acc_j = &acc[at[j]];
+      uint8_t* choice_j = &choice[at[j]];
       path_pass.assign(dj + 1u, n_rays);
       for (int32_t a = parent[j], k = (int32_t)dj; a >= 0; a = parent[a], k--) path_pass[k] = n_pass[a];
-      std::vector<uint64_t> f(dj + 1u);
-      choice[j].assign(dj + 1u, 0);
+      f.assign(dj + 1u, 0);
       for (uint32_t k = 0; k <= dj; k++) {
         const uint64_t own = follower && follower[j] ? 0u : path_pass[k];
-        const uint64_t keep = own + acc[j][dj + 1u], leave = acc[j][k];
-        if (choosable[j] && leave <= keep) f[k] = leave, choice[j][k] = 1;
+        const uint64_t keep = own + acc_j[dj + 1u], leave = acc_j[k];
+        if (choosable[j] && leave <= keep) f[k] = leave, choice_j[k] = 1;
         else f[k] = keep;
       }
-      std::vector<uint64_t>().swap(acc[j]);
       if (parent[j] >= 0) {
-        std::vector<uint64_t>& up = acc[parent[j]];
-        if (up.empty()) up.assign(dj + 1u, 0);
+        uint64_t* up = &acc[at[parent[j]]];
         for (uint32_t k = 0; k <= dj; k++) up[k] += f[k];
       }
     }
@@ -231,10 +273,10 @@
       if (op(j) != OP_BOX) continue;
       const int32_t p = parent[j];
       kidx[j] = p < 0 ? 0u : (pruned[p] ? kidx[p] : depth[j]);
-      pruned[j] = choice[j][kidx[j]];
+      pruned[j] = choice[at[j] + kidx[j]];
     }
   } else {
-    for (size_t j = 0; j < n; j++) pruned[j] = choosable[j] && n_rays && n_pass[j] == n_rays;
+    for (size_t j = 0; j < n; j++) pruned[j] = choosable[j] && n_rays && n_pass[j] == n_rays && op(j) == OP_BOX;
   }
   for (size_t j = 0; j < n; j++) {
     if (!pruned[j] || mask[j] == BOX_FOLLOWER) continue;
@@ -247,4 +289,96 @@
   return out;
 }
 
-}
+constexpr uint32_t BOX_TREE_NEW = 0xffffffffu;
+inline uint32_t box_tree_rebuild(const uint32_t (*lo)[4], const uint32_t (*hi)[4], size_t n, uint32_t (*out_lo)[4],
+                                 uint32_t (*out_hi)[4], uint32_t* origin) {
+  using namespace box_plan_detail;
+  for (size_t j = 0; j < n; j++) {
+    std::memcpy(out_lo[j], lo[j], 16), std::memcpy(out_hi[j], hi[j], 16);
+    origin[j] = (uint32_t)j;
+  }
+  Shape shape;
+  if (!program_shape(lo, hi, n, &shape) || !shape.n_prunable) return 0;
+  struct Box { float mn[3], mx[3]; };
+  auto merge = [](const Box& a, const Box& b) {
+    Box m;
+    for (int x = 0; x < 3; x++) m.mn[x] = b.mn[x] < a.mn[x] ? b.mn[x] : a.mn[x], m.mx[x] = b.mx[x] > a.mx[x] ? b.mx[x] : a.mx[x];
+    return m;
+  };
+  auto area = [](const Box& b) {
+    const double dx = (double)b.mx[0] - b.mn[0], dy = (double)b.mx[1] - b.mn[1], dz = (double)b.mx[2] - b.mn[2];
+    return 2.0 * (dx * dy + dy * dz + dz * dx);
+  };
+  std::vector<uint32_t> leaf;
+  std::vector<Box> box;
+  std::vector<double> suffix;
+  struct Job { uint32_t a, b, at; };
+  std::vector<Job> jobs;
+  std::vector<uint32_t> rec_lo, rec_hi, rec_origin;
+  uint32_t regions = 0;
+  for (size_t j = 0; j < n; j++) {
+    if (!shape.prunable[j]) continue;
+    const size_t end = hi[j][2];
+    if (shape.parent[j] >= 0 && shape.prunable[shape.parent[j]]) continue;
+    leaf.clear(), box.clear();
+    bool ok = true;
+    for (size_t i = j; i < end; i++) {
+      if (!leaf_box_at(hi, n, i)) continue;
+      ok = ok && finite6(lo[i], hi[i]);
+      leaf.push_back((uint32_t)i);
+      box.push_back(Box{{as_f(lo[i][0]), as_f(lo[i][2]), as_f(hi[i][0])}, {as_f(lo[i][1]), as_f(lo[i][3]), as_f(hi[i][1])}});
+    }
+    const size_t m = leaf.size();
+    if (!ok || m < 2 || 3 * m - 1 != end - j) { j = end - 1; continue; }
+    uint64_t budget = 64ull * m, work = 0;
+    for (size_t v = m; v > 1; v >>= 1) budget += 64ull * m;
+    const size_t len = end - j;
+    rec_lo.assign(4 * len, 0), rec_hi.assign(4 * len, 0), rec_origin.assign(len, BOX_TREE_NEW);
+    suffix.resize(m);
+    jobs.clear();
+    jobs.push_back(Job{0u, (uint32_t)m, 0u});
+    while (!jobs.empty() && ok) {
+      const Job t = jobs.back();
+      jobs.pop_back();
+      uint32_t* rl = &rec_lo[4 * t.at];
+      uint32_t* rh = &rec_hi[4 * t.at];
+      if (t.b - t.a == 1) {
+        const uint32_t src = leaf[t.a];
+        std::memcpy(rl, lo[src], 16), std::memcpy(rh, hi[src], 16), std::memcpy(rl + 4, lo[src + 1], 16), std::memcpy(rh + 4, hi[src + 1], 16);
+        rh[2] = (uint32_t)j + t.at + 2u;
+        rec_origin[t.at] = src, rec_origin[t.at + 1] = src + 1u;
+        continue;
+      }
+      work += 2ull * (t.b - t.a);
+      if (work > budget) { ok = false; break; }
+      Box run = box[t.b - 1];
+      for (uint32_t k = t.b - 1; k > t.a; k--) run = k == t.b - 1 ? run : merge(box[k], run), suffix[k] = area(run);
+      run = box[t.a];
+      uint32_t best_k = t.a + 1;
+      double best_cost = INFINITY;
+      for (uint32_t k = t.a + 1; k < t.b; k++) {
+        if (k > t.a + 1) run = merge(run, box[k - 1]);
+        const double cost = area(run) * (double)(k - t.a) + suffix[k] * (double)(t.b - k);
+        if (cost < best_cost) best_cost = cost, best_k = k;
+      }
+      const Box all = merge(run, box[t.b - 1]);
+      const float f[6] = {all.mn[0], all.mx[0], all.mn[1], all.mx[1], all.mn[2], all.mx[2]};
+      std::memcpy(rl, f, 16), std::memcpy(rh, f + 4, 8);
+      rh[2] = (uint32_t)j + t.at + 3u * (t.b - t.a) - 1u;
+      rh[3] = t.at == 0u ? hi[j][3] : (hi[j][3] & ~F_BVH_ROOT);
+      jobs.push_back(Job{best_k, t.b, t.at + 1u + 3u * (best_k - t.a) - 1u});
+      jobs.push_back(Job{t.a, best_k, t.at + 1u});
+    }
+    if (ok) {
+      for (size_t i = 0; i < len; i++) {
+        std::memcpy(out_lo[j + i], &rec_lo[4 * i], 16), std::memcpy(out_hi[j + i], &rec_hi[4 * i], 16);
+        origin[j + i] = rec_origin[i];
+      }
+      regions++;
+    }
+    j = end - 1;
+  }
+  return regions;
+}
+
+}
diff --git a/rtiow-rust_amd/csrc/rtg_api.hip b/rtiow-rust_amd/csrc/rtg_api.hip
--- a/rtiow-rust_amd/csrc/rtg_api.hip
+++ b/rtiow-rust_amd/csrc/rtg_api.hip
@@ -88,13 +88,32 @@
   rtg_features features_in{};
 };
 
+struct LeanImages {
+  const uint4* lo = nullptr;
+  const uint4* hi = nullptr;
+  const uint32_t* d_off = nullptr;
+  uint32_t bytes = 0;
+  uint32_t n_followers = 0;
+  const uint32_t* d_chain_off = nullptr;
+  uint32_t chain_bytes = 0;
+  bool planned = false;
+  uint32_t n_pruned = 0;
+  float plan_ms = 0.f;
+  const uint32_t* d_prune_off[2] = {nullptr, nullptr};
+  uint32_t prune_bytes[2] = {0, 0};
+  std::vector<uint32_t> plan_ops;
+  std::vector<uint8_t> plan_mask;
+  std::vector<uint8_t> follower;
+  int slot = 12;
+};
+
 struct rtg_scene {
   int device = 0;
   DevScene dev{};
   uint32_t features = 0;
   uint32_t n_prog = 0, n_mat = 0, n_tex = 0;
   uint64_t bytes = 0;
-  void* buffers[15] = {};
+  void* buffers[21] = {};
   const uint32_t* d_parent = nullptr;
   hipStream_t own_stream = nullptr;
   int num_cus = 0;
@@ -118,16 +137,15 @@
   int bvh4 = 0;
   uint32_t wide_bytes = 0;
   int box_chains = 1;
-  uint32_t n_followers = 0;
-  const uint32_t* d_chain_off = nullptr;
-  uint32_t chain_bytes = 0;
   int box_prune = 1;
-  uint32_t n_pruned = 0;
-  float plan_ms = 0.f;
-  const uint32_t* d_prune_off[2] = {nullptr, nullptr};
-  uint32_t prune_bytes[2] = {0, 0};
-  std::vector<uint32_t> plan_ops;
-  std::vector<uint8_t> plan_mask;
+  int box_tree = 1;
+  LeanImages ref;
+  LeanImages tree;
+  bool tree_tried = false;
+  float tree_ms = 0.f;
+  uint32_t n_regions = 0;
+  bool plannable = false;
+  std::vector<Packet> h_lo, h_hi;
   int sync_full = -1;
   uint32_t n_box = 0;
   int lpt = 2;
@@ -505,16 +523,65 @@
   return RTG_OK;
 }
 
-static int prune_table(rtg_scene* s, int chains) {
-  if (s->d_prune_off[chains] || !s->n_pruned) return RTG_OK;
-  const size_t n = s->plan_mask.size();
+static int prune_table(rtg_scene* s, LeanImages* im, int chains) {
+  if (im->d_prune_off[chains] || !im->n_pruned) return RTG_OK;
+  const size_t n = im->plan_mask.size();
   std::vector<uint8_t> drop(n);
   std::vector<uint32_t> off(n);
-  for (size_t i = 0; i < n; i++) drop[i] = s->plan_mask[i] == BOX_PRUNED || (chains && s->plan_mask[i] == BOX_FOLLOWER);
-  s->prune_bytes[chains] = lds_image_offsets(s->plan_ops.data(), n, off.data(), drop.data());
-  int rc = upload(&s->buffers[13 + chains], off.data(), n * sizeof(uint32_t), &s->bytes);
+  for (size_t i = 0; i < n; i++) drop[i] = im->plan_mask[i] == BOX_PRUNED || (chains && im->plan_mask[i] == BOX_FOLLOWER);
+  im->prune_bytes[chains] = lds_image_offsets(im->plan_ops.data(), n, off.data(), drop.data());
+  int rc = upload(&s->buffers[im->slot + 1 + chains], off.data(), n * sizeof(uint32_t), &s->bytes);
   if (rc) return rc;
-  s->d_prune_off[chains] = (const uint32_t*)s->buffers[13 + chains];
+  im->d_prune_off[chains] = (const uint32_t*)s->buffers[im->slot + 1 + chains];
+  return RTG_OK;
+}
+
+static int lean_images(rtg_scene* s, LeanImages* im, const std::vector<Packet>& lo, const std::vector<Packet>& hi, int off_slot) {
+  std::vector<uint32_t> off(hi.size());
+  im->plan_ops.resize(hi.size());
+  for (size_t i = 0; i < hi.size(); i++) im->plan_ops[i] = hi[i].w[3];
+  im->bytes = lds_image_offsets(im->plan_ops.data(), hi.size(), off.data());
+  int rc = upload(&s->buffers[off_slot], off.data(), off.size() * sizeof(uint32_t), &s->bytes);
+  if (rc) return rc;
+  im->d_off = (const uint32_t*)s->buffers[off_slot];
+  im->follower.resize(hi.size());
+  im->n_followers = box_chain_followers(reinterpret_cast<const uint32_t (*)[4]>(lo.data()), reinterpret_cast<const uint32_t (*)[4]>(hi.data()), hi.size(), im->follower.data());
+  if (im->n_followers) {
+    im->chain_bytes = lds_image_offsets(im->plan_ops.data(), hi.size(), off.data(), im->follower.data());
+    if ((rc = upload(&s->buffers[im->slot], off.data(), off.size() * sizeof(uint32_t), &s->bytes))) return rc;
+    im->d_chain_off = (const uint32_t*)s->buffers[im->slot];
+  }
+  return RTG_OK;
+}
+
+static int lean_plan(rtg_scene* s, LeanImages* im, const std::vector<Packet>& lo, const std::vector<Packet>& hi, BoxPlanKind kind) {
+  if (im->planned || !s->plannable) return RTG_OK;
+  im->planned = true;
+  im->plan_mask.resize(hi.size());
+  const auto t0 = std::chrono::steady_clock::now();
+  im->n_pruned = box_plan(reinterpret_cast<const uint32_t (*)[4]>(lo.data()), reinterpret_cast<const uint32_t (*)[4]>(hi.data()), hi.size(), im->follower.data(), im->plan_mask.data(), nullptr, BOX_PLAN_PROBES, kind).n_pruned;
+  im->plan_ms = std::chrono::duration<float, std::milli>(std::chrono::steady_clock::now() - t0).count();
+  return prune_table(s, im, 1);
+}
+static int ref_plan(rtg_scene* s) { return lean_plan(s, &s->ref, s->h_lo, s->h_hi, BOX_PLAN_DEFAULT); }
+
+static int tree_program(rtg_scene* s) {
+  if (s->tree_tried || !s->plannable) return RTG_OK;
+  s->tree_tried = true;
+  const size_t n = s->h_hi.size();
+  std::vector<Packet> lo(n), hi(n);
+  std::vector<uint32_t> origin(n);
+  const auto t0 = std::chrono::steady_clock::now();
+  s->n_regions = box_tree_rebuild(reinterpret_cast<const uint32_t (*)[4]>(s->h_lo.data()), reinterpret_cast<const uint32_t (*)[4]>(s->h_hi.data()), n,
+                                  reinterpret_cast<uint32_t (*)[4]>(lo.data()), reinterpret_cast<uint32_t (*)[4]>(hi.data()), origin.data());
+  s->tree_ms = std::chrono::duration<float, std::milli>(std::chrono::steady_clock::now() - t0).count();
+  if (!s->n_regions) return RTG_OK;
+  int rc;
+  if ((rc = upload(&s->buffers[15], lo.data(), n * 16, &s->bytes)) || (rc = upload(&s->buffers[16], hi.data(), n * 16, &s->bytes))) return rc;
+  s->tree.slot = 18;
+  if ((rc = lean_images(s, &s->tree, lo, hi, 17)) || (rc = lean_plan(s, &s->tree, lo, hi, BOX_TREE_PLAN))) return rc;
+  if (!s->box_chains && (rc = prune_table(s, &s->tree, 0))) return rc;
+  s->tree.lo = (const uint4*)s->buffers[15], s->tree.hi = (const uint4*)s->buffers[16];
   return RTG_OK;
 }
 
@@ -611,35 +678,18 @@
     for (const Packet& h : fs.hi2) s->n_box2 += (h.w[3] & 0xffu) == OP_BOX ? 1u : 0u;
   }
   if ((fs.features & (FEAT_ALL | FEAT_BOUNDARY)) == 0) {
-    std::vector<uint32_t> ops(fs.hi.size()), off(fs.hi.size());
-    for (size_t i = 0; i < fs.hi.size(); i++) ops[i] = fs.hi[i].w[3];
-    s->dev.lds_image_bytes = lds_image_offsets(ops.data(), ops.size(), off.data());
-    if ((rc = upload(&s->buffers[6], off.data(), off.size() * sizeof(uint32_t), &s->bytes))) {
+    s->ref.lo = s->dev.lo, s->ref.hi = s->dev.hi, s->ref.slot = 12;
+    if ((rc = lean_images(s, &s->ref, fs.lo, fs.hi, 6))) {
       rtg_scene_destroy(s);
       return rc;
     }
-    s->dev.lds_off = (const uint32_t*)s->buffers[6];
-    std::vector<uint8_t> follower(fs.hi.size());
-    s->n_followers = box_chain_followers(reinterpret_cast<const uint32_t (*)[4]>(fs.lo.data()), reinterpret_cast<const uint32_t (*)[4]>(fs.hi.data()), fs.hi.size(), follower.data());
-    if (s->n_followers) {
-      s->chain_bytes = lds_image_offsets(ops.data(), ops.size(), off.data(), follower.data());
-      if ((rc = upload(&s->buffers[12], off.data(), off.size() * sizeof(uint32_t), &s->bytes))) {
+    s->dev.lds_off = s->ref.d_off, s->dev.lds_image_bytes = s->ref.bytes;
+    s->plannable = s->dev.lds_image_bytes - LDS_BOX_BYTES * (s->n_box / 2u) <= 160u * 1024u;
+    if (s->plannable) {
+      s->h_lo = fs.lo, s->h_hi = fs.hi;
+      if ((s->box_tree && (rc = tree_program(s))) || (!s->tree.lo && (rc = ref_plan(s)))) {
         rtg_scene_destroy(s);
         return rc;
-      }
-      s->d_chain_off = (const uint32_t*)s->buffers[12];
-    }
-    if (s->dev.lds_image_bytes - LDS_BOX_BYTES * (s->n_box / 2u) <= 160u * 1024u) {
-      s->plan_mask.resize(fs.hi.size());
-      const auto t0 = std::chrono::steady_clock::now();
-      s->n_pruned = box_plan(reinterpret_cast<const uint32_t (*)[4]>(fs.lo.data()), reinterpret_cast<const uint32_t (*)[4]>(fs.hi.data()), fs.hi.size(), follower.data(), s->plan_mask.data()).n_pruned;
-      s->plan_ms = std::chrono::duration<float, std::milli>(std::chrono::steady_clock::now() - t0).count();
-      if (s->n_pruned) {
-        s->plan_ops = ops;
-        if ((rc = prune_table(s, 1))) {
-          rtg_scene_destroy(s);
-          return rc;
-        }
       }
     }
     std::vector<uint32_t> wide;
@@ -679,10 +729,19 @@
   else if (k == "box_chains") {
     if (!value) {
       HIP_TRY(hipSetDevice(s->device));
-      int rc = prune_table(s, 0);
+      int rc = prune_table(s, &s->ref, 0);
+      if (!rc) rc = prune_table(s, &s->tree, 0);
       if (rc) return rc;
     }
     s->box_chains = value;
+  }
+  else if (k == "box_tree") {
+    if (value < 0 || value > 1) return fail(RTG_ERR_INVALID, "box_tree: 0 or 1");
+    HIP_TRY(hipSetDevice(s->device));
+    int rc = value ? tree_program(s) : ref_plan(s);
+    if (!rc && !s->box_chains) rc = prune_table(s, value ? &s->tree : &s->ref, 0);
+    if (rc) return rc;
+    s->box_tree = value;
   }
   else if (k == "box_prune") {
     if (value < 0 || value > 2) return fail(RTG_ERR_INVALID, "box_prune: 0 .. 2");
@@ -742,7 +801,7 @@
   if (n_materials) *n_materials = s->n_mat;
   if (n_textures) *n_textures = s->n_tex;
   if (hbm_bytes) *hbm_bytes = s->bytes;
-  if (n_box_followers) *n_box_followers = s->n_followers;
+  if (n_box_followers) *n_box_followers = s->ref.n_followers;
   return RTG_OK;
 }
 
diff --git a/rtiow-rust_amd/csrc/rtg_launch.inc b/rtiow-rust_amd/csrc/rtg_launch.inc
--- a/rtiow-rust_amd/csrc/rtg_launch.inc
+++ b/rtiow-rust_amd/csrc/rtg_launch.inc
@@ -165,12 +165,24 @@
   const uint32_t waves = (uint32_t)bt / 64;
   const size_t lds_limit = 160 * 1024;
   const bool wide = s->bvh4 && s->wide_bytes != 0 && !sl.counts;
-  const bool chains = !COUNT && !wide && s->box_chains && s->d_chain_off != nullptr;
-  const bool prune = !wide && s->box_prune && (!COUNT || s->box_prune == 2) && s->d_prune_off[s->box_chains ? 1 : 0] != nullptr;
+  const bool production = !COUNT || s->box_prune == 2;
   DevScene dev = s->dev;
+  bool chains = false, prune = false;
+  auto choose = [&](const LeanImages& im) {
+    chains = !COUNT && !wide && s->box_chains && im.d_chain_off != nullptr;
+    prune = !wide && s->box_prune && production && im.d_prune_off[s->box_chains ? 1 : 0] != nullptr;
+    dev.lo = im.lo, dev.hi = im.hi, dev.lds_off = im.d_off, dev.lds_image_bytes = im.bytes;
+    if (chains) dev.lds_off = im.d_chain_off, dev.lds_image_bytes = im.chain_bytes;
+    if (prune) dev.lds_off = im.d_prune_off[s->box_chains ? 1 : 0], dev.lds_image_bytes = im.prune_bytes[s->box_chains ? 1 : 0];
+  };
+  bool tree = s->box_tree && s->tree.lo != nullptr && production && !wide && s->ref.lo != nullptr;
+  if (tree) {
+    choose(s->tree);
+    if (pool_lds_bytes(dev.lds_image_bytes, s->n_mat, waves, true, false) > lds_limit) tree = false;
+  }
+  if (!tree && s->ref.lo != nullptr) choose(s->ref);
+  const LeanImages& im = tree ? s->tree : s->ref;
   if (wide) dev.lds_off = (const uint32_t*)s->buffers[7], dev.lds_image_bytes = s->wide_bytes;
-  if (chains) dev.lds_off = s->d_chain_off, dev.lds_image_bytes = s->chain_bytes;
-  if (prune) dev.lds_off = s->d_prune_off[s->box_chains ? 1 : 0], dev.lds_image_bytes = s->prune_bytes[s->box_chains ? 1 : 0];
   const uint32_t image = dev.lds_image_bytes;
   bool use_lds = image != 0 && pool_lds_bytes(image, s->n_mat, waves, true, false) <= lds_limit;
   if (wide && !use_lds) return hipErrorNotSupported;
@@ -186,9 +198,9 @@
   else if (ray_lds) kernel = use_lds ? render_lean_pool<true, COUNT, true> : render_lean_pool<false, COUNT, true>;
   else kernel = use_lds ? render_lean_pool<true, COUNT, false> : render_lean_pool<false, COUNT, false>;
   if (s->verbose && (chains || prune) && use_lds)
-    fprintf(stderr, "[rtg] pool: box chains: %u follower record(s)%s, box pruning: %u interior record(s)%s (plan %.2f ms): LDS image %u B, %u records of %u; without followers %u B, full image %u B\n",
-            s->n_followers, s->box_chains ? " dropped" : " kept", s->n_pruned, prune ? " dropped" : " kept", s->plan_ms, image,
-            s->n_prog - (s->box_chains ? s->n_followers : 0u) - (prune ? s->n_pruned : 0u), s->n_prog, s->chain_bytes ? s->chain_bytes : s->dev.lds_image_bytes, s->dev.lds_image_bytes);
+    fprintf(stderr, "[rtg] pool: %s program (%u region(s) rebuilt in %.2f ms), box chains: %u follower record(s)%s, box pruning: %u interior record(s)%s (plan %.2f ms): LDS image %u B, %u records of %u; without followers %u B, full image %u B\n",
+            tree ? "rebuilt" : "reference", s->n_regions, s->tree_ms, im.n_followers, chains || (prune && s->box_chains) ? " dropped" : " kept", im.n_pruned, prune ? " dropped" : " kept", im.plan_ms, image,
+            s->n_prog - (chains || (prune && s->box_chains) ? im.n_followers : 0u) - (prune ? im.n_pruned : 0u), s->n_prog, im.chain_bytes ? im.chain_bytes : im.bytes, im.bytes);
   PoolLaunch L{KernelKind::lean_pool, bt, 0, lds, geo, POOL};
   hipError_t e = kernel_setup(s, (const void*)kernel, bt, lds, &L.per_cu);
   if (e != hipSuccess) return e;
diff --git a/rtiow-rust_amd/csrc/rtg_probes.inc b/rtiow-rust_amd/csrc/rtg_probes.inc
--- a/rtiow-rust_amd/csrc/rtg_probes.inc
+++ b/rtiow-rust_amd/csrc/rtg_probes.inc
@@ -177,17 +177,16 @@
   return RTG_OK;
 }
 
-int rtg_debug_box_plan(rtg_builder* b, const rtg_id* world, size_t n, const uint32_t* words, size_t n_records, uint8_t* mask_out,
-                       size_t capacity) {
-  std::vector<Packet> lo, hi;
-  bool lean = true;
+static int debug_lean_program(const char* who, rtg_builder* b, const rtg_id* world, size_t n, const uint32_t* words, size_t n_records,
+                              std::vector<Packet>* lo, std::vector<Packet>* hi, bool* lean) {
+  *lean = true;
   if (words) {
-    lo.resize(n_records), hi.resize(n_records);
+    lo->resize(n_records), hi->resize(n_records);
     for (size_t i = 0; i < n_records; i++) {
-      std::memcpy(lo[i].w, words + 8 * i, 16), std::memcpy(hi[i].w, words + 8 * i + 4, 16);
-      const uint32_t op = hi[i].w[3] & 0xffu;
-      lean = lean && (op == OP_BOX || op == OP_SPHERE || op == OP_END) && !(hi[i].w[3] & F_MOVE);
-      if (op == OP_BOX && hi[i].w[2] >= n_records) return fail(RTG_ERR_INVALID, "rtg_debug_box_plan: a skip pointer leaves the program");
+      std::memcpy((*lo)[i].w, words + 8 * i, 16), std::memcpy((*hi)[i].w, words + 8 * i + 4, 16);
+      const uint32_t op = (*hi)[i].w[3] & 0xffu;
+      *lean = *lean && (op == OP_BOX || op == OP_SPHERE || op == OP_END) && !((*hi)[i].w[3] & F_MOVE);
+      if (op == OP_BOX && (*hi)[i].w[2] >= n_records) return fail(RTG_ERR_INVALID, std::string(who) + ": a skip pointer leaves the program");
     }
   } else {
     if (!b || (!world && n)) return fail(RTG_ERR_INVALID, "null argument");
@@ -197,10 +196,19 @@
     } catch (const BuildError& e) {
       return fail(e.code, e.msg);
     }
-    lean = (fs.features & (FEAT_ALL | FEAT_BOUNDARY)) == 0;
-    lo.swap(fs.lo), hi.swap(fs.hi);
-  }
-  if (hi.size() > 0x7fffffffu) return fail(RTG_ERR_INVALID, "rtg_debug_box_plan: program too large");
+    *lean = (fs.features & (FEAT_ALL | FEAT_BOUNDARY)) == 0;
+    lo->swap(fs.lo), hi->swap(fs.hi);
+  }
+  if (hi->size() > 0x7fffffffu) return fail(RTG_ERR_INVALID, std::string(who) + ": program too large");
+  return RTG_OK;
+}
+
+int rtg_debug_box_plan(rtg_builder* b, const rtg_id* world, size_t n, const uint32_t* words, size_t n_records, uint8_t* mask_out,
+                       size_t capacity) {
+  std::vector<Packet> lo, hi;
+  bool lean = true;
+  int rc = debug_lean_program("rtg_debug_box_plan", b, world, n, words, n_records, &lo, &hi, &lean);
+  if (rc) return rc;
   std::vector<uint8_t> follower(hi.size(), 0), mask(hi.size(), 0);
   if (lean && !hi.empty()) {
     box_chain_followers(reinterpret_cast<const uint32_t (*)[4]>(lo.data()), reinterpret_cast<const uint32_t (*)[4]>(hi.data()), hi.size(), follower.data());
@@ -208,6 +216,30 @@
   }
   if (mask_out) std::memcpy(mask_out, mask.data(), std::min(mask.size(), capacity));
   return (int)hi.size();
+}
+
+int rtg_debug_production_program(rtg_builder* b, const rtg_id* world, size_t n, const uint32_t* words, size_t n_records,
+                                 uint32_t* words_out, uint32_t* origin_out, uint8_t* mask_out, size_t capacity) {
+  std::vector<Packet> lo, hi;
+  bool lean = true;
+  int rc = debug_lean_program("rtg_debug_production_program", b, world, n, words, n_records, &lo, &hi, &lean);
+  if (rc) return rc;
+  const size_t m = hi.size();
+  std::vector<Packet> plo(lo), phi(hi);
+  std::vector<uint32_t> origin(m);
+  std::vector<uint8_t> follower(m, 0), mask(m, 0);
+  for (size_t i = 0; i < m; i++) origin[i] = (uint32_t)i;
+  if (lean && m) {
+    box_tree_rebuild(reinterpret_cast<const uint32_t (*)[4]>(lo.data()), reinterpret_cast<const uint32_t (*)[4]>(hi.data()), m,
+                     reinterpret_cast<uint32_t (*)[4]>(plo.data()), reinterpret_cast<uint32_t (*)[4]>(phi.data()), origin.data());
+    box_chain_followers(reinterpret_cast<const uint32_t (*)[4]>(plo.data()), reinterpret_cast<const uint32_t (*)[4]>(phi.data()), m, follower.data());
+    box_plan(reinterpret_cast<const uint32_t (*)[4]>(plo.data()), reinterpret_cast<const uint32_t (*)[4]>(phi.data()), m, follower.data(), mask.data(), nullptr, BOX_PLAN_PROBES, BOX_TREE_PLAN);
+  }
+  const size_t k = std::min(m, capacity);
+  for (size_t i = 0; words_out && i < k; i++) std::memcpy(words_out + 8 * i, plo[i].w, 16), std::memcpy(words_out + 8 * i + 4, phi[i].w, 16);
+  if (origin_out) std::memcpy(origin_out, origin.data(), k * sizeof(uint32_t));
+  if (mask_out) std::memcpy(mask_out, mask.data(), k);
+  return (int)m;
 }
 
 int rtg_debug_math(int device, int op, size_t n, const float* in, const float* in2, float* out) {
```
